# langtech-bsc/quantool

Hardware: AMD Instinct MI355X
Metric: quantized weights/sec (GPTQ int4, Llama-3-8B, 512 calib samples) (higher is better)
Workload: dtype f32

## Files before the change

include/quantool_amd.h:

```cpp
#ifndef QUANTOOL_AMD_H
#define QUANTOOL_AMD_H

#include <stddef.h>
#include <stdint.h>

#ifdef __cplusplus
extern "C" {
#endif

typedef void* qt_stream_t;

enum qt_status {
    QT_OK = 0,
    QT_ERR_INVALID = -1,
    QT_ERR_NOT_PD = -2,
    QT_ERR_WORKSPACE = -3,
    QT_ERR_HIP = -4,
    QT_ERR_UNSUPPORTED = -5
};

enum qt_dtype { QT_F32 = 0, QT_BF16 = 1, QT_F16 = 2 };

int qt_version(void);
const char* qt_last_error(void);

size_t qt_xtx_workspace_bytes(int64_t n_tokens, int K);
int qt_xtx_accumulate(const void* X, int x_dtype, int64_t n_tokens, int K, int64_t ldx, float* G,
                      void* workspace, size_t workspace_bytes, qt_stream_t stream);

size_t qt_xtx_accumulate_f32_workspace_bytes(int64_t n_tokens, int K);
int qt_xtx_accumulate_f32(const float* X, int64_t n_tokens, int K, int64_t ldx, float* G, void* workspace,
                          size_t workspace_bytes, qt_stream_t stream);

size_t qt_act_stats_workspace_bytes(int64_t n_tokens, int K);
int qt_act_stats_accumulate(const void* X, int x_dtype, int64_t n_tokens, int K, int64_t ldx, float* abs_sum,
                            float* cmin, float* cmax, void* workspace, size_t workspace_bytes,
                            qt_stream_t stream);

size_t qt_hessian_prepare_workspace_bytes(int K);
int qt_hessian_prepare(const float* G, int K, int64_t n_samples, float percdamp,
                       const int32_t* perm, float* A, uint8_t* dead, float* diag_out,
                       void* workspace, size_t workspace_bytes, qt_stream_t stream);
int qt_hessian_prepare_damp(const float* G, int K, int64_t n_samples, float percdamp,
                            const int32_t* perm, float* A, uint8_t* dead, float* diag_out, float* damp_out,
                            void* workspace, size_t workspace_bytes, qt_stream_t stream);
int qt_hessian_diag(const float* G, int K, int64_t n_samples, float* diag_out, qt_stream_t stream);
int qt_argsort_desc(const float* values, int K, int32_t* perm, int32_t* inv, qt_stream_t stream);

size_t qt_cholesky_inverse_upper_workspace_bytes(int K);
int qt_cholesky_inverse_upper(float* A, int K, float* U, int32_t* info, void* workspace,
                              size_t workspace_bytes, qt_stream_t stream);

size_t qt_cholesky_inverse_upper_batched_workspace_bytes(int K, int n_problems);
int qt_cholesky_inverse_upper_batched(float* A, int64_t strideA, int K, float* U, int64_t strideU, int32_t* info,
                                      int n_problems, void* workspace, size_t workspace_bytes, qt_stream_t stream);

int qt_cholesky_inverse_upper_bounded(float* A, int K, float* U, int32_t* info, const float* min_eig_lb,
                                      void* workspace, size_t workspace_bytes, qt_stream_t stream);
int qt_cholesky_inverse_upper_batched_bounded(float* A, int64_t strideA, int K, float* U, int64_t strideU, int32_t* info,
                                              int n_problems, const float* min_eig_lb, void* workspace,
                                              size_t workspace_bytes, qt_stream_t stream);

int qt_group_minmax_qparams(const void* W, int w_dtype, int R, int K, int64_t ldw, int group_size,
                            int symmetric, int num_bits, float* scale, float* zp, float* scale_t,
                            float* zp_t, qt_stream_t stream);

int qt_weight_gather_f32(const void* W, int w_dtype, int R, int K, int64_t ldw, const int32_t* perm,
                         const uint8_t* dead, float* W_f32, qt_stream_t stream);

int qt_weight_gather_qparams(const void* W, int w_dtype, int R, int K, int64_t ldw, const int32_t* perm,
                             const uint8_t* dead, int group_size, int symmetric, int num_bits, float* W_f32, float* scale,
                             float* zp, float* scale_t, float* zp_t, int64_t ld_t, qt_stream_t stream);

size_t qt_gptq_sweep_workspace_bytes(int R, int K, int blocksize);
int qt_gptq_sweep(float* W, int R, int K, const float* U, const float* scale_t, const float* zp_t,
                  int G, const int32_t* g_idx, int blocksize, int num_bits, int8_t* Qt,
                  float* loss, void* workspace, size_t workspace_bytes, qt_stream_t stream);

int qt_gptq_sweep_grouped(float* W, int R, int K, const float* U, int64_t strideU, int n_groups, const int32_t* row_end,
                          const float* scale_t, const float* zp_t, int G, const int32_t* g_idx, int blocksize,
                          int num_bits, int8_t* Qt, float* loss, void* workspace, size_t workspace_bytes,
                          qt_stream_t stream);

int qt_pack_int4(const int8_t* Qt, int R, int K, const int32_t* col_src, int32_t* packed,
                 qt_stream_t stream);

int qt_dequantize(const int8_t* Qt, int R, int K, const int32_t* col_src, const float* scale,
                  const float* zp, int G, const int32_t* g_of_col, void* out, int out_dtype,
                  int64_t ldo, qt_stream_t stream);

size_t qt_awq_weight_mean_workspace_bytes(int R, int K);
int qt_awq_weight_mean_accumulate(const void* W, int w_dtype, int R, int K, int64_t ldw, int group_size,
                                  float* w_sum, void* workspace, size_t workspace_bytes,
                                  qt_stream_t stream);
int qt_awq_scales(const float* x_abs_sum, int64_t n_tokens, const float* w_sum, int64_t n_rows, int K,
                  int n_grid, int duo_scaling, float* scales, qt_stream_t stream);
int qt_symmetrize_lower(float* G, int K, qt_stream_t stream);
size_t qt_awq_loss_workspace_bytes(int R, int K);
int qt_awq_loss(const void* W, int w_dtype, int R, int K, int64_t ldw, const float* s, int group_size,
                int symmetric, int num_bits, const float* Gfull, int64_t n_tokens, int exact, float weight,
                int accumulate, float* loss_out, void* workspace, size_t workspace_bytes, qt_stream_t stream);
size_t qt_awq_losses_workspace_bytes(int R, int K, int n_grid);
int qt_awq_losses(const void* W, int w_dtype, int R, int K, int64_t ldw, const float* scales, int n_grid,
                  int group_size, int symmetric, int num_bits, const float* Gfull, int64_t n_tokens, float weight,
                  int accumulate, float* losses, void* workspace, size_t workspace_bytes, qt_stream_t stream);
int qt_argmin_f32(const float* values, int n, int32_t* index_out, qt_stream_t stream);
int qt_awq_pseudo_quantize(const void* W, int w_dtype, int R, int K, int64_t ldw, const float* s, int group_size,
                           int symmetric, int num_bits, void* out, int64_t ldo, qt_stream_t stream);
int qt_scale_columns(const void* W, int w_dtype, int R, int K, int64_t ldw, const float* s, int divide,
                     void* out, int64_t ldo, qt_stream_t stream);
int qt_rtn_quantize(const void* W, int w_dtype, int R, int K, int64_t ldw, const float* scale,
                    const float* zp, int G, int group_size, int num_bits, int8_t* Qt, qt_stream_t stream);

size_t qt_col_absmax_workspace_bytes(int R, int K);
int qt_col_absmax_accumulate(const void* W, int w_dtype, int R, int K, int64_t ldw, float* wmax,
                             void* workspace, size_t workspace_bytes, qt_stream_t stream);
int qt_smoothquant_scales(const float* cmin, const float* cmax, const float* wmax, int K, float alpha,
                          float* s, qt_stream_t stream);

size_t qt_sgemm_tn_f32_workspace_bytes(int M, int N);
int qt_sgemm_tn_f32(const float* A, int64_t lda, const float* B, int64_t ldb, const float* Cin,
                    int64_t ldcin, float* Cout, int64_t ldcout, int M, int N, int kdim, int skip_zero_k,
                    int mode, int allow_split_k, void* workspace, size_t workspace_bytes, qt_stream_t stream);

int qt_xtx_tile_table_check(int K, int* n_tiles_out, int* chunk_panels_out, int* round_panels_out);

size_t qt_xtx_dot_workspace_bytes(int64_t n_tokens, int K);
int qt_xtx_dot(const void* X, int x_dtype, int64_t n_tokens, int K, int64_t ldx, const float* H, double scale,
               float* out, int accumulate, void* workspace, size_t workspace_bytes, qt_stream_t stream);

size_t qt_gemm3_tn_f32_workspace_bytes(int M, int N, int k);
int qt_gemm3_tn_f32(const float* A, int64_t lda, const float* B, int64_t ldb, float* C, int64_t ldc, int M,
                    int N, int k, int kind, void* workspace, size_t workspace_bytes, qt_stream_t stream);
int qt_gemm3_tn_f32_ex(const float* A, int64_t lda, const float* B, int64_t ldb, float* C, int64_t ldc, int M, int N,
                       int k, int kind, int tri, int tight, int batch, int64_t bsA, int64_t bsB, int64_t bsC,
                       void* workspace, size_t workspace_bytes, qt_stream_t stream);

int qt_gemm3_tn_f16x2(const float* A, int64_t lda, const float* B, int64_t ldb, float* C, int64_t ldc, int M, int N,
                      int k, int kind, int tri, int tight, int batch, int64_t bsA, int64_t bsB, int64_t bsC,
                      const float* bound_a, const float* bound_b, void* workspace, size_t workspace_bytes,
                      qt_stream_t stream);

int qt_gemm3_plan_check(int Tm, int Tn, int c_end, int tri, int* n_items_out, int* n_slabs_out, int* longest_out);
int qt_chol_g3_plan_check(int K, int merged, int min_chunks, long long* counts_out);
enum qt_act { QT_ACT_SILU = 0 };
#define QT_I8_MID_MAX_M 128
#define QT_I8_MID_K_UNIT 128
#define QT_I8_RING_K_UNIT 128
#define QT_I8_RING_SLOTS 8
#define QT_I8_RING_LEAD 6
#define QT_I8_RING_W4_K_UNIT 128
#define QT_I8_RING_W4_SLOTS 8
#define QT_I8_RING_W4_LEAD 6
#define QT_MOE_I8_WIDE_K_UNIT 128
#define QT_MOE_I8_WIDE_TILE_ROWS 128
#define QT_MOE_I8_WIDE_MAX_E 4096
enum qt_weight_format { QT_W_INT8 = 0, QT_W_INT4_PACKED = 1 };
int qt_quantize_tokens_i8(const void* X, int x_dtype, int64_t M, int K, int64_t ldx, const int32_t* col_perm,
                          int symmetric, int8_t* Xq, float* s_x, int32_t* zp_x, qt_stream_t stream);
int qt_act_mul_quantize_i8(const void* gate, int64_t ldg, const void* up, int64_t ldu, int x_dtype, int64_t M, int K,
                           int act, const int32_t* col_perm, int symmetric, int8_t* Xq, float* s_x, int32_t* zp_x,
                           void* H, int64_t ldh, qt_stream_t stream);
int qt_rmsnorm_quantize_i8(const void* X, int64_t ldx, const void* weight, int x_dtype, int64_t M, int K, float eps,
                           const int32_t* col_perm, int symmetric, int8_t* Xq, float* s_x, int32_t* zp_x,
                           void* Y, int64_t ldy, float* rstd, qt_stream_t stream);
int qt_gemm_i8(const int8_t* Xq, int64_t M, int K, const void* Wq, int w_format, int N, const float* s_x,
               const int32_t* zp_x, const float* s_w, int G, const int32_t* wsum, const void* bias, void* Y,
               int out_dtype, int64_t ldy, qt_stream_t stream);
int qt_gemm_i8_skinny(const int8_t* Xq, int M, int K, const void* Wq, int w_format, int N, const float* s_x,
                      const int32_t* zp_x, const float* s_w, int G, const int32_t* wsum, const void* bias, void* Y,
                      int out_dtype, int64_t ldy, qt_stream_t stream);
int qt_gemm_i8_ring(const int8_t* Xq, int64_t M, int K, const void* Wq, int w_format, int N, const float* s_x,
                    const int32_t* zp_x, const float* s_w, int G, const int32_t* wsum, const void* bias, void* Y,
                    int out_dtype, int64_t ldy, qt_stream_t stream);
int qt_gemm_i8_ring_w4(const int8_t* Xq, int64_t M, int K, const void* Wq, int w_format, int N, const float* s_x,
                       const int32_t* zp_x, const float* s_w, int G, const int32_t* wsum, const void* bias, void* Y,
                       int out_dtype, int64_t ldy, qt_stream_t stream);
int qt_gemm_i8_mid(const int8_t* Xq, int64_t M, int K, const void* Wq, int w_format, int N, const float* s_x,
                   const int32_t* zp_x, const float* s_w, int G, const int32_t* wsum, const void* bias, void* Y,
                   int out_dtype, int64_t ldy, qt_stream_t stream);

int qt_moe_route(const void* top_k_index, int index_is_int64, int64_t T, int k, int E, int32_t* offsets,
                 int32_t* src_token, int32_t* src_slot, int32_t* row_of, qt_stream_t stream);
int qt_gemm_i8_grouped(const int8_t* Xq, int K, const int32_t* row_idx, int64_t R, const int32_t* offsets, int E,
                       const void* Wq, int w_format, int N, const float* s_x, const int32_t* zp_x, const float* s_w,
                       int G, const int32_t* wsum, void* Y, int out_dtype, int64_t ldy, qt_stream_t stream);
int qt_gemm_i8_skinny_grouped(const int8_t* Xq, int K, const int32_t* row_idx, int64_t R, const int32_t* offsets,
                              int E, const void* Wq, int w_format, int N, const float* s_x, const int32_t* zp_x,
                              const float* s_w, int G, const int32_t* wsum, void* Y, int out_dtype, int64_t ldy,
                              qt_stream_t stream);
int qt_gemm_i8_ring_grouped(const int8_t* Xq, int K, const int32_t* row_idx, int64_t R, const int32_t* offsets, int E,
                            const void* Wq, int w_format, int N, const float* s_x, const int32_t* zp_x,
                            const float* s_w, int G, const int32_t* wsum, void* Y, int out_dtype, int64_t ldy,
                            int64_t x_rows, qt_stream_t stream);
int qt_moe_gemm_i8_ring_w4(const int8_t* Xq, int K, const int32_t* row_idx, int64_t R, const int32_t* offsets, int E,
                           const void* Wq, int w_format, int N, const float* s_x, const int32_t* zp_x,
                           const float* s_w, int G, const int32_t* wsum, void* Y, int out_dtype, int64_t ldy,
                           int64_t x_rows, qt_stream_t stream);
int qt_moe_gemm_i8_wide(const int8_t* Xq, int K, const int32_t* row_idx, int64_t R, const int32_t* offsets, int E,
                        const void* Wq, int w_format, int N, const float* s_x, const int32_t* zp_x, const float* s_w,
                        int G, const int32_t* wsum, void* Y, int out_dtype, int64_t ldy, int64_t x_rows,
                        qt_stream_t stream);
int qt_moe_combine(const void* Y, int dtype, int H, int64_t ldy, const int32_t* row_of, const float* weights,
                   int64_t T, int k, void* out, qt_stream_t stream);

int qt_dequantize_weight(const void* Wq, int w_format, int N, int K, const float* s_w, int G, const int8_t* zp_w,
                         const int32_t* g_idx, void* W, int dtype, int64_t ldw, qt_stream_t stream);
int qt_gemm_wq_skinny(const void* X, int x_dtype, int M, int K, int64_t ldx, const void* Wq, int w_format, int N,
                      const float* s_w, int G, const int8_t* zp_w, const int32_t* g_idx, const void* bias, void* Y,
                      int64_t ldy, qt_stream_t stream);

int qt_gemm_wq_stream(const void* X, int x_dtype, int M, int K, int64_t ldx, const void* Wq, int w_format, int N,
                      const float* s_w, int G, const int8_t* zp_w, const int32_t* g_idx, const void* bias, void* Y,
                      int64_t ldy, qt_stream_t stream);
#define QT_WQ_STREAM_MAX_M 128
#define QT_WQ_STREAM_K_UNIT 128
#define QT_WQ_STREAM_MAX_LDX 33554432

int qt_gemm_wq_grouped(const void* X, int x_dtype, int K, int64_t ldx, const int32_t* row_idx, int64_t R,
                       const int32_t* offsets, int E, const void* Wq, int w_format, int N, const float* s_w, int G,
                       const int8_t* zp_w, const int32_t* g_idx, void* Y, int64_t ldy, qt_stream_t stream);

int qt_moe_gemm_wq_wide(const void* X, int x_dtype, int K, int64_t ldx, const int32_t* row_idx, int64_t R,
                        const int32_t* offsets, int E, const void* Wq, int w_format, int N, const float* s_w, int G,
                        const int8_t* zp_w, const int32_t* g_idx, void* Y, int64_t ldy, int64_t x_rows,
                        qt_stream_t stream);
#define QT_MOE_WQ_WIDE_K_UNIT 128
#define QT_MOE_WQ_WIDE_MAX_E 4096
#define QT_MOE_WQ_WIDE_MAX_SLOTS 65535

enum qt_prof_kernel { QT_PROF_XTX = 0, QT_PROF_SWEEP_BLOCK = 1, QT_PROF_NUM_KERNELS = 2 };
int qt_profile_enable(int on);
int qt_profile_read(int kernel_id, double* total_ms, int64_t* launches);

#ifdef __cplusplus
}
#endif
#endif
```

quantool_amd/csrc/cholesky.hip:

```cpp
#include <stdlib.h>
#include <string.h>

#include <map>
#include <tuple>
#include <vector>

#include "common.h"
#include "gemm3_tn.h"
#include "sgemm_tn.h"

namespace {

constexpr int NB = 128;
constexpr int NBO_MAX = 1024;
static int chol_block_env(const char* name) {
    const char* e = getenv(name);
    if (!e) return 0;
    int x = atoi(e) / 128 * 128;
    return x < 128 ? 128 : (x > NBO_MAX ? NBO_MAX : x);
}
struct G3Step {
    int n_items = 0, n_red = 0;
    size_t item_off = 0, red_off = 0;
};
struct CholG3Plan {
    bool any = false;
    std::vector<G3Step> fac, inv;
    std::vector<G3Step> row;
    char* blob = nullptr;
    size_t blob_bytes = 0;
    int max_slabs = 0;
    bool any_row = false;
};

static int chol_g3_min_chunks() {
    const char* on = getenv("QT_CHOL_G3");
    if (on && atoi(on) == 0) return 0;
    const char* e = getenv("QT_CHOL_G3_MIN_CHUNKS");
    const int x = e ? atoi(e) : 64;
    return x < 1 ? 1 : x;
}

static int chol_g3_target_items(int K) {
    const char* e = getenv("QT_G3_TARGET_ITEMS");
    if (e && atoi(e) > 0) return atoi(e);
    return K < 8192 ? 96 : 256;
}

enum { CHOL_TWO_PHASE = 0, CHOL_WALK = 1, CHOL_WALK_MERGED = 2 };
static int chol_merge_mode() {
    const char* e = getenv("QT_CHOL_MERGE");
    if (!e) return CHOL_WALK_MERGED;
    if (strcmp(e, "order") == 0) return CHOL_WALK;
    return atoi(e) != 0 ? CHOL_WALK_MERGED : CHOL_TWO_PHASE;
}

static void chol_g3_build(int K, int NBO, int NBI, int min_chunks, int target_items, bool merged, CholG3Plan& pl,
                          std::vector<char>& bytes) {
    pl = CholG3Plan();
    bytes.clear();
    int slab_budget = 0;
    if (merged) {
        CholG3Plan sep;
        std::vector<char> sep_bytes;
        chol_g3_build(K, NBO, NBI, min_chunks, target_items, false, sep, sep_bytes);
        slab_budget = sep.max_slabs;
    }
    auto enough = [&](int Tm, int Tn, int c_end, int tri) {
        return min_chunks > 0 && K % 8 == 0 && g3_row_chunks(Tm, Tn, c_end, tri) * G3_CHUNK_ROWS >= (long)min_chunks * 128;
    };
    auto store = [&](const std::vector<G3Item>& items, const std::vector<G3Red>& red) {
        G3Step st;
        st.n_items = (int)items.size();
        st.n_red = (int)red.size();
        st.item_off = qt_align_up(bytes.size(), 256);
        bytes.resize(st.item_off + items.size() * sizeof(G3Item));
        memcpy(bytes.data() + st.item_off, items.data(), items.size() * sizeof(G3Item));
        st.red_off = qt_align_up(bytes.size(), 256);
        bytes.resize(st.red_off + red.size() * sizeof(G3Red));
        if (!red.empty()) memcpy(bytes.data() + st.red_off, red.data(), red.size() * sizeof(G3Red));
        for (const G3Red& r : red) pl.max_slabs = pl.max_slabs > r.first + r.count ? pl.max_slabs : r.first + r.count;
        pl.any = true;
        return st;
    };
    auto add = [&](int Tm, int Tn, int c_end, int tri) {
        if (!enough(Tm, Tn, c_end, tri)) return G3Step();
        std::vector<G3Item> items;
        std::vector<G3Red> red;
        g3_plan_row(Tm, Tn, c_end, tri, items, red, target_items);
        return store(items, red);
    };
    const bool walk = merged && NBO == NBI;
    const int cap = target_items > 0 && target_items < 256 ? target_items : 256;
    pl.row.assign(walk ? (K + NBO - 1) / NBO : 0, G3Step());
    std::vector<char> is_merged(pl.row.size(), 0);
    for (int J0 = 0, Jb = 0; J0 < K; J0 += NBO, ++Jb) {
        const int J1 = (K - J0 < NBO) ? K : J0 + NBO;
        const int Tm = (J1 - J0 + 255) / 256, Tn0 = (K - J0 + 255) / 256, Tn1 = (J0 + 255) / 256, c_end = J0 / G3_CHUNK_ROWS;
        if (walk && J0 > 0 && 2 * Tm * (Tn0 + Tn1) <= cap && enough(Tm, Tn0, c_end, 0) && enough(Tm, Tn1, c_end, 1)) {
            std::vector<G3Item> items;
            std::vector<G3Red> red;
            g3_plan_row2(Tm, Tn0, Tn1, c_end, items, red, target_items, slab_budget);
            pl.row[Jb] = store(items, red);
            is_merged[Jb] = 1;
            pl.any_row = true;
        }
    }
    for (int J0 = 0, Jb = 0; J0 < K; J0 += NBO, ++Jb) {
        const int J1 = (K - J0 < NBO) ? K : J0 + NBO;
        const bool skip = J0 == 0 || (walk && is_merged[Jb]);
        pl.fac.push_back(skip ? G3Step() : add((J1 - J0 + 255) / 256, (K - J0 + 255) / 256, J0 / G3_CHUNK_ROWS, 0));
    }
    for (int I0 = 0, Ib = 0; I0 < K; I0 += NBI, ++Ib) {
        const int I1 = (K - I0 < NBI) ? K : I0 + NBI;
        const bool skip = I0 == 0 || (walk && is_merged[Ib]);
        pl.inv.push_back(skip ? G3Step() : add((I1 - I0 + 255) / 256, (I0 + 255) / 256, I0 / G3_CHUNK_ROWS, 1));
    }
    pl.blob_bytes = pl.any ? qt_align_up(bytes.size(), 256) : 0;
}

static const CholG3Plan* chol_g3_plan(int K, int NBO, int NBI, bool merged = false) {
    static std::mutex m;
    static std::map<std::tuple<int, int, int, int>, CholG3Plan*> plans;
    const int min_chunks = chol_g3_min_chunks();
    const int target_items = chol_g3_target_items(K);
    std::lock_guard<std::mutex> lock(m);
    const auto key = std::make_tuple(K, NBO, NBI, (merged ? 1 << 30 : 0) + min_chunks * 1024 + target_items);
    auto it = plans.find(key);
    if (it != plans.end()) return it->second;
    CholG3Plan* pl = new CholG3Plan();
    std::vector<char> bytes;
    chol_g3_build(K, NBO, NBI, min_chunks, target_items, merged, *pl, bytes);
    if (pl->any) {
        if (hipHostMalloc((void**)&pl->blob, pl->blob_bytes, hipHostMallocDefault) != hipSuccess) {
            pl->any = false;
            pl->blob = nullptr;
        } else {
            memcpy(pl->blob, bytes.data(), bytes.size());
        }
    }
    if (!pl->any) {
        pl->blob_bytes = 0;
        pl->max_slabs = 0;
        for (G3Step& st : pl->fac) st = G3Step();
        for (G3Step& st : pl->inv) st = G3Step();
        for (G3Step& st : pl->row) st = G3Step();
    }
    plans[key] = pl;
    return pl;
}
static size_t chol_g3_ws_bytes(const CholG3Plan* pl, int K) {
    if (!pl->any) return 0;
    return 2 * qt_align_up((size_t)3 * K * K * 2, 256) + (size_t)pl->max_slabs * 256 * 256 * 4 + pl->blob_bytes + 256;
}

static const CholG3Plan* chol_blocks(int K, int& NBO, int& NBI) {
    const int eo = chol_block_env("QT_CHOL_NBO"), ei = chol_block_env("QT_CHOL_NBI");
    NBO = eo ? eo : 512;
    NBI = ei ? ei : 512;
    const CholG3Plan* pl = chol_g3_plan(K, NBO, NBI);
    if (pl->any) return pl;
    NBO = eo ? eo : 256;
    NBI = ei ? ei : 256;
    return chol_g3_plan(K, NBO, NBI);
}

constexpr int LDP = NB + 1;

constexpr int LDT = NB + 4;
constexpr int RD_STRIDE = NB * NB + 4 * 32 * 32;

#define QT_SEL4(kb, v0, v1, v2, v3) ((kb) == 0 ? (v0) : (kb) == 1 ? (v1) : (kb) == 2 ? (v2) : (v3))

constexpr int LDA = NB + 4;

__device__ __forceinline__ float readlane_f(float v, int lane) {
    return __int_as_float(__builtin_amdgcn_readlane(__float_as_int(v), lane));
}

__device__ __forceinline__ void mma32_tn(const float* A, int lda, const float* B, int ldb, f32x16& acc,
                                         int l31, int h, bool negate_a) {
#pragma unroll
    for (int kk = 0; kk < 16; ++kk) {
        float a = A[(2 * kk + h) * lda + l31];
        const float b = B[(2 * kk + h) * ldb + l31];
        if (negate_a) a = -a;
        acc = __builtin_amdgcn_mfma_f32_32x32x2f32(a, b, acc, 0, 0, 0);
    }
}

constexpr int POTF2_THREADS = 512, POTF2_WAVES = POTF2_THREADS / 64;
__global__ __launch_bounds__(POTF2_THREADS) void potf2_kernel(const float* P, int64_t ldp, int n,
                                                    float* Rout, int64_t ldr,
                                                    float* __restrict__ Rd, int32_t* info, int col0, int prio,
                                                    int64_t bsP, int64_t bsRd) {
    qt_set_chain_prio(prio);
    if (blockIdx.x) {
        P += (size_t)blockIdx.x * bsP;
        Rout += (size_t)blockIdx.x * bsP;
        Rd += (size_t)blockIdx.x * bsRd;
        info += blockIdx.x;
    }
    extern __shared__ __attribute__((aligned(16))) float sm[];
    float* As = sm;
    float* Xs = sm + NB * LDA;
    const int tid = threadIdx.x, lane = tid & 63;
    const int wave = __builtin_amdgcn_readfirstlane(tid >> 6);
    const int l31 = lane & 31, h = lane >> 5;

    if ((ldp & 3) == 0 && (n & 3) == 0 && (((uintptr_t)P) & 15) == 0) {
        constexpr int NV = NB * NB / 4 / POTF2_THREADS;
        f32x4 v[NV];
#pragma unroll
        for (int r = 0; r < NV; ++r) {
            const int e4 = tid + POTF2_THREADS * r;
            const int i = e4 >> 5, j = (e4 & 31) * 4;
            const int ic = i < n ? i : n - 1, jc = j < n ? j : n - 4;
            v[r] = *(const f32x4*)(P + (size_t)ic * ldp + jc);
        }
#pragma unroll
        for (int r = 0; r < NV; ++r) {
            const int e4 = tid + POTF2_THREADS * r;
            const int i = e4 >> 5, j = (e4 & 31) * 4;
            f32x4 x;
#pragma unroll
            for (int q = 0; q < 4; ++q) x[q] = (i < n && j + q < n) ? v[r][q] : (i == j + q ? 1.0f : 0.0f);
            *(f32x4*)(As + i * LDA + j) = x;
        }
    } else {
        for (int e = tid; e < NB * NB; e += POTF2_THREADS) {
            const int i = e / NB, j = e % NB;
            const int lo = i < j ? i : j, hi = i < j ? j : i;
            float v = (i == j) ? 1.0f : 0.0f;
            if (hi < n) v = P[(size_t)lo * ldp + hi];
            As[i * LDA + j] = v;
        }
    }
    __syncthreads();

    int bad = 0;
#pragma unroll 1
    for (int kb = 0; kb < 4; ++kb) {
        float* Akk = As + (32 * kb) * LDA + 32 * kb;
        if (wave == 0) {
            f32x16 c1, c2;
#pragma unroll
            for (int r = 0; r < 16; ++r) {
                const int i = (r & 3) + 8 * (r >> 2) + 4 * h;
                c1[r] = Akk[i * LDA + l31];
                c2[r] = (i == l31) ? 1.0f : 0.0f;
            }
#pragma unroll
            for (int c = 0; c < 32; ++c) {
                const int rc = (c & 3) + 4 * (c >> 3);
                const int hc = (c >> 2) & 1;
                float piv = readlane_f(c1[rc], c + 32 * hc);
                const bool isbad = !(piv > 0.0f);
                bad = (isbad && bad == 0 && 32 * kb + c < n) ? 32 * kb + c + 1 : bad;
                piv = isbad ? 1.0f : piv;
                float rs = __builtin_amdgcn_rsqf(piv);
                rs = rs * fmaf(-0.5f * piv * rs, rs, 1.5f);
                const bool mine = h == hc;
                const float rr = c1[rc] * rs, zz = c2[rc] * rs;
                c1[rc] = mine ? rr : c1[rc];
                c2[rc] = mine ? zz : c2[rc];
                if (c < 31) {
                    const float a = (mine && l31 > c) ? -rr : 0.0f;
                    const float b1 = (mine && l31 >= c) ? rr : 0.0f, b2 = mine ? zz : 0.0f;
                    c1 = __builtin_amdgcn_mfma_f32_32x32x2f32(a, b1, c1, 0, 0, 0);
                    c2 = __builtin_amdgcn_mfma_f32_32x32x2f32(a, b2, c2, 0, 0, 0);
                }
            }
#pragma unroll
            for (int r = 0; r < 16; ++r) {
                const int i = (r & 3) + 8 * (r >> 2) + 4 * h;
                Akk[i * LDA + l31] = (i <= l31) ? c1[r] : 0.0f;
                Xs[(kb * 32 + l31) * 32 + i] = (i >= l31) ? c2[r] : 0.0f;
            }
        }
        __syncthreads();
        if (kb == 3) break;
        for (int a = kb + 1 + wave; a < 4; a += POTF2_WAVES) {
            f32x16 acc;
#pragma unroll
            for (int r = 0; r < 16; ++r) acc[r] = 0.0f;
            float* Bt = As + (32 * kb) * LDA + 32 * a;
            mma32_tn(Xs + kb * 1024, 32, Bt, LDA, acc, l31, h, false);
#pragma unroll
            for (int r = 0; r < 16; ++r) Bt[((r & 3) + 8 * (r >> 2) + 4 * h) * LDA + l31] = acc[r];
        }
        __syncthreads();
        {
            int t = 0;
            for (int a = kb + 1; a < 4; ++a)
                for (int a2 = a; a2 < 4; ++a2, ++t) {
                    if ((t % POTF2_WAVES) != wave) continue;
                    float* Ct = As + (32 * a) * LDA + 32 * a2;
                    f32x16 acc;
#pragma unroll
                    for (int r = 0; r < 16; ++r) acc[r] = Ct[((r & 3) + 8 * (r >> 2) + 4 * h) * LDA + l31];
                    mma32_tn(As + (32 * kb) * LDA + 32 * a, LDA, As + (32 * kb) * LDA + 32 * a2, LDA, acc, l31, h,
                             true);
#pragma unroll
                    for (int r = 0; r < 16; ++r) Ct[((r & 3) + 8 * (r >> 2) + 4 * h) * LDA + l31] = acc[r];
                }
        }
        __syncthreads();
    }
    if (bad != 0 && tid == 0) atomicCAS(info, 0, col0 + bad);
    const bool vec_out = (ldr & 3) == 0 && (n & 3) == 0 && (((uintptr_t)Rout) & 15) == 0;
    for (int e4 = tid; e4 < NB * NB / 4; e4 += POTF2_THREADS) {
        const int i = e4 >> 5, j = (e4 & 31) * 4;
        f32x4 v = *(const f32x4*)(As + i * LDA + j);
#pragma unroll
        for (int q = 0; q < 4; ++q) v[q] = (j + q >= i) ? v[q] : 0.0f;
        *(f32x4*)(Rd + i * NB + j) = v;
        if (i < n && j + 3 >= i && j < n) {
            if (vec_out) {
                *(f32x4*)(Rout + (size_t)i * ldr + j) = v;
            } else {
#pragma unroll
                for (int q = 0; q < 4; ++q)
                    if (j + q >= i && j + q < n) Rout[(size_t)i * ldr + j + q] = v[q];
            }
        }
    }
    for (int e4 = tid; e4 < 4 * 32 * 32 / 4; e4 += POTF2_THREADS) *(f32x4*)(Rd + NB * NB + 4 * e4) = *(const f32x4*)(Xs + 4 * e4);
}

__global__ __launch_bounds__(256) void trsm_rt_kernel(const float* __restrict__ Rd, int n,
                                                      const float* B, int64_t ldb,
                                                      float* Z, int64_t ldz, int ncols, int prio, int64_t bsRd,
                                                      int64_t bsB) {
    qt_set_chain_prio(prio);
    if (blockIdx.y) {
        Rd += (size_t)blockIdx.y * bsRd;
        B += (size_t)blockIdx.y * bsB;
        Z += (size_t)blockIdx.y * bsB;
    }
    extern __shared__ __attribute__((aligned(16))) float Rs[];
    const int tid = threadIdx.x, lane = tid & 63, wave = tid >> 6;
    const float* D32 = Rs + NB * NB;
    const int l31 = lane & 31, h = lane >> 5;
    const int col = blockIdx.x * 128 + wave * 32 + l31;
    const bool cok = col < ncols;
    const int colc = cok ? col : ncols - 1;

    f32x16 acc[4];
#pragma unroll
    for (int a = 0; a < 4; ++a)
#pragma unroll
        for (int r = 0; r < 16; ++r) {
            const int row = 32 * a + (r & 3) + 8 * (r >> 2) + 4 * h;
            acc[a][r] = (row < n) ? B[(size_t)row * ldb + colc] : 0.0f;
        }
    {
        constexpr int NV = RD_STRIDE / 4 / 256;
        static_assert(NV * 4 * 256 == RD_STRIDE, "whole float4s per thread");
        f32x4 v[NV];
#pragma unroll
        for (int r = 0; r < NV; ++r) v[r] = ((const f32x4*)Rd)[tid + 256 * r];
#pragma unroll
        for (int r = 0; r < NV; ++r) ((f32x4*)Rs)[tid + 256 * r] = v[r];
    }
    __syncthreads();

#pragma unroll
    for (int b = 0; b < 4; ++b) {
        f32x16 zb;
#pragma unroll
        for (int r = 0; r < 16; ++r) zb[r] = 0.0f;
#pragma unroll
        for (int r = 0; r < 16; ++r) {
            const int k = (r & 3) + 8 * (r >> 2) + 4 * h;
            const float av = D32[(b * 32 + k) * 32 + l31];
            zb = __builtin_amdgcn_mfma_f32_32x32x2f32(av, acc[b][r], zb, 0, 0, 0);
        }
        acc[b] = zb;
#pragma unroll
        for (int a = b + 1; a < 4; ++a) {
#pragma unroll
            for (int r = 0; r < 16; ++r) {
                const int k = (r & 3) + 8 * (r >> 2) + 4 * h;
                const float av = -Rs[(32 * b + k) * NB + 32 * a + l31];
                acc[a] = __builtin_amdgcn_mfma_f32_32x32x2f32(av, zb[r], acc[a], 0, 0, 0);
            }
        }
    }
    if (cok) {
#pragma unroll
        for (int a = 0; a < 4; ++a)
#pragma unroll
            for (int r = 0; r < 16; ++r) {
                const int row = 32 * a + (r & 3) + 8 * (r >> 2) + 4 * h;
                if (row < n) Z[(size_t)row * ldz + col] = acc[a][r];
            }
    }
}

__global__ __launch_bounds__(128) void trinv_batched_kernel(const float* __restrict__ Rd_all, int K,
                                                            float* __restrict__ Dinv_all,
                                                            float* __restrict__ Y, int64_t ldy, int64_t bsW, int64_t bsY,
                                                            int blk0) {
    if (blockIdx.y) {
        Rd_all += (size_t)blockIdx.y * bsW;
        Dinv_all += (size_t)blockIdx.y * bsW;
        Y += (size_t)blockIdx.y * bsY;
    }
    extern __shared__ __attribute__((aligned(16))) float sm[];
    float* Rt = sm;
    float* Xs = sm + NB * LDT;
    const int b = blk0 + blockIdx.x;
    const int n = (K - b * NB < NB) ? K - b * NB : NB;
    const float* Rd = Rd_all + (size_t)b * RD_STRIDE;
    const int j = threadIdx.x;
    for (int e = j; e < NB * NB; e += NB) {
        const int i = e / NB, c = e % NB;
        Rt[c * LDT + i] = Rd[e];
    }
    __syncthreads();
    float x0[32], x1[32], x2[32], x3[32];
#pragma unroll
    for (int r = 0; r < 32; ++r) {
        x0[r] = (r == j) ? 1.0f : 0.0f;
        x1[r] = (32 + r == j) ? 1.0f : 0.0f;
        x2[r] = (64 + r == j) ? 1.0f : 0.0f;
        x3[r] = (96 + r == j) ? 1.0f : 0.0f;
    }
#pragma unroll 1
    for (int pb = 3; pb >= 0; --pb) {
#pragma unroll
        for (int pp = 31; pp >= 0; --pp) {
            const int p = 32 * pb + pp;
            const float* rp = Rt + p * LDT;
            const float xp = QT_SEL4(pb, x0[pp], x1[pp], x2[pp], x3[pp]) / rp[p];
            if (pb == 0) x0[pp] = xp;
            if (pb == 1) x1[pp] = xp;
            if (pb == 2) x2[pp] = xp;
            if (pb == 3) x3[pp] = xp;
#define QT_XUPD(arr, a, r_to)                                                 \
    _Pragma("unroll") for (int r4 = 0; r4 < (r_to); r4 += 4) {                 \
        const f32x4 v4 = *(const f32x4*)(rp + 32 * (a) + r4);                 \
        _Pragma("unroll") for (int e = 0; e < 4; ++e)                         \
            if (r4 + e < (r_to)) arr[r4 + e] = fmaf(-v4[e], xp, arr[r4 + e]); \
    }
            if (pb == 0) { QT_XUPD(x0, 0, pp) } else { QT_XUPD(x0, 0, 32) }
            if (pb == 1) { QT_XUPD(x1, 1, pp) } else if (pb > 1) { QT_XUPD(x1, 1, 32) }
            if (pb == 2) { QT_XUPD(x2, 2, pp) } else if (pb > 2) { QT_XUPD(x2, 2, 32) }
            if (pb == 3) { QT_XUPD(x3, 3, pp) }
#undef QT_XUPD
        }
    }
#pragma unroll
    for (int r = 0; r < 32; ++r) {
        Xs[r * LDP + j] = x0[r];
        Xs[(32 + r) * LDP + j] = x1[r];
        Xs[(64 + r) * LDP + j] = x2[r];
        Xs[(96 + r) * LDP + j] = x3[r];
    }
    __syncthreads();
    float* Dinv = Dinv_all + (size_t)b * NB * NB;
    float* Yd = Y + (size_t)(b * NB) * ldy + b * NB;
    for (int e = j; e < NB * NB; e += NB) {
        const int i = e / NB, jj = e % NB;
        const bool in = (i < n && jj < n);
        Dinv[e] = (in && jj >= i) ? Xs[i * LDP + jj] : 0.0f;
        if (in) Yd[(size_t)i * ldy + jj] = (jj <= i) ? Xs[jj * LDP + i] : 0.0f;
    }
}

__global__ __launch_bounds__(256) void trinv_mfma_kernel(const float* __restrict__ Rd_all, int K,
                                                         float* __restrict__ Dinv_all,
                                                         float* __restrict__ Y, int64_t ldy, int64_t bsW, int64_t bsY,
                                                         int blk0) {
    if (blockIdx.y) {
        Rd_all += (size_t)blockIdx.y * bsW;
        Dinv_all += (size_t)blockIdx.y * bsW;
        Y += (size_t)blockIdx.y * bsY;
    }
    extern __shared__ __attribute__((aligned(16))) float Rs[];
    const int blk = blk0 + blockIdx.x;
    const int n = (K - blk * NB < NB) ? K - blk * NB : NB;
    const float* Rd = Rd_all + (size_t)blk * RD_STRIDE;
    const int tid = threadIdx.x, lane = tid & 63, wave = tid >> 6;
    {
        constexpr int NV = RD_STRIDE / 4 / 256;
        f32x4 v[NV];
#pragma unroll
        for (int r = 0; r < NV; ++r) v[r] = ((const f32x4*)Rd)[tid + 256 * r];
#pragma unroll
        for (int r = 0; r < NV; ++r) ((f32x4*)Rs)[tid + 256 * r] = v[r];
    }
    const float* D32 = Rs + NB * NB;
    const int l31 = lane & 31, h = lane >> 5;
    const int col = wave * 32 + l31;

    f32x16 acc[4];
#pragma unroll
    for (int a = 0; a < 4; ++a)
#pragma unroll
        for (int r = 0; r < 16; ++r) {
            const int row = 32 * a + (r & 3) + 8 * (r >> 2) + 4 * h;
            acc[a][r] = (row == col) ? 1.0f : 0.0f;
        }
    __syncthreads();

#pragma unroll
    for (int b = 0; b < 4; ++b) {
        f32x16 zb;
#pragma unroll
        for (int r = 0; r < 16; ++r) zb[r] = 0.0f;
#pragma unroll
        for (int r = 0; r < 16; ++r) {
            const int k = (r & 3) + 8 * (r >> 2) + 4 * h;
            const float av = D32[(b * 32 + k) * 32 + l31];
            zb = __builtin_amdgcn_mfma_f32_32x32x2f32(av, acc[b][r], zb, 0, 0, 0);
        }
        acc[b] = zb;
#pragma unroll
        for (int a = b + 1; a < 4; ++a) {
#pragma unroll
            for (int r = 0; r < 16; ++r) {
                const int k = (r & 3) + 8 * (r >> 2) + 4 * h;
                const float av = -Rs[(32 * b + k) * NB + 32 * a + l31];
                acc[a] = __builtin_amdgcn_mfma_f32_32x32x2f32(av, zb[r], acc[a], 0, 0, 0);
            }
        }
    }
    float* Dinv = Dinv_all + (size_t)blk * NB * NB;
    float* Yd = Y + (size_t)(blk * NB) * ldy + blk * NB;
#pragma unroll
    for (int a = 0; a < 4; ++a)
#pragma unroll
        for (int r = 0; r < 16; ++r) {
            const int row = 32 * a + (r & 3) + 8 * (r >> 2) + 4 * h;
            const bool in = row < n && col < n;
            const float z = (in && row >= col) ? acc[a][r] : 0.0f;
            Dinv[col * NB + row] = z;
            if (in) Yd[(size_t)row * ldy + col] = z;
        }
}

__global__ __launch_bounds__(256) void transpose_lower_block_kernel(const float* __restrict__ Y, int64_t ldy, int w,
                                                                    float* __restrict__ XT, int ldx, int64_t bsY,
                                                                    int64_t bsXT) {
    if (blockIdx.z) {
        Y += (size_t)blockIdx.z * bsY;
        XT += (size_t)blockIdx.z * bsXT;
    }
    __shared__ float tile[32][33];
    const int bx = blockIdx.x * 32, by = blockIdx.y * 32;
    const int tx = threadIdx.x & 31, ty = threadIdx.x >> 5;
    for (int r = ty; r < 32; r += 8) {
        const int m = bx + r, k = by + tx;
        tile[r][tx] = (m < w && k < w && k <= m) ? Y[(size_t)m * ldy + k] : 0.0f;
    }
    __syncthreads();
    for (int r = ty; r < 32; r += 8) {
        const int k = by + r, m = bx + tx;
        if (k < w && m < w) XT[(size_t)k * ldx + m] = tile[tx][r];
    }
}

__global__ __launch_bounds__(256) void flat_reverse_lower_to_upper_kernel(float* __restrict__ U, int K, int64_t bsU) {
    U += (size_t)blockIdx.z * bsU;
    const int j = blockIdx.x * blockDim.x + threadIdx.x;
    const int i = blockIdx.y;
    if (j >= K || j < i) return;
    const size_t e = (size_t)i * K + j;
    const size_t pe = (size_t)(K - 1 - i) * K + (K - 1 - j);
    if (i == j) {
        if (e <= pe) {
            const float t = U[e];
            U[e] = U[pe];
            U[pe] = t;
        }
    } else {
        U[e] = U[pe];
        U[pe] = 0.0f;
    }
}

__global__ __launch_bounds__(256) void identity_if_failed_kernel(float* __restrict__ U, int K,
                                                                 const int32_t* __restrict__ info, int64_t bsU) {
    if (info[blockIdx.z] == 0) return;
    U += (size_t)blockIdx.z * bsU;
    for (int i = blockIdx.x; i < K; i += gridDim.x)
        for (int j = threadIdx.x; j < K; j += blockDim.x) U[(size_t)i * K + j] = (i == j) ? 1.0f : 0.0f;
}

__global__ __launch_bounds__(256) void chol_scales_kernel(const float* __restrict__ A, int64_t bsA, int K,
                                                          const float* __restrict__ min_eig_lb, int32_t* __restrict__ e,
                                                          int32_t* __restrict__ info) {
    __shared__ float red[256];
    const int b = blockIdx.x, nprob = gridDim.x;
    const float* Ab = A + (size_t)b * bsA;
    float m = 0.0f;
    for (int i = threadIdx.x; i < K; i += 256) m = fmaxf(m, Ab[(size_t)i * K + i]);
    red[threadIdx.x] = m;
    __syncthreads();
    for (int s = 128; s > 0; s >>= 1) {
        if ((int)threadIdx.x < s) red[threadIdx.x] = fmaxf(red[threadIdx.x], red[threadIdx.x + s]);
        __syncthreads();
    }
    if (threadIdx.x == 0) {
        auto clampe = [](float t) { return (int)fminf(fmaxf(t, (float)-G3_E_MAX), (float)G3_E_MAX); };
        const float d = red[0], lb = min_eig_lb[b];
        e[b] = (d > 0.0f && d < 3.0e38f) ? clampe(3.0f - ceilf(0.5f * log2f(d))) : 0;
        if (lb > 0.0f && lb < 3.0e38f) {
            e[nprob + b] = clampe(3.0f - ceilf(-0.5f * log2f(lb)));
        } else {
            e[nprob + b] = 0;
            info[b] = K + 1;
        }
    }
}

}

static size_t chol_problem_ws_bytes(int K, const CholG3Plan* g3) {
    const size_t nb = (K + NB - 1) / NB;
    const size_t split = (size_t)2048 * NB * NB * 4 + (size_t)NBO_MAX * K * 4;
    size_t n = (size_t)NB * K * 4 + (size_t)NBO_MAX * K * 4 + (size_t)NBO_MAX * NBO_MAX * 4 + nb * (NB * NB + RD_STRIDE) * 4 + split + 256;
    if (g3->any) n += 2 * qt_align_up((size_t)3 * K * K * 2, 256) + (size_t)g3->max_slabs * 256 * 256 * 4 + 256;
    return qt_align_up(n, 256);
}

extern "C" size_t qt_cholesky_inverse_upper_batched_workspace_bytes(int K, int n_problems) {
    if (K <= 0 || n_problems <= 0) return 0;
    int nbo_, nbi_;
    const CholG3Plan* g3 = chol_blocks(K, nbo_, nbi_);
    return (size_t)n_problems * chol_problem_ws_bytes(K, g3) + g3->blob_bytes + 512;
}

extern "C" size_t qt_cholesky_inverse_upper_workspace_bytes(int K) {
    return qt_cholesky_inverse_upper_batched_workspace_bytes(K, 1);
}

static int chol_run(float* A, int64_t strideA, int K, float* U, int64_t strideU, int32_t* info, int nprob, void* workspace,
                    size_t workspace_bytes, hipStream_t stream, const float* min_eig_lb = nullptr) {
    bool f16x2 = min_eig_lb != nullptr;
    if (const char* e = getenv("QT_CHOL_PLANES")) {
        if (strcmp(e, "bf16x3") == 0) f16x2 = false;
        else if (strcmp(e, "f16x2") == 0) {
            QT_CHECK_ARG(min_eig_lb, "qt_cholesky_inverse_upper: QT_CHOL_PLANES=f16x2 needs a bound on lambda_min (the _bounded entry points)");
        } else {
            QT_CHECK_ARG(false, "qt_cholesky_inverse_upper: QT_CHOL_PLANES=%s (bf16x3 | f16x2)", e);
        }
    }
    const size_t need = qt_cholesky_inverse_upper_batched_workspace_bytes(K, nprob);
    if (!workspace || workspace_bytes < need) {
        qt_set_error("qt_cholesky_inverse_upper: workspace %zu < required %zu", workspace_bytes, need);
        return QT_ERR_WORKSPACE;
    }
    const int nblk = (K + NB - 1) / NB;
    char* ws = (char*)qt_align_up((size_t)workspace, 256);
    int NBO, NBI;
    const CholG3Plan* g3 = chol_blocks(K, NBO, NBI);
    int merge_mode = (g3->any && NBO == NBI) ? chol_merge_mode() : CHOL_TWO_PHASE;
    const CholG3Plan* tab = g3;
    if (merge_mode == CHOL_WALK_MERGED) {
        tab = chol_g3_plan(K, NBO, NBI, true);
        if (!tab->any || !tab->any_row || tab->max_slabs > g3->max_slabs || tab->blob_bytes > g3->blob_bytes) {
            tab = g3;
            merge_mode = CHOL_TWO_PHASE;
        }
    }
    const size_t prob_bytes = chol_problem_ws_bytes(K, g3);
    const int64_t sW = (int64_t)(prob_bytes / 4);
    const int64_t sA = nprob > 1 ? strideA : 0, sU = nprob > 1 ? strideU : 0;
    float* T = (float*)ws;
    float* TI = T + (size_t)NB * K;
    float* XT = TI + (size_t)NBO_MAX * K;
    float* Rd = XT + (size_t)NBO_MAX * NBO_MAX;
    float* Dinv = Rd + (size_t)nblk * RD_STRIDE;
    float* split_ws = Dinv + (size_t)nblk * NB * NB;
    const size_t split_ws_bytes = (size_t)2048 * NB * NB * 4 + (size_t)NBO_MAX * K * 4;
    unsigned short *Rpl = nullptr, *Ypl = nullptr;
    float* g3_slabs = nullptr;
    char* g3_tab = nullptr;
    const int64_t plane_stride = (int64_t)K * K;
    if (g3->any) {
        char* q = (char*)qt_align_up((size_t)((char*)split_ws + split_ws_bytes), 256);
        Rpl = (unsigned short*)q;
        q += qt_align_up((size_t)3 * K * K * 2, 256);
        Ypl = (unsigned short*)q;
        q += qt_align_up((size_t)3 * K * K * 2, 256);
        g3_slabs = (float*)q;
        g3_tab = (char*)qt_align_up((size_t)(ws + (size_t)nprob * prob_bytes), 256);
        QT_HIP(hipMemcpyAsync(g3_tab, tab->blob, tab->blob_bytes, hipMemcpyHostToDevice, stream));
    }
    f16x2 = f16x2 && g3->any;
    int32_t* eR = f16x2 ? (int32_t*)(Rpl + 2 * plane_stride) : nullptr;
    int32_t* eY = f16x2 ? eR + nprob : nullptr;
    static_assert(2 * SG_MAX_BATCH * sizeof(int32_t) <= (size_t)NB * NB * 2, "the exponents fit the smallest third plane");
    auto g3_row = [&](const G3Step& st, const unsigned short* Bplanes, int col_a0, int col_b0, int M, int N, float* C,
                      int64_t bsC, int mode, bool second = false) -> int {
        G3Args a;
        a.Apl = Rpl;
        a.Bpl = Bplanes;
        a.plane_stride = plane_stride;
        a.ld = K;
        a.rowA0 = a.rowB0 = 0;
        a.colA0 = col_a0;
        a.colB0 = col_b0;
        a.colmax = K;
        a.M = M;
        a.N = N;
        a.C = C;
        a.ldc = K;
        a.mode = mode;
        a.slabs = g3_slabs;
        a.items = (const G3Item*)(g3_tab + st.item_off);
        a.n_items = st.n_items;
        a.red = (const G3Red*)(g3_tab + st.red_off);
        a.n_red = st.n_red;
        a.batch = nprob;
        a.bsApl = a.bsBpl = sW * 2;
        a.bsC = bsC;
        a.bsSlabs = sW;
        if (f16x2) {
            a.planes = G3_F16X2;
            a.eA = eR;
            a.eB = Bplanes == Rpl ? eR : eY;
        }
        if (second) {
            a.Bpl1 = Ypl;
            a.colB01 = 0;
            a.eB1 = eY;
            a.C1 = TI;
            a.ldc1 = K;
            a.bsC1 = sW;
            a.mode1 = G3_SET;
            a.N1 = col_a0;
        }
        return qt_gemm3_launch(a, stream);
    };
    auto sgemm = [&](SgemmArgs& g, int64_t bsA_, int64_t bsB_, int64_t bsC_) -> int {
        g.batch = nprob;
        g.bsA = bsA_;
        g.bsB = bsB_;
        g.bsCin = g.bsCout = bsC_;
        g.bs_split = sW;
        return qt_sgemm_tn(g, stream);
    };
    float* Y = U;
    const int64_t sY = sU;
    const size_t inv_lds = (size_t)(NB * LDT + NB * LDP) * sizeof(float);
    const size_t potf2_lds = (size_t)(NB * LDA + 4 * 32 * 32) * sizeof(float);
    static QtOncePerDevice lds_attr;
    QT_HIP(lds_attr.run([&] {
        hipError_t e = hipFuncSetAttribute((const void*)potf2_kernel, hipFuncAttributeMaxDynamicSharedMemorySize,
                                           (int)potf2_lds);
        if (e == hipSuccess)
            e = hipFuncSetAttribute((const void*)trsm_rt_kernel, hipFuncAttributeMaxDynamicSharedMemorySize,
                                    (int)(RD_STRIDE * sizeof(float)));
        if (e == hipSuccess)
            e = hipFuncSetAttribute((const void*)trinv_batched_kernel, hipFuncAttributeMaxDynamicSharedMemorySize,
                                    (int)inv_lds);
        if (e == hipSuccess)
            e = hipFuncSetAttribute((const void*)trinv_mfma_kernel, hipFuncAttributeMaxDynamicSharedMemorySize,
                                    (int)(RD_STRIDE * sizeof(float)));
        return e;
    }));
    QT_HIP(hipMemsetAsync(info, 0, sizeof(int32_t) * nprob, stream));
    const int prio = qt_chain_prio();
    if (f16x2) {
        hipLaunchKernelGGL(chol_scales_kernel, dim3(nprob), dim3(256), 0, stream, (const float*)A, sA, K, min_eig_lb, eR, info);
        QT_LAUNCH_CHECK();
    }

    auto fac_product = [&](int J0, int J1, int Jb) -> int {
        if (!(g3->any && J0 > 0)) return QT_OK;
        const G3Step& st = tab->fac[Jb];
        float* C = A + (size_t)J0 * K + J0;
        if (st.n_items > 0) return g3_row(st, Rpl, J0, J0, J1 - J0, K - J0, C, sA, G3_SUB);
        SgemmArgs g;
        g.A = A + J0; g.lda = K;
        g.B = A + J0; g.ldb = K;
        g.Cin = C; g.ldcin = K;
        g.Cout = C; g.ldcout = K;
        g.M = J1 - J0; g.N = K - J0; g.kdim = J0; g.k_mode = SG_K_FULL; g.mode = SG_MODE_SUB;
        g.split_ws = split_ws; g.split_ws_bytes = split_ws_bytes;
        return sgemm(g, sA, sA, sA);
    };
    auto fac_panels = [&](int J0, int J1) -> int {
        for (int j0 = J0; j0 < J1; j0 += NB) {
            const int j = j0 / NB, nbj = (K - j0 < NB) ? K - j0 : NB;
            float* Ajj = A + (size_t)j0 * K + j0;
            if (j0 > J0) {
                SgemmArgs g;
                g.A = A + (size_t)J0 * K + j0; g.lda = K;
                g.B = A + (size_t)J0 * K + j0; g.ldb = K;
                g.Cin = Ajj; g.ldcin = K;
                g.Cout = Ajj; g.ldcout = K;
                g.M = nbj; g.N = K - j0; g.kdim = j0 - J0; g.k_mode = SG_K_FULL; g.mode = SG_MODE_SUB;
                int rc = sgemm(g, sA, sA, sA);
                if (rc) return rc;
            }
            hipLaunchKernelGGL(potf2_kernel, dim3(nprob), dim3(POTF2_THREADS), potf2_lds, stream, (const float*)Ajj, (int64_t)K, nbj,
                               Ajj, (int64_t)K, Rd + (size_t)j * RD_STRIDE, info, j0, prio, sA, sW);
            QT_LAUNCH_CHECK();
            const int rest = K - j0 - nbj;
            if (rest > 0) {
                hipLaunchKernelGGL(trsm_rt_kernel, dim3((rest + 127) / 128, nprob), dim3(256), RD_STRIDE * sizeof(float),
                                   stream, (const float*)(Rd + (size_t)j * RD_STRIDE), nbj, (const float*)(Ajj + nbj),
                                   (int64_t)K, Ajj + nbj, (int64_t)K, rest, prio, sW, sA);
                QT_LAUNCH_CHECK();
            }
        }
        const int rem = K - J1;
        if (g3->any) {
            if (rem > 0) {
                int rc = f16x2 ? qt_split2h_launch(A + (size_t)J0 * K + J0, K, J1 - J0, K - J0, Rpl + (size_t)J0 * K + J0, K,
                                                   plane_stride, 0, 0, 0, eR, stream, nprob, sA, sW * 2)
                               : qt_split3_launch(A + (size_t)J0 * K + J0, K, J1 - J0, K - J0, Rpl + (size_t)J0 * K + J0, K,
                                                  plane_stride, 0, 0, 0, stream, nprob, sA, sW * 2);
                if (rc) return rc;
            }
        } else if (rem > 0) {
            SgemmArgs g;
            g.A = A + (size_t)J0 * K + J1; g.lda = K;
            g.B = A + (size_t)J0 * K + J1; g.ldb = K;
            g.Cin = A + (size_t)J1 * K + J1; g.ldcin = K;
            g.Cout = A + (size_t)J1 * K + J1; g.ldcout = K;
            g.M = rem; g.N = rem; g.kdim = J1 - J0; g.k_mode = SG_K_FULL; g.mode = SG_MODE_SUB;
            g.upper_only = 1;
            int rc = sgemm(g, sA, sA, sA);
            if (rc) return rc;
        }
        return QT_OK;
    };
    auto trinv = [&](int blk0, int n) -> int {
        const char* e = getenv("QT_CHOL_TRINV");
        if (e && strcmp(e, "div") == 0)
            hipLaunchKernelGGL(trinv_batched_kernel, dim3(n, nprob), dim3(NB), inv_lds, stream, (const float*)Rd, K, Dinv, Y,
                               (int64_t)K, sW, sY, blk0);
        else
            hipLaunchKernelGGL(trinv_mfma_kernel, dim3(n, nprob), dim3(256), RD_STRIDE * sizeof(float), stream,
                               (const float*)Rd, K, Dinv, Y, (int64_t)K, sW, sY, blk0);
        QT_LAUNCH_CHECK();
        return QT_OK;
    };
    auto inv_product = [&](int I0, int I1, int Ib) -> int {
        if (I0 == 0) return QT_OK;
        if (g3->any && tab->inv[Ib].n_items > 0) return g3_row(tab->inv[Ib], Ypl, I0, 0, I1 - I0, I0, TI, sW, G3_SET);
        SgemmArgs g;
        g.A = A + I0; g.lda = K;
        g.B = Y; g.ldb = K;
        g.Cin = nullptr; g.ldcin = 0;
        g.Cout = TI; g.ldcout = K;
        g.M = I1 - I0; g.N = I0; g.kdim = I0; g.k_mode = SG_K_FROM_N0; g.mode = SG_MODE_SET;
        g.split_ws = split_ws; g.split_ws_bytes = split_ws_bytes;
        return sgemm(g, sA, sY, sW);
    };
    auto inv_row = [&](int I0, int I1) -> int {
        const int Wi = I1 - I0;
        for (int i0 = I0 + NB; i0 < I1; i0 += NB) {
            const int i = i0 / NB, nbi = (K - i0 < NB) ? K - i0 : NB;
            SgemmArgs g;
            g.A = A + (size_t)I0 * K + i0; g.lda = K;
            g.B = Y + (size_t)I0 * K + I0; g.ldb = K;
            g.Cin = nullptr; g.ldcin = 0;
            g.Cout = T; g.ldcout = K;
            g.M = nbi; g.N = i0 - I0; g.kdim = i0 - I0; g.k_mode = SG_K_FROM_N0; g.mode = SG_MODE_SET;
            int rc = sgemm(g, sA, sY, sW);
            if (rc) return rc;
            SgemmArgs t;
            t.A = Dinv + (size_t)i * NB * NB; t.lda = NB;
            t.B = T; t.ldb = K;
            t.Cin = nullptr; t.ldcin = 0;
            t.Cout = Y + (size_t)i0 * K + I0; t.ldcout = K;
            t.M = nbi; t.N = i0 - I0; t.kdim = nbi; t.k_mode = SG_K_FULL; t.mode = SG_MODE_NEG;
            rc = sgemm(t, sW, sW, sY);
            if (rc) return rc;
        }
        auto split_row = [&]() -> int {
            if (!g3->any || I1 >= K) return QT_OK;
            if (f16x2)
                return qt_split2h_launch(Y + (size_t)I0 * K, K, Wi, I1, Ypl + (size_t)I0 * K, K, plane_stride, 1, I0, 0, eY,
                                         stream, nprob, sY, sW * 2);
            return qt_split3_launch(Y + (size_t)I0 * K, K, Wi, I1, Ypl + (size_t)I0 * K, K, plane_stride, 1, I0, 0, stream,
                                    nprob, sY, sW * 2);
        };
        if (I0 == 0) return split_row();
        hipLaunchKernelGGL(transpose_lower_block_kernel, dim3((Wi + 31) / 32, (Wi + 31) / 32, nprob), dim3(256), 0, stream,
                           (const float*)(Y + (size_t)I0 * K + I0), (int64_t)K, Wi, XT, NBO_MAX, sY, sW);
        QT_LAUNCH_CHECK();
        SgemmArgs t;
        t.A = XT; t.lda = NBO_MAX;
        t.B = TI; t.ldb = K;
        t.Cin = nullptr; t.ldcin = 0;
        t.Cout = Y + (size_t)I0 * K; t.ldcout = K;
        t.M = Wi; t.N = I0; t.kdim = Wi; t.k_mode = SG_K_FULL; t.mode = SG_MODE_NEG;
        int rc = sgemm(t, sW, sW, sY);
        if (rc) return rc;
        return split_row();
    };
    if (merge_mode == CHOL_TWO_PHASE) {
        for (int J0 = 0, Jb = 0; J0 < K; J0 += NBO, ++Jb) {
            const int J1 = (K - J0 < NBO) ? K : J0 + NBO;
            int rc = fac_product(J0, J1, Jb);
            if (!rc) rc = fac_panels(J0, J1);
            if (rc) return rc;
        }
        int rc = trinv(0, nblk);
        if (rc) return rc;
        for (int I0 = 0, Ib = 0; I0 < K; I0 += NBI, ++Ib) {
            const int I1 = (K - I0 < NBI) ? K : I0 + NBI;
            rc = inv_product(I0, I1, Ib);
            if (!rc) rc = inv_row(I0, I1);
            if (rc) return rc;
        }
    } else {
        for (int J0 = 0, Jb = 0; J0 < K; J0 += NBO, ++Jb) {
            const int J1 = (K - J0 < NBO) ? K : J0 + NBO;
            int rc;
            if (merge_mode == CHOL_WALK_MERGED && tab->row[Jb].n_items > 0) {
                rc = g3_row(tab->row[Jb], Rpl, J0, J0, J1 - J0, K - J0, A + (size_t)J0 * K + J0, sA, G3_SUB, true);
            } else {
                rc = fac_product(J0, J1, Jb);
                if (!rc) rc = inv_product(J0, J1, Jb);
            }
            if (!rc) rc = fac_panels(J0, J1);
            if (!rc) rc = trinv(J0 / NB, (J1 - J0 + NB - 1) / NB);
            if (!rc) rc = inv_row(J0, J1);
            if (rc) return rc;
        }
    }
    hipLaunchKernelGGL(flat_reverse_lower_to_upper_kernel, dim3((K + 255) / 256, K, nprob), dim3(256), 0, stream, U, K, sU);
    QT_LAUNCH_CHECK();
    hipLaunchKernelGGL(identity_if_failed_kernel, dim3(K < 1024 ? K : 1024, 1, nprob), dim3(256), 0, stream, U, K,
                       (const int32_t*)info, sU);
    QT_LAUNCH_CHECK();
    return QT_OK;
}

extern "C" int qt_cholesky_inverse_upper(float* A, int K, float* U, int32_t* info, void* workspace,
                                         size_t workspace_bytes, qt_stream_t stream_) {
    QT_CHECK_ARG(K > 0 && A && U && info, "qt_cholesky_inverse_upper: bad arguments");
    return chol_run(A, 0, K, U, 0, info, 1, workspace, workspace_bytes, (hipStream_t)stream_);
}

extern "C" int qt_cholesky_inverse_upper_batched(float* A, int64_t strideA, int K, float* U, int64_t strideU, int32_t* info,
                                                 int n_problems, void* workspace, size_t workspace_bytes,
                                                 qt_stream_t stream_) {
    QT_CHECK_ARG(K > 0 && A && U && info && n_problems >= 1 && n_problems <= SG_MAX_BATCH,
                 "qt_cholesky_inverse_upper_batched: bad arguments (1 <= n_problems <= %d)", SG_MAX_BATCH);
    QT_CHECK_ARG(n_problems == 1 || (strideA >= (int64_t)K * K && strideU >= (int64_t)K * K && strideA % 4 == 0 && strideU % 4 == 0),
                 "qt_cholesky_inverse_upper_batched: strides must be multiples of 4 elements and >= K*K");
    return chol_run(A, strideA, K, U, strideU, info, n_problems, workspace, workspace_bytes, (hipStream_t)stream_);
}

extern "C" int qt_cholesky_inverse_upper_bounded(float* A, int K, float* U, int32_t* info, const float* min_eig_lb,
                                                 void* workspace, size_t workspace_bytes, qt_stream_t stream_) {
    QT_CHECK_ARG(K > 0 && A && U && info && min_eig_lb, "qt_cholesky_inverse_upper_bounded: bad arguments");
    return chol_run(A, 0, K, U, 0, info, 1, workspace, workspace_bytes, (hipStream_t)stream_, min_eig_lb);
}

extern "C" int qt_cholesky_inverse_upper_batched_bounded(float* A, int64_t strideA, int K, float* U, int64_t strideU,
                                                         int32_t* info, int n_problems, const float* min_eig_lb,
                                                         void* workspace, size_t workspace_bytes, qt_stream_t stream_) {
    QT_CHECK_ARG(K > 0 && A && U && info && min_eig_lb && n_problems >= 1 && n_problems <= SG_MAX_BATCH,
                 "qt_cholesky_inverse_upper_batched_bounded: bad arguments (1 <= n_problems <= %d)", SG_MAX_BATCH);
    QT_CHECK_ARG(n_problems == 1 || (strideA >= (int64_t)K * K && strideU >= (int64_t)K * K && strideA % 4 == 0 && strideU % 4 == 0),
                 "qt_cholesky_inverse_upper_batched_bounded: strides must be multiples of 4 elements and >= K*K");
    return chol_run(A, strideA, K, U, strideU, info, n_problems, workspace, workspace_bytes, (hipStream_t)stream_, min_eig_lb);
}

extern "C" int qt_chol_g3_plan_check(int K, int merged, int min_chunks, long long* counts_out) {
    if (K <= 0) return -1;
    constexpr int NBX = 512, TRI_STEP = 256 / G3_CHUNK_ROWS;
    if (min_chunks <= 0) min_chunks = 64;
    const int cap = chol_g3_target_items(K);
    CholG3Plan sep, pl;
    std::vector<char> sep_bytes, bytes;
    chol_g3_build(K, NBX, NBX, min_chunks, cap, false, sep, sep_bytes);
    chol_g3_build(K, NBX, NBX, min_chunks, cap, merged != 0, pl, bytes);
    if (pl.max_slabs > sep.max_slabs || pl.blob_bytes > sep.blob_bytes) return -2;
    long long launches = 0, n_items = 0, n_slabs = 0;
    auto check = [&](const G3Step& st, int Tm, int Tn0, int tri0, int Tn1, int c_end) -> int {
        if (st.n_items <= 0) return 0;
        const G3Item* items = (const G3Item*)(bytes.data() + st.item_off);
        const G3Red* red = (const G3Red*)(bytes.data() + st.red_off);
        if (st.n_items > cap && st.n_items > Tm * (Tn0 + Tn1)) return -3;
        const int Tn[2] = {Tn0, Tn1};
        auto lo_of = [&](int seg, int tj) { return (seg == 1 || tri0) ? TRI_STEP * tj : 0; };
        std::vector<int> cover((size_t)2 * Tm * (Tn0 + Tn1 + 1) * c_end, 0);
        auto cell = [&](int seg, int ti, int tj, int c) { return (((size_t)seg * Tm + ti) * (Tn0 + Tn1 + 1) + tj) * c_end + c; };
        std::vector<int> owner(sep.max_slabs, -1);
        int slabs_here = 0;
        for (int q = 0; q < st.n_items; ++q) {
            const G3Item& it = items[q];
            const int seg = (it.tile & G3_SEG_BIT) ? 1 : 0, ti = it.tile >> 16, tj = it.tile & G3_TJ_MASK;
            if (ti < 0 || ti >= Tm || tj >= Tn[seg]) return -4;
            const int lo = lo_of(seg, tj);
            if (it.c_lo < lo || it.c_hi > c_end || it.c_hi - it.c_lo < 2) return -5;
            for (int c = it.c_lo; c < it.c_hi; ++c) cover[cell(seg, ti, tj, c)]++;
            if (it.slab < 0) {
                if (it.c_lo != lo || it.c_hi != c_end) return -6;
            } else {
                if (it.slab >= sep.max_slabs) return -7;
                if (owner[it.slab] >= 0) return -8;
                owner[it.slab] = q;
                ++slabs_here;
            }
        }
        for (int seg = 0; seg < 2; ++seg)
            for (int ti = 0; ti < Tm; ++ti)
                for (int tj = 0; tj < Tn[seg]; ++tj)
                    for (int c = 0; c < c_end; ++c)
                        if (cover[cell(seg, ti, tj, c)] != (c >= lo_of(seg, tj) ? 1 : 0)) return -9;
        int in_red = 0;
        for (int r = 0; r < st.n_red; ++r) {
            const G3Red& e = red[r];
            if (e.count < 2 || e.first < 0 || e.first + e.count > sep.max_slabs || (e.seg != 0 && e.seg != 1)) return -10;
            const int want_tile = e.tile | (e.seg ? G3_SEG_BIT : 0);
            int prev_hi = lo_of(e.seg, e.tile & G3_TJ_MASK);
            for (int q = 0; q < e.count; ++q) {
                const int o = owner[e.first + q];
                if (o < 0 || items[o].tile != want_tile || items[o].c_lo != prev_hi) return -11;
                prev_hi = items[o].c_hi;
                owner[e.first + q] = -2;
            }
            if (prev_hi != c_end) return -12;
            in_red += e.count;
        }
        if (in_red != slabs_here) return -13;
        ++launches;
        n_items += st.n_items;
        n_slabs += slabs_here;
        return 0;
    };
    for (int J0 = 0, Jb = 0; J0 < K; J0 += NBX, ++Jb) {
        const int J1 = (K - J0 < NBX) ? K : J0 + NBX;
        const int Tm = (J1 - J0 + 255) / 256, Tn0 = (K - J0 + 255) / 256, Tn1 = (J0 + 255) / 256, c_end = J0 / G3_CHUNK_ROWS;
        int rc = 0;
        if (Jb < (int)pl.row.size() && pl.row[Jb].n_items > 0) {
            if (pl.fac[Jb].n_items > 0 || pl.inv[Jb].n_items > 0) return -14;
            rc = check(pl.row[Jb], Tm, Tn0, 0, Tn1, c_end);
        } else {
            rc = check(pl.fac[Jb], Tm, Tn0, 0, 0, c_end);
            if (!rc) rc = check(pl.inv[Jb], Tm, Tn1, 1, 0, c_end);
        }
        if (rc) return rc;
    }
    if (counts_out) {
        counts_out[0] = launches;
        counts_out[1] = n_items;
        counts_out[2] = n_slabs;
        counts_out[3] = sep.max_slabs;
        counts_out[4] = (long long)pl.blob_bytes;
    }
    return 0;
}
```

quantool_amd/csrc/common.h:

```cpp
#pragma once
#include <hip/hip_runtime.h>
#include <stdint.h>
#include <stdio.h>

#include <mutex>

#include "../../include/quantool_amd.h"

typedef __attribute__((ext_vector_type(8))) __bf16 bf16x8;
typedef __attribute__((ext_vector_type(8))) _Float16 f16x8;
typedef __attribute__((ext_vector_type(4))) short s16x4;
typedef __attribute__((ext_vector_type(8))) short s16x8;
typedef __attribute__((ext_vector_type(2))) float f32x2;
typedef __attribute__((ext_vector_type(4))) float f32x4;
typedef __attribute__((ext_vector_type(16))) float f32x16;

#define QT_LDS __attribute__((address_space(3)))
#define QT_GLOBAL __attribute__((address_space(1)))

void qt_set_error(const char* fmt, ...);
void qt_prof_mark(int kernel_id, hipStream_t stream);

#define QT_CHECK_ARG(cond, ...)         \
    do {                                \
        if (!(cond)) {                  \
            qt_set_error(__VA_ARGS__);  \
            return QT_ERR_INVALID;      \
        }                               \
    } while (0)

#define QT_HIP(expr)                                                              \
    do {                                                                          \
        hipError_t _e = (expr);                                                   \
        if (_e != hipSuccess) {                                                   \
            qt_set_error("%s failed: %s (%s:%d)", #expr, hipGetErrorString(_e),   \
                         __FILE__, __LINE__);                                     \
            return QT_ERR_HIP;                                                    \
        }                                                                         \
    } while (0)

#define QT_LAUNCH_CHECK()                                                         \
    do {                                                                          \
        hipError_t _e = hipGetLastError();                                        \
        if (_e != hipSuccess) {                                                   \
            qt_set_error("kernel launch failed: %s (%s:%d)", hipGetErrorString(_e), \
                         __FILE__, __LINE__);                                     \
            return QT_ERR_HIP;                                                    \
        }                                                                         \
    } while (0)

static inline size_t qt_align_up(size_t x, size_t a) { return (x + a - 1) / a * a; }

size_t qt_xtx_frobenius_workspace_bytes(int64_t n_tokens, int K, int n_batch);
int qt_xtx_frobenius(const void* X, int x_dtype, int64_t n_tokens, int K, int64_t ldx, const float* H, double scale,
                     float* loss_out, int accumulate, void* workspace, size_t workspace_bytes, hipStream_t stream,
                     int n_batch, int64_t x_batch_stride);

int qt_chain_prio();
__device__ __forceinline__ void qt_set_chain_prio(int prio) {
    if (prio >= 3) __builtin_amdgcn_s_setprio(3);
    else if (prio == 2) __builtin_amdgcn_s_setprio(2);
    else if (prio == 1) __builtin_amdgcn_s_setprio(1);
}

struct QtOncePerDevice {
    std::mutex m;
    uint64_t done = 0;
    template <class F>
    hipError_t run(F&& f) {
        int dev = 0;
        hipError_t e = hipGetDevice(&dev);
        if (e != hipSuccess) return e;
        const uint64_t bit = 1ull << (dev & 63);
        std::lock_guard<std::mutex> lock(m);
        if (done & bit) return hipSuccess;
        e = f();
        if (e == hipSuccess) done |= bit;
        return e;
    }
};

__device__ __forceinline__ float qt_bf16_to_f32(unsigned short h) {
    return __uint_as_float(((unsigned)h) << 16);
}
__device__ __forceinline__ float qt_f16_to_f32(unsigned short h) {
    return (float)__builtin_bit_cast(_Float16, h);
}
__device__ __forceinline__ float qt_h16_to_f32(unsigned short h, int dtype) {
    return dtype == QT_F16 ? qt_f16_to_f32(h) : qt_bf16_to_f32(h);
}
__device__ __forceinline__ float qt_load_w(const void* W, int dtype, size_t idx) {
    if (dtype == QT_F32) return ((const float*)W)[idx];
    return qt_h16_to_f32(((const unsigned short*)W)[idx], dtype);
}
__device__ __forceinline__ void qt_store_w(void* out, int dtype, size_t idx, float v) {
    if (dtype == QT_F32) ((float*)out)[idx] = v;
    else if (dtype == QT_F16) ((_Float16*)out)[idx] = (_Float16)v;
    else ((__bf16*)out)[idx] = (__bf16)v;
}
static inline bool qt_dtype_ok(int d) { return d == QT_F32 || d == QT_BF16 || d == QT_F16; }
static inline bool qt_dtype_is16(int d) { return d == QT_BF16 || d == QT_F16; }
static inline size_t qt_dtype_size(int d) { return d == QT_F32 ? 4 : 2; }
```

quantool_amd/csrc/gemm3_tn.h:

```cpp
#pragma once
#include <vector>

#include "common.h"

constexpr int G3_CHUNK_ROWS = 64;

struct G3Item {
    int tile;
    int c_lo;
    int c_hi;
    int slab;
};
struct G3Red {
    int tile;
    int first;
    int count;
    int seg;
};
constexpr int G3_SEG_BIT = 1 << 15;
constexpr int G3_TJ_MASK = G3_SEG_BIT - 1;

enum { G3_SUB = 0, G3_SET = 1, G3_ADD = 2 };

enum { G3_BF16X3 = 0, G3_F16X2 = 1 };
constexpr int G3_E_MAX = 40;

struct G3Args {
    const unsigned short* Apl;
    const unsigned short* Bpl;
    int64_t plane_stride;
    int64_t ld;
    int64_t rowA0, rowB0;
    int colA0, colB0;
    int colmax;
    int M, N;
    float* C;
    int64_t ldc;
    int64_t ldB = 0, plane_strideB = 0;
    int colmaxB = 0;
    int mode;
    float* slabs;
    const G3Item* items;
    int n_items;
    const G3Red* red;
    int n_red;
    int batch = 1;
    int64_t bsApl = 0, bsBpl = 0, bsC = 0, bsSlabs = 0;
    int planes = G3_BF16X3;
    const int32_t* eA = nullptr;
    const int32_t* eB = nullptr;
    const unsigned short* Bpl1 = nullptr;
    int colB01 = 0;
    const int32_t* eB1 = nullptr;
    float* C1 = nullptr;
    int64_t ldc1 = 0, bsC1 = 0;
    int mode1 = G3_SET;
    int N1 = 0;
};

int qt_gemm3_launch(const G3Args& a, hipStream_t stream);

int qt_split3_launch(const float* src, int64_t ld_src, int rows, int cols, unsigned short* planes, int64_t ld_pl,
                     int64_t plane_stride, int mask_upper, int row_g0, int col_g0, hipStream_t stream, int batch = 1,
                     int64_t bs_src = 0, int64_t bs_planes = 0);

int qt_split2h_launch(const float* src, int64_t ld_src, int rows, int cols, unsigned short* planes, int64_t ld_pl,
                      int64_t plane_stride, int mask_upper, int row_g0, int col_g0, const int32_t* e, hipStream_t stream,
                      int batch = 1, int64_t bs_src = 0, int64_t bs_planes = 0);

int g3_scale_exponent(float bound);

long g3_row_chunks(int Tm, int Tn, int c_end, int tri);
void g3_plan_row(int Tm, int Tn, int c_end, int tri, std::vector<G3Item>& items, std::vector<G3Red>& red, int target_items = 0);
void g3_plan_row2(int Tm, int Tn0, int Tn1, int c_end, std::vector<G3Item>& items, std::vector<G3Red>& red,
                  int target_items = 0, int max_slabs = 0);
```

quantool_amd/csrc/gemm3_tn.hip:

```cpp
#include <math.h>
#include <stdlib.h>
#include <string.h>

#include <algorithm>
#include <map>
#include <mutex>
#include <type_traits>

#include "gemm3_tn.h"
#include "ring_pipe.h"

namespace {

constexpr int RING = 8;
constexpr int CH_ROWS = G3_CHUNK_ROWS;
constexpr int CH_UNITS = 6 * (CH_ROWS / UT);
constexpr int TRING = 3;
constexpr int TRI_BYTES = 3 * UNIT_BYTES;
constexpr int TRI_DMA = 6;
constexpr int DRING = 4;
constexpr int DUO_BYTES = 2 * UNIT_BYTES;
constexpr int DUO_DMA = 4;
constexpr int DUO_LEAD = 2;
enum { LOOP_CHUNK = 0, LOOP_TRI = 1, LOOP_DUO = 2 };
static_assert(CH_ROWS / UT == 4, "the phase code below recomputes the source pointers every 4 units");
constexpr unsigned PA_BITS = 2u | (0u << 2) | (1u << 4) | (1u << 6) | (0u << 8) | (0u << 10);
constexpr unsigned PB_BITS = 0u | (2u << 2) | (1u << 4) | (0u << 6) | (1u << 8) | (0u << 10);
constexpr int g3_plane_a(int pr) { return (PA_BITS >> (2 * pr)) & 3u; }
constexpr int g3_plane_b(int pr) { return (PB_BITS >> (2 * pr)) & 3u; }

struct G3Params {
    const char* Apl;
    const char* Bpl;
    int64_t plane_bytes, plane_bytesB;
    int64_t ld2, ld2B;
    int64_t rowA0, rowB0;
    int colA0, colB0, colmax, colmaxB;
    int M, N;
    float* C;
    int64_t ldc;
    float* slabs;
    const G3Item* items;
    int64_t bsA_bytes, bsB_bytes, bsC, bsSlabs;
    const int32_t* eA;
    const int32_t* eB;
    const char* Bpl1;
    const int32_t* eB1;
    float* C1;
    int64_t ldc1, bsC1;
    int colB01, N1, mode1;
};

template <int MODE, int LOOP>
__global__ __launch_bounds__(NTHREADS, 2) void gemm3_kernel(G3Params p) {
    constexpr bool TRI = LOOP == LOOP_TRI;
    __shared__ __attribute__((aligned(16))) char ring[LOOP == LOOP_DUO ? DRING * DUO_BYTES : TRI ? TRING * TRI_BYTES : RING * UNIT_BYTES];
    const int tid = threadIdx.x;
    const int lane = tid & 63;
    const int wave = __builtin_amdgcn_readfirstlane(tid >> 6);
    const int wave_m = wave >> 2, wave_n = wave & 3;
    const bool group_b = wave >= 4;

    const G3Item* itp = p.items + blockIdx.x;
    const int it_tile = __builtin_amdgcn_readfirstlane(itp->tile);
    const bool seg1 = (it_tile & G3_SEG_BIT) != 0;
    const char* Bpl = seg1 ? p.Bpl1 : p.Bpl;
    const int colB0 = seg1 ? p.colB01 : p.colB0;
    if (blockIdx.y) {
        p.Apl += (size_t)blockIdx.y * p.bsA_bytes;
        Bpl += (size_t)blockIdx.y * p.bsB_bytes;
        p.slabs += (size_t)blockIdx.y * p.bsSlabs;
    }
    const int c_lo = __builtin_amdgcn_readfirstlane(itp->c_lo);
    const int c_hi = __builtin_amdgcn_readfirstlane(itp->c_hi);
    const int slab_idx = __builtin_amdgcn_readfirstlane(itp->slab);
    const int ti = it_tile >> 16, tj = it_tile & G3_TJ_MASK;
    const int nu = (c_hi - c_lo) * (LOOP != LOOP_CHUNK ? CH_ROWS / UT : CH_UNITS);

    const int rsub = lane >> 4;
    const int lch = (lane & 15) ^ (rsub << 2);
    const int trow = 4 * (wave & 3) + rsub;
    int colA = p.colA0 + ti * BT + (wave >> 2) * 128 + lch * 8;
    int colB = colB0 + tj * BT + (wave >> 2) * 128 + lch * 8;
    colA = colA > p.colmax - 8 ? p.colmax - 8 : colA;
    colB = colB > p.colmaxB - 8 ? p.colmaxB - 8 : colB;
    const unsigned voffA = (unsigned)((size_t)trow * (size_t)p.ld2 + (size_t)colA * 2);
    const unsigned voffB = (unsigned)((size_t)trow * (size_t)p.ld2B + (size_t)colB * 2);
    const unsigned ring_lds = (unsigned)(size_t)(QT_LDS char*)ring;
    const unsigned dst_wave =
        __builtin_amdgcn_readfirstlane(ring_lds + (wave >> 2) * 4096 + (wave & 3) * 1024);

    const int64_t ustride = (int64_t)UT * p.ld2, ustrideB = (int64_t)UT * p.ld2B;

    const int g = lane >> 4, il = lane & 15, q = il >> 2, pp = il & 3;
    const int rowpart = (8 * (g >> 1) + q) * 256 + 32 * (g & 1) + 8 * pp;
    int aoff[4], boff[2];
#pragma unroll
    for (int mi = 0; mi < 4; ++mi) aoff[mi] = wave_m * 4096 + rowpart + 64 * (mi ^ q);
#pragma unroll
    for (int ni = 0; ni < 2; ++ni)
        boff[ni] = (2 + (wave_n >> 1)) * 4096 + rowpart + 64 * ((((wave_n & 1) << 1) + ni) ^ q);

    f32x16 acc[4][2];
#pragma unroll
    for (int mi = 0; mi < 4; ++mi)
#pragma unroll
        for (int ni = 0; ni < 2; ++ni)
#pragma unroll
            for (int r = 0; r < 16; ++r) acc[mi][ni][r] = 0.0f;

    if constexpr (LOOP == LOOP_DUO) {
        const char* runA = p.Apl + (p.rowA0 + (int64_t)c_lo * CH_ROWS) * p.ld2;
        const char* runB = Bpl + (p.rowB0 + (int64_t)c_lo * CH_ROWS) * p.ld2B;
        auto issue2 = [&](int slot) {
            const unsigned d = dst_wave + (unsigned)slot * DUO_BYTES;
#pragma unroll
            for (int pl = 0; pl < 2; ++pl)
                glds16_pair2(voffA, voffB, runA + pl * p.plane_bytes, runB + pl * p.plane_bytesB, d + pl * UNIT_BYTES,
                             d + pl * UNIT_BYTES + 8192);
            runA += ustride;
            runB += ustrideB;
        };
        s16x8 fa[2][4], fb[2][2];
        auto phase = [&](auto slot_c, int u) {
            constexpr int S = decltype(slot_c)::value;
            constexpr int ISLOT = (S + DUO_LEAD) % DRING;
            const char* base = ring + S * DUO_BYTES;
#pragma unroll
            for (int pl = 0; pl < 2; ++pl) {
#pragma unroll
                for (int mi = 0; mi < 4; ++mi) fa[pl][mi] = tr_load8(base + pl * UNIT_BYTES + aoff[mi]);
#pragma unroll
                for (int ni = 0; ni < 2; ++ni) fb[pl][ni] = tr_load8(base + pl * UNIT_BYTES + boff[ni]);
            }
            if (u + DUO_LEAD < nu) issue2(ISLOT);
            ring_drain_wait<DUO_DMA, DUO_LEAD>(nu - u - 2);
            ring_sync_math([&] {
                s16x8 fbs[2];
#pragma unroll
                for (int ni = 0; ni < 2; ++ni)
                    fbs[ni] = __builtin_bit_cast(s16x8, __builtin_bit_cast(f16x8, fb[0][ni]) * (_Float16)2048.0f);
                ring_mma32<true>(fa[1], fb[0], acc);
                ring_mma32<true>(fa[0], fb[1], acc);
                ring_mma32<true>(fa[0], fbs, acc);
            });
        };
        if (nu > 0) {
            issue2(0);
            issue2(1);
            wait_vmcnt<DUO_DMA*(DUO_LEAD - 1)>();
            ring_stagger_begin(group_b);
            for (int u = 0; u < nu; u += DRING) ring_body<DRING>(phase, u);
            ring_stagger_end(group_b);
        }
        const int es = -(11 + p.eA[blockIdx.y] + (seg1 ? p.eB1 : p.eB)[blockIdx.y]);
        const float unscale = __builtin_bit_cast(float, (unsigned)(127 + (es < -126 ? -126 : es > 127 ? 127 : es)) << 23);
#pragma unroll
        for (int mi = 0; mi < 4; ++mi)
#pragma unroll
            for (int ni = 0; ni < 2; ++ni)
#pragma unroll
                for (int r = 0; r < 16; ++r) acc[mi][ni][r] *= unscale;
    } else if constexpr (TRI) {
        const char* runA = p.Apl + (p.rowA0 + (int64_t)c_lo * CH_ROWS) * p.ld2;
        const char* runB = Bpl + (p.rowB0 + (int64_t)c_lo * CH_ROWS) * p.ld2B;
        auto issue3 = [&](int slot) {
            const unsigned d = dst_wave + (unsigned)slot * TRI_BYTES;
#pragma unroll
            for (int pl = 0; pl < 3; ++pl)
                glds16_pair2(voffA, voffB, runA + pl * p.plane_bytes, runB + pl * p.plane_bytesB, d + pl * UNIT_BYTES,
                             d + pl * UNIT_BYTES + 8192);
            runA += ustride;
            runB += ustrideB;
        };
        s16x8 fa[3][4], fb[3][2];
        auto phase = [&](auto slot_c, int u) {
            constexpr int S = decltype(slot_c)::value;
            constexpr int ISLOT = (S + 2) % TRING;
            const bool more = u + 2 < nu;
            if (group_b && more) issue3(ISLOT);
            const char* base = ring + S * TRI_BYTES;
#pragma unroll
            for (int pl = 0; pl < 3; ++pl) {
#pragma unroll
                for (int mi = 0; mi < 4; ++mi) fa[pl][mi] = tr_load8(base + pl * UNIT_BYTES + aoff[mi]);
#pragma unroll
                for (int ni = 0; ni < 2; ++ni) fb[pl][ni] = tr_load8(base + pl * UNIT_BYTES + boff[ni]);
            }
            if (group_b) ring_drain_wait<TRI_DMA, 2>(nu - u - 2);
            ring_sync_math(
                [&] {
                    if (!group_b && more) issue3(ISLOT);
                },
                [&] {
                    ring_mma32<false>(fa[g3_plane_a(0)], fb[g3_plane_b(0)], acc);
                    ring_mma32<false>(fa[g3_plane_a(1)], fb[g3_plane_b(1)], acc);
                    ring_mma32<false>(fa[g3_plane_a(2)], fb[g3_plane_b(2)], acc);
                    ring_mma32<false>(fa[g3_plane_a(3)], fb[g3_plane_b(3)], acc);
                    ring_mma32<false>(fa[g3_plane_a(4)], fb[g3_plane_b(4)], acc);
                    ring_mma32<false>(fa[g3_plane_a(5)], fb[g3_plane_b(5)], acc);
                },
                [&] {
                    if (!group_b) ring_drain_wait<TRI_DMA, 2>(nu - u - 2);
                });
        };
        if (nu > 0) {
            issue3(0);
            issue3(1);
            wait_vmcnt<TRI_DMA>();
            ring_stagger_begin(group_b);
            int u = 0;
            for (; u + TRING <= nu; u += TRING) ring_body<TRING>(phase, u);
            if (u < nu) phase(std::integral_constant<int, 0>{}, u);
            if (u + 1 < nu) phase(std::integral_constant<int, 1>{}, u + 1);
            ring_stagger_end(group_b);
        }
    } else {
        constexpr int LEAD = 6;
        auto unit_src = [&](int i, const char*& a, const char*& b) {
            const int g = i >> 2, j = i & 3;
            const int c = g / 6, pr = g - 6 * c;
            const int64_t plA = (PA_BITS >> (2 * pr)) & 3u, plB = (PB_BITS >> (2 * pr)) & 3u;
            const int64_t row = (int64_t)(c_lo + c) * CH_ROWS + j * UT;
            a = p.Apl + plA * p.plane_bytes + (p.rowA0 + row) * p.ld2;
            b = Bpl + plB * p.plane_bytesB + (p.rowB0 + row) * p.ld2B;
        };
        auto issue = [&](int i, int slot) {
            const char *a, *b;
            unit_src(i, a, b);
            const unsigned d = dst_wave + (unsigned)slot * UNIT_BYTES;
            glds16_pair2(voffA, voffB, a, b, d, d + 8192);
        };
        const char *runA = nullptr, *runB = nullptr;

        s16x8 fa[4], fb[2];
        auto drain_wait = [&](int u) {
            ring_drain_wait<2, LEAD>(nu - u - 2);
        };
        auto phase = [&](auto slot_c, auto steady_c, int u) {
            constexpr int S = decltype(slot_c)::value;
            constexpr bool STEADY = decltype(steady_c)::value;
            constexpr int ISLOT = (S + LEAD) & (RING - 1);
            const char* base = ring + S * UNIT_BYTES;
#pragma unroll
            for (int mi = 0; mi < 4; ++mi) fa[mi] = tr_load8(base + aoff[mi]);
#pragma unroll
            for (int ni = 0; ni < 2; ++ni) fb[ni] = tr_load8(base + boff[ni]);
            if (STEADY) {
                if (S == 2 || S == 6) unit_src(u + LEAD, runA, runB);
                const unsigned d = dst_wave + (unsigned)ISLOT * UNIT_BYTES;
                glds16_pair2(voffA, voffB, runA, runB, d, d + 8192);
                runA += ustride;
                runB += ustrideB;
                wait_vmcnt<2 * (LEAD - 1)>();
            } else if (u + LEAD < nu) {
                issue(u + LEAD, ISLOT);
                wait_vmcnt<2 * (LEAD - 1)>();
            } else {
                drain_wait(u);
            }
            ring_sync_math([&] { ring_mma32<false>(fa, fb, acc); });
        };
        auto body8 = [&](auto steady_c, int u) {
            ring_body<8>([&](auto slot_c, int uu) { phase(slot_c, steady_c, uu); }, u);
        };

        if (nu > 0) {
#pragma unroll
            for (int i = 0; i < LEAD; ++i) issue(i, i);
            wait_vmcnt<2 * (LEAD - 1)>();
            ring_stagger_begin(group_b);
            unit_src(LEAD, runA, runB);
            int u = 0;
            for (; u + 8 + LEAD <= nu; u += 8) body8(std::true_type{}, u);
            for (; u + 8 <= nu; u += 8) body8(std::false_type{}, u);
            ring_stagger_end(group_b);
        }
    }

    const int jl = lane & 31, ih = 4 * (lane >> 5);
    if (slab_idx < 0) {
        float* C = (seg1 ? p.C1 : p.C) + (size_t)blockIdx.y * (size_t)(seg1 ? p.bsC1 : p.bsC);
        const int64_t ldc = seg1 ? p.ldc1 : p.ldc;
        const int N = seg1 ? p.N1 : p.N;
        auto apply = [&](auto mode_c) {
            constexpr int M_ = decltype(mode_c)::value;
#pragma unroll
            for (int mi = 0; mi < 4; ++mi)
#pragma unroll
                for (int ni = 0; ni < 2; ++ni) {
                    const int gj = tj * BT + wave_n * 64 + ni * 32 + jl;
#pragma unroll
                    for (int r = 0; r < 16; ++r) {
                        const int gi = ti * BT + wave_m * 128 + mi * 32 + (r & 3) + 8 * (r >> 2) + ih;
                        if (gi < p.M && gj < N) {
                            float* dst = C + (size_t)gi * ldc + gj;
                            if (M_ == G3_SUB) *dst = *dst - acc[mi][ni][r];
                            else if (M_ == G3_ADD) *dst = *dst + acc[mi][ni][r];
                            else *dst = acc[mi][ni][r];
                        }
                    }
                }
        };
        const int mode = seg1 ? p.mode1 : MODE;
        if (mode == G3_SUB) apply(std::integral_constant<int, G3_SUB>{});
        else if (mode == G3_ADD) apply(std::integral_constant<int, G3_ADD>{});
        else apply(std::integral_constant<int, G3_SET>{});
    } else {
        float* slab = p.slabs + (size_t)slab_idx * (size_t)(BT * BT);
#pragma unroll
        for (int mi = 0; mi < 4; ++mi)
#pragma unroll
            for (int ni = 0; ni < 2; ++ni)
#pragma unroll
                for (int r = 0; r < 16; ++r) {
                    const int i_loc = wave_m * 128 + mi * 32 + (r & 3) + 8 * (r >> 2) + ih;
                    const int j_loc = wave_n * 64 + ni * 32 + jl;
                    slab[i_loc * BT + j_loc] = acc[mi][ni][r];
                }
    }
}

__global__ __launch_bounds__(256) void gemm3_reduce_kernel(const float* __restrict__ slabs,
                                                           const G3Red* __restrict__ red, float* C, int64_t ldc,
                                                           int M, int N, int mode, int64_t bsSlabs, int64_t bsC,
                                                           float* C1, int64_t ldc1, int N1, int mode1, int64_t bsC1) {
    const G3Red t = red[blockIdx.x];
    if (t.seg) {
        C = C1;
        ldc = ldc1;
        N = N1;
        mode = mode1;
        bsC = bsC1;
    }
    if (blockIdx.z) {
        slabs += (size_t)blockIdx.z * bsSlabs;
        C += (size_t)blockIdx.z * bsC;
    }
    const int ti = t.tile >> 16, tj = t.tile & 0xFFFF;
    const int part = blockIdx.y;
    const size_t tile_elems = (size_t)BT * BT;
    for (int e = threadIdx.x; e < 16 * (BT / 4); e += blockDim.x) {
        const int i_loc = part * 16 + e / (BT / 4);
        const int j_loc = (e % (BT / 4)) * 4;
        const int gi = ti * BT + i_loc, gj = tj * BT + j_loc;
        if (gi >= M || gj >= N) continue;
        f32x4 s = {0.f, 0.f, 0.f, 0.f};
        for (int sp = 0; sp < t.count; ++sp) {
            const f32x4 v = *(const f32x4*)(slabs + (size_t)(t.first + sp) * tile_elems + (size_t)i_loc * BT + j_loc);
            s += v;
        }
        float* dst = C + (size_t)gi * ldc + gj;
        if (gj + 3 < N && (ldc & 3) == 0 && (((uintptr_t)C) & 15) == 0) {
            if (mode == G3_SUB) {
                f32x4 o = *(f32x4*)dst;
                o -= s;
                *(f32x4*)dst = o;
            } else if (mode == G3_ADD) {
                f32x4 o = *(f32x4*)dst;
                o += s;
                *(f32x4*)dst = o;
            } else {
                *(f32x4*)dst = s;
            }
        } else {
            for (int c = 0; c < 4 && gj + c < N; ++c)
                dst[c] = (mode == G3_SUB) ? dst[c] - s[c] : (mode == G3_ADD) ? dst[c] + s[c] : s[c];
        }
    }
}

__device__ __forceinline__ unsigned short bf16_bits_rne(float v) {
    return __builtin_bit_cast(unsigned short, (__bf16)v);
}

__global__ __launch_bounds__(256) void split3_kernel(const float* __restrict__ src, int64_t ld_src, int cols,
                                                     unsigned short* __restrict__ planes, int64_t ld_pl,
                                                     int64_t plane_stride, int mask_upper, int row_g0, int col_g0,
                                                     int64_t bs_src, int64_t bs_planes) {
    if (blockIdx.z) {
        src += (size_t)blockIdx.z * bs_src;
        planes += (size_t)blockIdx.z * bs_planes;
    }
    const int c4 = (blockIdx.x * 256 + threadIdx.x) * 4;
    const int r = blockIdx.y;
    if (c4 >= cols) return;
    f32x4 v = *(const f32x4*)(src + (size_t)r * ld_src + c4);
    typedef __attribute__((ext_vector_type(4))) unsigned short u16x4;
    u16x4 hi, mid, lo;
#pragma unroll
    for (int e = 0; e < 4; ++e) {
        float x = v[e];
        if (mask_upper && col_g0 + c4 + e > row_g0 + r) x = 0.0f;
        const unsigned short h = bf16_bits_rne(x);
        const float r1 = x - qt_bf16_to_f32(h);
        const unsigned short m = bf16_bits_rne(r1);
        const float r2 = r1 - qt_bf16_to_f32(m);
        hi[e] = h;
        mid[e] = m;
        lo[e] = bf16_bits_rne(r2);
    }
    unsigned short* dst = planes + (size_t)r * ld_pl + c4;
    *(u16x4*)dst = hi;
    *(u16x4*)(dst + plane_stride) = mid;
    *(u16x4*)(dst + 2 * plane_stride) = lo;
}

__global__ __launch_bounds__(256) void split2h_kernel(const float* __restrict__ src, int64_t ld_src, int cols,
                                                      unsigned short* __restrict__ planes, int64_t ld_pl,
                                                      int64_t plane_stride, int mask_upper, int row_g0, int col_g0,
                                                      int64_t bs_src, int64_t bs_planes, const int32_t* __restrict__ e) {
    const int ex = e[blockIdx.z];
    if (blockIdx.z) {
        src += (size_t)blockIdx.z * bs_src;
        planes += (size_t)blockIdx.z * bs_planes;
    }
    const int c4 = (blockIdx.x * 256 + threadIdx.x) * 4;
    const int r = blockIdx.y;
    if (c4 >= cols) return;
    const float scale = __builtin_bit_cast(float, (unsigned)(127 + (ex < -G3_E_MAX ? -G3_E_MAX : ex > G3_E_MAX ? G3_E_MAX : ex)) << 23);
    f32x4 v = *(const f32x4*)(src + (size_t)r * ld_src + c4);
    typedef __attribute__((ext_vector_type(4))) unsigned short u16x4;
    u16x4 hi, lo;
#pragma unroll
    for (int q = 0; q < 4; ++q) {
        float x = v[q] * scale;
        if (mask_upper && col_g0 + c4 + q > row_g0 + r) x = 0.0f;
        const _Float16 h = (_Float16)x;
        const float r1 = x - (float)h;
        hi[q] = __builtin_bit_cast(unsigned short, h);
        lo[q] = __builtin_bit_cast(unsigned short, (_Float16)(r1 * 2048.0f));
    }
    unsigned short* dst = planes + (size_t)r * ld_pl + c4;
    *(u16x4*)dst = hi;
    *(u16x4*)(dst + plane_stride) = lo;
}

}

int qt_gemm3_launch(const G3Args& a, hipStream_t stream) {
    if (a.n_items <= 0) return QT_OK;
    QT_CHECK_ARG(a.ld % 8 == 0 && a.colmax >= 8, "qt_gemm3_launch: plane pitch %lld must be a multiple of 8", (long long)a.ld);
    QT_CHECK_ARG(((uintptr_t)a.Apl & 15) == 0 && ((uintptr_t)a.Bpl & 15) == 0 && (a.plane_stride % 8) == 0,
                 "qt_gemm3_launch: planes must be 16-byte aligned");
    QT_CHECK_ARG((uint64_t)a.ld * 2 * UT + (uint64_t)a.colmax * 2 < ((uint64_t)1 << 32), "qt_gemm3_launch: pitch too large");
    G3Params p;
    p.Apl = (const char*)a.Apl;
    p.Bpl = (const char*)a.Bpl;
    p.plane_bytes = a.plane_stride * 2;
    p.ld2 = a.ld * 2;
    p.plane_bytesB = (a.plane_strideB ? a.plane_strideB : a.plane_stride) * 2;
    p.ld2B = (a.ldB ? a.ldB : a.ld) * 2;
    p.colmaxB = a.colmaxB ? a.colmaxB : a.colmax;
    QT_CHECK_ARG(p.ld2B % 16 == 0 && p.colmaxB >= 8 && (p.plane_bytesB % 16) == 0 &&
                     (uint64_t)p.ld2B * UT + (uint64_t)p.colmaxB * 2 < ((uint64_t)1 << 32),
                 "qt_gemm3_launch: B-side pitch %lld / columns %d unsupported", (long long)(p.ld2B / 2), p.colmaxB);
    p.rowA0 = a.rowA0;
    p.rowB0 = a.rowB0;
    p.colA0 = a.colA0;
    p.colB0 = a.colB0;
    p.colmax = a.colmax;
    p.M = a.M;
    p.N = a.N;
    p.C = a.C;
    p.ldc = a.ldc;
    p.slabs = a.slabs;
    p.items = a.items;
    const int nb = a.batch > 1 ? a.batch : 1;
    QT_CHECK_ARG(nb <= 65535 && (a.bsApl % 8) == 0 && (a.bsBpl % 8) == 0, "qt_gemm3_launch: batch %d / plane strides unsupported", nb);
    p.bsA_bytes = a.bsApl * 2;
    p.bsB_bytes = a.bsBpl * 2;
    p.bsC = a.bsC;
    p.bsSlabs = a.bsSlabs;
    QT_CHECK_ARG(a.planes == G3_BF16X3 || (a.planes == G3_F16X2 && a.eA && a.eB),
                 "qt_gemm3_launch: plane mode %d needs its scale exponents", a.planes);
    p.eA = a.eA;
    p.eB = a.eB;
    const bool two = a.Bpl1 != nullptr;
    QT_CHECK_ARG(!two || (((uintptr_t)a.Bpl1 & 15) == 0 && a.C1 && a.N1 > 0 && (a.planes != G3_F16X2 || a.eB1) &&
                          a.mode1 >= G3_SUB && a.mode1 <= G3_ADD),
                 "qt_gemm3_launch: second segment incomplete");
    p.Bpl1 = two ? (const char*)a.Bpl1 : p.Bpl;
    p.eB1 = two ? a.eB1 : a.eB;
    p.C1 = two ? a.C1 : a.C;
    p.ldc1 = two ? a.ldc1 : a.ldc;
    p.bsC1 = two ? a.bsC1 : a.bsC;
    p.colB01 = two ? a.colB01 : a.colB0;
    p.N1 = two ? a.N1 : a.N;
    p.mode1 = two ? a.mode1 : a.mode;
    const dim3 grid(a.n_items, nb);
    const char* loop_env = getenv("QT_G3_LOOP");
    const bool chunk_loop = loop_env && strcmp(loop_env, "chunk") == 0;
    auto launch = [&](auto loop_c) {
        constexpr int LOOP = decltype(loop_c)::value;
        if (a.mode == G3_SUB) hipLaunchKernelGGL((gemm3_kernel<G3_SUB, LOOP>), grid, dim3(NTHREADS), 0, stream, p);
        else if (a.mode == G3_ADD) hipLaunchKernelGGL((gemm3_kernel<G3_ADD, LOOP>), grid, dim3(NTHREADS), 0, stream, p);
        else hipLaunchKernelGGL((gemm3_kernel<G3_SET, LOOP>), grid, dim3(NTHREADS), 0, stream, p);
    };
    if (a.planes == G3_F16X2) launch(std::integral_constant<int, LOOP_DUO>{});
    else if (chunk_loop) launch(std::integral_constant<int, LOOP_CHUNK>{});
    else launch(std::integral_constant<int, LOOP_TRI>{});
    QT_LAUNCH_CHECK();
    if (a.n_red > 0) {
        hipLaunchKernelGGL(gemm3_reduce_kernel, dim3(a.n_red, 16, nb), dim3(256), 0, stream, (const float*)a.slabs, a.red,
                           a.C, a.ldc, a.M, a.N, a.mode, a.bsSlabs, a.bsC, p.C1, p.ldc1, p.N1, p.mode1, p.bsC1);
        QT_LAUNCH_CHECK();
    }
    return QT_OK;
}

int qt_split3_launch(const float* src, int64_t ld_src, int rows, int cols, unsigned short* planes, int64_t ld_pl,
                     int64_t plane_stride, int mask_upper, int row_g0, int col_g0, hipStream_t stream, int batch,
                     int64_t bs_src, int64_t bs_planes) {
    if (rows <= 0 || cols <= 0) return QT_OK;
    QT_CHECK_ARG(cols % 4 == 0 && ld_src % 4 == 0 && ld_pl % 4 == 0 && plane_stride % 4 == 0 &&
                     ((uintptr_t)src & 15) == 0 && ((uintptr_t)planes & 7) == 0,
                 "qt_split3_launch: columns / pitches must be multiples of 4 and the pointers aligned");
    QT_CHECK_ARG(bs_src % 4 == 0 && bs_planes % 4 == 0, "qt_split3_launch: batch strides must be multiples of 4");
    hipLaunchKernelGGL(split3_kernel, dim3((cols / 4 + 255) / 256, rows, batch > 1 ? batch : 1), dim3(256), 0, stream, src,
                       ld_src, cols, planes, ld_pl, plane_stride, mask_upper, row_g0, col_g0, bs_src, bs_planes);
    QT_LAUNCH_CHECK();
    return QT_OK;
}

int qt_split2h_launch(const float* src, int64_t ld_src, int rows, int cols, unsigned short* planes, int64_t ld_pl,
                      int64_t plane_stride, int mask_upper, int row_g0, int col_g0, const int32_t* e, hipStream_t stream,
                      int batch, int64_t bs_src, int64_t bs_planes) {
    if (rows <= 0 || cols <= 0) return QT_OK;
    QT_CHECK_ARG(e && cols % 4 == 0 && ld_src % 4 == 0 && ld_pl % 4 == 0 && plane_stride % 4 == 0 &&
                     ((uintptr_t)src & 15) == 0 && ((uintptr_t)planes & 7) == 0,
                 "qt_split2h_launch: columns / pitches must be multiples of 4 and the pointers aligned");
    QT_CHECK_ARG(bs_src % 4 == 0 && bs_planes % 4 == 0, "qt_split2h_launch: batch strides must be multiples of 4");
    hipLaunchKernelGGL(split2h_kernel, dim3((cols / 4 + 255) / 256, rows, batch > 1 ? batch : 1), dim3(256), 0, stream, src,
                       ld_src, cols, planes, ld_pl, plane_stride, mask_upper, row_g0, col_g0, bs_src, bs_planes, e);
    QT_LAUNCH_CHECK();
    return QT_OK;
}

long g3_row_chunks(int Tm, int Tn, int c_end, int tri) {
    constexpr int TRI_STEP = 256 / G3_CHUNK_ROWS;
    long total = 0;
    for (int tj = 0; tj < Tn; ++tj) total += (long)Tm * std::max(0, c_end - (tri ? TRI_STEP * tj : 0));
    return total;
}

namespace {
struct G3PlanTile {
    int tile, lo, seg;
};
void g3_deal_xcds(std::vector<G3Item>& items);
void g3_plan_tiles(const std::vector<G3PlanTile>& tiles, int c_end, std::vector<G3Item>& items, std::vector<G3Red>& red,
                   int target_items, int max_slabs) {
    items.clear();
    red.clear();
    long total = 0;
    for (const G3PlanTile& t : tiles) total += std::max(0, c_end - t.lo);
    const int cap = target_items > 0 && target_items < NUM_CU ? target_items : NUM_CU;
    auto count_items = [&](int per, long& n_slabs) {
        long n_items = 0;
        n_slabs = 0;
        for (const G3PlanTile& t : tiles) {
            const int n = c_end - t.lo;
            if (n <= 0) continue;
            const int pieces = (n + per - 1) / per;
            n_items += pieces;
            if (pieces > 1) n_slabs += pieces;
        }
        return n_items;
    };
    int per = std::max(2, (int)((total + cap - 1) / cap));
    long n_slabs = 0;
    while ((count_items(per, n_slabs) > cap || (max_slabs > 0 && n_slabs > max_slabs)) && per < c_end) ++per;
    int next_slab = 0;
    for (const G3PlanTile& t : tiles) {
        const int lo = t.lo, n = c_end - lo;
        if (n <= 0) continue;
        const int pieces = (n + per - 1) / per;
        if (pieces == 1) {
            items.push_back({t.tile, lo, c_end, -1});
            continue;
        }
        red.push_back({t.tile & ~G3_SEG_BIT, next_slab, pieces, t.seg});
        for (int s = 0; s < pieces; ++s) {
            const int a = lo + (int)((long)n * s / pieces), b = lo + (int)((long)n * (s + 1) / pieces);
            items.push_back({t.tile, a, b, next_slab++});
        }
    }
    g3_deal_xcds(items);
}
}

void g3_plan_row(int Tm, int Tn, int c_end, int tri, std::vector<G3Item>& items, std::vector<G3Red>& red, int target_items) {
    constexpr int TRI_STEP = 256 / G3_CHUNK_ROWS;
    std::vector<G3PlanTile> tiles;
    for (int ti = 0; ti < Tm; ++ti)
        for (int tj = 0; tj < Tn; ++tj) tiles.push_back({(ti << 16) | tj, tri ? TRI_STEP * tj : 0, 0});
    g3_plan_tiles(tiles, c_end, items, red, target_items, 0);
}

void g3_plan_row2(int Tm, int Tn0, int Tn1, int c_end, std::vector<G3Item>& items, std::vector<G3Red>& red, int target_items,
                  int max_slabs) {
    constexpr int TRI_STEP = 256 / G3_CHUNK_ROWS;
    std::vector<G3PlanTile> tiles;
    for (int ti = 0; ti < Tm; ++ti)
        for (int tj = 0; tj < Tn0; ++tj) tiles.push_back({(ti << 16) | tj, 0, 0});
    for (int ti = 0; ti < Tm; ++ti)
        for (int tj = 0; tj < Tn1; ++tj) tiles.push_back({(ti << 16) | G3_SEG_BIT | tj, TRI_STEP * tj, 1});
    g3_plan_tiles(tiles, c_end, items, red, target_items, max_slabs);
}

namespace {
void g3_deal_xcds(std::vector<G3Item>& items) {
    std::stable_sort(items.begin(), items.end(),
                     [](const G3Item& x, const G3Item& y) { return (x.c_hi - x.c_lo) > (y.c_hi - y.c_lo); });
    static const bool deal = [] { const char* e = getenv("QT_G3_DEAL"); return !(e && atoi(e) == 0); }();
    if (deal && items.size() > 8) {
        std::vector<int> starts;
        for (const G3Item& it : items) starts.push_back(it.c_lo);
        std::sort(starts.begin(), starts.end());
        starts.erase(std::unique(starts.begin(), starts.end()), starts.end());
        const int P = (int)starts.size();
        const int g = P >= 8 ? 1 : 8 / P;
        std::vector<std::vector<G3Item>> cls(8);
        for (const G3Item& it : items) {
            const int rank = (int)(std::lower_bound(starts.begin(), starts.end(), it.c_lo) - starts.begin());
            const int tj = it.tile & 0xFFFF;
            cls[(rank * g + (g > 1 ? tj % g : 0)) % 8].push_back(it);
        }
        std::vector<G3Item> dealt;
        dealt.reserve(items.size());
        for (size_t q = 0; dealt.size() < items.size(); ++q)
            for (int x = 0; x < 8; ++x)
                if (q < cls[x].size()) dealt.push_back(cls[x][q]);
        items.swap(dealt);
    }
}
}

int g3_scale_exponent(float bound) {
    if (!(bound > 0.0f) || bound > 3.0e38f) return 0;
    int x;
    const float m = frexpf(bound, &x);
    const int ceil_log2 = m == 0.5f ? x - 1 : x;
    const int e = 3 - ceil_log2;
    return e < -G3_E_MAX ? -G3_E_MAX : e > G3_E_MAX ? G3_E_MAX : e;
}

constexpr size_t G3_TEST_TABLE_BYTES = (size_t)1 << 20;
constexpr size_t G3_TEST_SLACK = 1024;
static size_t g3_test_layout(int M, int N, int k, int64_t& ldp, size_t& planes_bytes, size_t& slabs_bytes) {
    ldp = (int64_t)qt_align_up((size_t)std::max(M, N), 256);
    planes_bytes = (size_t)3 * k * ldp * 2;
    slabs_bytes = (size_t)2 * NUM_CU * BT * BT * 4;
    return 2 * planes_bytes + slabs_bytes + G3_TEST_TABLE_BYTES + G3_TEST_SLACK;
}

extern "C" size_t qt_gemm3_tn_f32_workspace_bytes(int M, int N, int k) {
    if (M <= 0 || N <= 0 || k <= 0) return 0;
    int64_t ldp;
    size_t pb, sb;
    return g3_test_layout(M, N, k, ldp, pb, sb);
}

static int g3_test_run(const char* who, const float* A, int64_t lda, const float* B, int64_t ldb, float* C, int64_t ldc,
                       int M, int N, int k, int kind, int tri, int tight, int batch, int64_t bsA, int64_t bsB, int64_t bsC,
                       void* workspace, size_t workspace_bytes, hipStream_t stream, const float* bound_a = nullptr,
                       const float* bound_b = nullptr) {
    const bool f16x2 = bound_a && bound_b;
    constexpr size_t EXP_BYTES = 256;
    QT_CHECK_ARG(!f16x2 || batch <= 32, "%s: at most 32 problems with bounds", who);
    QT_CHECK_ARG(A && B && C && M > 0 && N > 0 && k > 0 && k % 128 == 0, "%s: k=%d must be a positive multiple of 128", who, k);
    QT_CHECK_ARG(M % 4 == 0 && N % 4 == 0 && lda % 4 == 0 && ldb % 4 == 0, "%s: M, N, lda, ldb must be multiples of 4", who);
    QT_CHECK_ARG(batch >= 1 && bsA % 4 == 0 && bsB % 4 == 0, "%s: batch %d / strides unsupported", who, batch);
    int64_t ldp;
    size_t pb, sb;
    const size_t need = g3_test_layout(M, N, k, ldp, pb, sb);
    if (!workspace || workspace_bytes < need * (size_t)batch) {
        qt_set_error("%s: workspace %zu < required %zu", who, workspace_bytes, need * (size_t)batch);
        return QT_ERR_WORKSPACE;
    }
    const size_t per = need - G3_TEST_SLACK;
    if (tight) ldp = (int64_t)qt_align_up((size_t)std::max(M, N), 8);
    const int64_t plane_stride = (int64_t)k * ldp;
    char* ws = (char*)qt_align_up((size_t)workspace, 256);
    unsigned short* Apl = (unsigned short*)ws;
    unsigned short* Bpl = (unsigned short*)(ws + pb);
    float* slabs = (float*)(ws + 2 * pb);
    char* tab = ws + 2 * pb + sb;
    int32_t* exps = (int32_t*)(tab + G3_TEST_TABLE_BYTES - EXP_BYTES);
    if (f16x2) {
        int32_t host_e[64] = {0};
        for (int b = 0; b < batch; ++b) {
            QT_CHECK_ARG(bound_a[b] > 0.0f && bound_b[b] > 0.0f, "%s: bounds must be positive", who);
            host_e[b] = g3_scale_exponent(bound_a[b]);
            host_e[32 + b] = g3_scale_exponent(bound_b[b]);
        }
        QT_HIP(hipStreamSynchronize(stream));
        QT_HIP(hipMemcpy(exps, host_e, sizeof(host_e), hipMemcpyHostToDevice));
    }
    for (int b = 0; b < batch; ++b) QT_HIP(hipMemsetAsync(ws + (size_t)b * per, 0, 2 * pb, stream));
    int rc = f16x2 ? qt_split2h_launch(A, lda, k, M, Apl, ldp, plane_stride, 0, 0, 0, exps, stream, batch, bsA, (int64_t)(per / 2))
                   : qt_split3_launch(A, lda, k, M, Apl, ldp, plane_stride, 0, 0, 0, stream, batch, bsA, (int64_t)(per / 2));
    if (rc) return rc;
    rc = f16x2 ? qt_split2h_launch(B, ldb, k, N, Bpl, ldp, plane_stride, 0, 0, 0, exps + 32, stream, batch, bsB, (int64_t)(per / 2))
               : qt_split3_launch(B, ldb, k, N, Bpl, ldp, plane_stride, 0, 0, 0, stream, batch, bsB, (int64_t)(per / 2));
    if (rc) return rc;
    const int Tm = (M + BT - 1) / BT, Tn = (N + BT - 1) / BT, nch = k / CH_ROWS;
    constexpr int TRI_STEP = 256 / G3_CHUNK_ROWS;
    QT_CHECK_ARG(!tri || TRI_STEP * (Tn - 1) < nch, "%s: tri needs k > 256 * (tile columns - 1)", who);
    std::vector<G3Item> items;
    std::vector<G3Red> red;
    if (kind == 0) {
        for (int ti = 0; ti < Tm; ++ti)
            for (int tj = 0; tj < Tn; ++tj) items.push_back({(ti << 16) | tj, tri ? TRI_STEP * tj : 0, nch, -1});
    } else {
        int next = 0;
        for (int ti = 0; ti < Tm; ++ti)
            for (int tj = 0; tj < Tn; ++tj) {
                const int lo = tri ? TRI_STEP * tj : 0, n = nch - lo;
                const int pieces = std::min(n / 2, std::max(1, 2 * NUM_CU / (Tm * Tn)));
                red.push_back({(ti << 16) | tj, next, pieces, 0});
                for (int s = 0; s < pieces; ++s)
                    items.push_back({(ti << 16) | tj, lo + (int)((long)n * s / pieces), lo + (int)((long)n * (s + 1) / pieces), next++});
            }
        QT_CHECK_ARG((size_t)next * BT * BT * 4 <= sb, "%s: too many tiles for the test face", who);
    }
    const size_t ib = items.size() * sizeof(G3Item), rb = red.size() * sizeof(G3Red);
    QT_CHECK_ARG(qt_align_up(ib, 256) + rb <= G3_TEST_TABLE_BYTES - EXP_BYTES, "%s: table too large for the test face", who);
    QT_HIP(hipStreamSynchronize(stream));
    QT_HIP(hipMemcpy(tab, items.data(), ib, hipMemcpyHostToDevice));
    if (rb) QT_HIP(hipMemcpy(tab + qt_align_up(ib, 256), red.data(), rb, hipMemcpyHostToDevice));
    G3Args g;
    g.Apl = Apl;
    g.Bpl = Bpl;
    g.plane_stride = plane_stride;
    g.ld = ldp;
    g.rowA0 = g.rowB0 = 0;
    g.colA0 = g.colB0 = 0;
    g.colmax = (int)ldp;
    g.M = M;
    g.N = N;
    g.C = C;
    g.ldc = ldc;
    g.mode = kind == 0 ? G3_SUB : G3_SET;
    g.slabs = slabs;
    g.items = (const G3Item*)tab;
    g.n_items = (int)items.size();
    g.red = (const G3Red*)(tab + qt_align_up(ib, 256));
    g.n_red = (int)red.size();
    g.batch = batch;
    g.bsApl = g.bsBpl = (int64_t)(per / 2);
    g.bsC = bsC;
    g.bsSlabs = (int64_t)(per / 4);
    if (f16x2) {
        g.planes = G3_F16X2;
        g.eA = exps;
        g.eB = exps + 32;
    }
    return qt_gemm3_launch(g, stream);
}

extern "C" int qt_gemm3_tn_f32(const float* A, int64_t lda, const float* B, int64_t ldb, float* C, int64_t ldc, int M,
                               int N, int k, int kind, void* workspace, size_t workspace_bytes, qt_stream_t stream_) {
    return g3_test_run("qt_gemm3_tn_f32", A, lda, B, ldb, C, ldc, M, N, k, kind, 0, 0, 1, 0, 0, 0, workspace, workspace_bytes,
                       (hipStream_t)stream_);
}

extern "C" int qt_gemm3_tn_f32_ex(const float* A, int64_t lda, const float* B, int64_t ldb, float* C, int64_t ldc, int M,
                                  int N, int k, int kind, int tri, int tight, int batch, int64_t bsA, int64_t bsB,
                                  int64_t bsC, void* workspace, size_t workspace_bytes, qt_stream_t stream_) {
    return g3_test_run("qt_gemm3_tn_f32_ex", A, lda, B, ldb, C, ldc, M, N, k, kind, tri, tight, batch, bsA, bsB, bsC, workspace,
                       workspace_bytes, (hipStream_t)stream_);
}

extern "C" int qt_gemm3_tn_f16x2(const float* A, int64_t lda, const float* B, int64_t ldb, float* C, int64_t ldc, int M,
                                 int N, int k, int kind, int tri, int tight, int batch, int64_t bsA, int64_t bsB,
                                 int64_t bsC, const float* bound_a, const float* bound_b, void* workspace,
                                 size_t workspace_bytes, qt_stream_t stream_) {
    QT_CHECK_ARG(bound_a && bound_b, "qt_gemm3_tn_f16x2: bounds are required");
    return g3_test_run("qt_gemm3_tn_f16x2", A, lda, B, ldb, C, ldc, M, N, k, kind, tri, tight, batch, bsA, bsB, bsC, workspace,
                       workspace_bytes, (hipStream_t)stream_, bound_a, bound_b);
}

constexpr int XF_CHUNK = 8192;

static int64_t xf_pitch(int K) { return (int64_t)qt_align_up((size_t)K, 256); }

extern "C" size_t qt_xtx_accumulate_f32_workspace_bytes(int64_t n_tokens, int K) {
    if (n_tokens <= 0 || K <= 0) return 0;
    const int nt = (K + BT - 1) / BT;
    return (size_t)3 * XF_CHUNK * xf_pitch(K) * 2 + qt_align_up((size_t)nt * (nt + 1) / 2 * sizeof(G3Item), 256) * 2 + 1024;
}

extern "C" int qt_xtx_accumulate_f32(const float* X, int64_t n_tokens, int K, int64_t ldx, float* G, void* workspace,
                                     size_t workspace_bytes, qt_stream_t stream_) {
    hipStream_t stream = (hipStream_t)stream_;
    QT_CHECK_ARG(X && G && K > 0 && n_tokens >= 0 && ldx >= K, "qt_xtx_accumulate_f32: bad arguments");
    QT_CHECK_ARG(K % 4 == 0 && ldx % 4 == 0 && ((uintptr_t)X & 15) == 0,
                 "qt_xtx_accumulate_f32: K, ldx must be multiples of 4 and X 16-byte aligned (K=%d)", K);
    if (n_tokens == 0) return QT_OK;
    const size_t need = qt_xtx_accumulate_f32_workspace_bytes(n_tokens, K);
    if (!workspace || workspace_bytes < need) {
        qt_set_error("qt_xtx_accumulate_f32: workspace %zu < required %zu", workspace_bytes, need);
        return QT_ERR_WORKSPACE;
    }
    const int64_t ldp = xf_pitch(K);
    const int64_t plane_stride = (int64_t)XF_CHUNK * ldp;
    char* ws = (char*)qt_align_up((size_t)workspace, 256);
    unsigned short* planes = (unsigned short*)ws;
    const size_t planes_bytes = (size_t)3 * XF_CHUNK * ldp * 2;
    char* tab = ws + planes_bytes;
    const int nt = (K + BT - 1) / BT;
    const size_t tab_bytes = qt_align_up((size_t)nt * (nt + 1) / 2 * sizeof(G3Item), 256);
    static std::mutex m;
    static std::map<std::pair<int, int>, G3Item*> tabs;
    auto table = [&](int nch) -> const G3Item* {
        std::lock_guard<std::mutex> lock(m);
        auto key = std::make_pair(K, nch);
        auto it = tabs.find(key);
        if (it != tabs.end()) return it->second;
        G3Item* pinned = nullptr;
        if (hipHostMalloc((void**)&pinned, tab_bytes, hipHostMallocDefault) != hipSuccess) return nullptr;
        int n = 0;
        for (int ti = 0; ti < nt; ++ti)
            for (int tj = 0; tj <= ti; ++tj) pinned[n++] = {(ti << 16) | tj, 0, nch, -1};
        tabs[key] = pinned;
        return pinned;
    };
    if (ldp != K) QT_HIP(hipMemsetAsync(planes, 0, planes_bytes, stream));
    int slot = 0;
    for (int64_t t0 = 0; t0 < n_tokens; t0 += XF_CHUNK) {
        const int rows = (int)std::min<int64_t>(XF_CHUNK, n_tokens - t0);
        const int rows_pad = (rows + 127) / 128 * 128;
        if (rows_pad != rows) {
            for (int q = 0; q < 3; ++q)
                QT_HIP(hipMemsetAsync(planes + q * plane_stride + (size_t)rows * ldp, 0, (size_t)(rows_pad - rows) * ldp * 2,
                                      stream));
        }
        int rc = qt_split3_launch(X + (size_t)t0 * ldx, ldx, rows, K, planes, ldp, plane_stride, 0, 0, 0, stream);
        if (rc) return rc;
        const int nch = rows_pad / CH_ROWS;
        const G3Item* host_tab = table(nch);
        if (!host_tab) {
            qt_set_error("qt_xtx_accumulate_f32: hipHostMalloc failed");
            return QT_ERR_HIP;
        }
        char* dev_tab = tab + (size_t)(slot & 1) * tab_bytes;
        ++slot;
        QT_HIP(hipMemcpyAsync(dev_tab, host_tab, (size_t)nt * (nt + 1) / 2 * sizeof(G3Item), hipMemcpyHostToDevice, stream));
        G3Args g;
        g.Apl = planes;
        g.Bpl = planes;
        g.plane_stride = plane_stride;
        g.ld = ldp;
        g.rowA0 = g.rowB0 = 0;
        g.colA0 = g.colB0 = 0;
        g.colmax = (int)ldp;
        g.M = K;
        g.N = K;
        g.C = G;
        g.ldc = K;
        g.mode = G3_ADD;
        g.slabs = nullptr;
        g.items = (const G3Item*)dev_tab;
        g.n_items = nt * (nt + 1) / 2;
        g.red = nullptr;
        g.n_red = 0;
        rc = qt_gemm3_launch(g, stream);
        if (rc) return rc;
    }
    return QT_OK;
}

extern "C" int qt_gemm3_plan_check(int Tm, int Tn, int c_end, int tri, int* n_items_out, int* n_slabs_out,
                                   int* longest_out) {
    if (Tm <= 0 || Tn <= 0 || c_end <= 0) return -1;
    std::vector<G3Item> items;
    std::vector<G3Red> red;
    g3_plan_row(Tm, Tn, c_end, tri, items, red);
    const int step = 256 / G3_CHUNK_ROWS;
    std::vector<int> cover((size_t)Tm * Tn * c_end, 0);
    std::vector<int> slab_seen;
    int longest = 0, n_slabs = 0;
    for (const G3Item& it : items) {
        const int ti = it.tile >> 16, tj = it.tile & 0xFFFF;
        if (ti >= Tm || tj >= Tn || it.c_lo >= it.c_hi || it.c_hi > c_end) return -2;
        const int lo = tri ? step * tj : 0;
        if (it.c_lo < lo) return -3;
        for (int c = it.c_lo; c < it.c_hi; ++c) cover[((size_t)ti * Tn + tj) * c_end + c]++;
        longest = std::max(longest, it.c_hi - it.c_lo);
        if (it.slab < 0) {
            if (it.c_lo != lo || it.c_hi != c_end) return -4;
        } else {
            if ((int)slab_seen.size() <= it.slab) slab_seen.resize(it.slab + 1, 0);
            if (slab_seen[it.slab]++) return -5;
            n_slabs = std::max(n_slabs, it.slab + 1);
        }
    }
    for (int ti = 0; ti < Tm; ++ti)
        for (int tj = 0; tj < Tn; ++tj)
            for (int c = 0; c < c_end; ++c) {
                const int want = (c >= (tri ? step * tj : 0)) ? 1 : 0;
                if (cover[((size_t)ti * Tn + tj) * c_end + c] != want) return -6;
            }
    std::vector<int> in_red(n_slabs, 0);
    for (const G3Red& r : red) {
        if (r.count < 2 || r.first < 0 || r.first + r.count > n_slabs) return -7;
        for (int q = 0; q < r.count; ++q)
            if (in_red[r.first + q]++) return -8;
        int prev_hi = -1;
        for (int q = 0; q < r.count; ++q) {
            bool found = false;
            for (const G3Item& it : items)
                if (it.slab == r.first + q) {
                    if (it.tile != r.tile || (prev_hi >= 0 && it.c_lo != prev_hi)) return -9;
                    prev_hi = it.c_hi;
                    found = true;
                }
            if (!found) return -10;
        }
    }
    for (int q = 0; q < n_slabs; ++q)
        if (!in_red[q]) return -11;
    long tiles = 0;
    for (int tj = 0; tj < Tn; ++tj) tiles += (c_end > (tri ? step * tj : 0)) ? Tm : 0;
    if (tiles <= NUM_CU && (long)items.size() > NUM_CU) return -12;
    if (n_items_out) *n_items_out = (int)items.size();
    if (n_slabs_out) *n_slabs_out = n_slabs;
    if (longest_out) *longest_out = longest;
    return 0;
}
```

quantool_amd/csrc/sgemm_tn.hip:

```cpp
#include <stdlib.h>

#include <type_traits>

#include "ring_pipe.h"
#include "sgemm_ring.h"
#include "sgemm_tn.h"

namespace {

constexpr int BK = 16;

#ifndef QT_SGEMM_PD
#define QT_SGEMM_PD 2
#endif

template <int N, class F>
__device__ __forceinline__ void sg_static_for(F&& f) {
    if constexpr (N > 0) {
        sg_static_for<N - 1>(f);
        f(std::integral_constant<int, N - 1>{});
    }
}

template <int BM, int BN, int MODE, bool CHAIN = false, int NWAVE = 4>
__global__ __launch_bounds__(64 * NWAVE) __attribute__((amdgpu_waves_per_eu(NWAVE == 8 ? 4 : 2))) void sgemm_tn_kernel(const SgemmArgs p) {
    constexpr int NT = 64 * NWAVE;
    constexpr int WGM = NWAVE == 8 ? 4 : 2, WGN = 2;
    constexpr int WM = BM / (32 * WGM), WN = BN / (32 * WGN);
    constexpr int A4 = BK * BM / 4 / NT;
    constexpr int B4 = BK * BN / 4 / NT;
    static_assert(A4 >= 1 && B4 >= 1, "tile too small for the workgroup");
    __shared__ __attribute__((aligned(16))) float As[2][BK][BM];
    __shared__ __attribute__((aligned(16))) float Bs[2][BK][BN];

    const int tid = threadIdx.x, lane = tid & 63, wave = tid >> 6;
    const int wave_m = wave >> 1, wave_n = wave & 1;
    const int m0 = blockIdx.y * BM, n0 = blockIdx.x * BN;
    if (p.upper_only && m0 >= n0 + BN) return;
    const float* Ap = p.A;
    const float* Bp = p.B;
    const float* Cinp = p.Cin;
    float* Coutp = p.Cout;
    int zsplit = blockIdx.z;
    if (p.batch > 1) {
        const int b = zsplit / p.n_splits;
        zsplit -= b * p.n_splits;
        Ap += (size_t)b * p.bsA;
        Bp += (size_t)b * p.bsB;
        if (Cinp) Cinp += (size_t)b * p.bsCin;
        Coutp += (size_t)b * p.bsCout;
    }
    if (p.n_groups > 0) {
        int g = 0;
        while (g + 1 < p.n_groups && m0 >= p.group_m_end[g]) ++g;
        Bp += (size_t)g * p.group_bsB;
    }
    const bool tile_inside = p.fast_interior && m0 + BM <= p.M && n0 + BN <= p.N;

    int k_begin = 0;
    if (p.k_mode == SG_K_FROM_N0) k_begin = n0 / BK * BK;
    int k_end = p.kdim;
    if (p.k_chunk > 0) {
        const int lo = zsplit * p.k_chunk, hi = lo + p.k_chunk;
        k_begin = k_begin > lo ? k_begin : lo;
        k_end = k_end < hi ? k_end : hi;
        Coutp += (size_t)zsplit * (size_t)p.M * (size_t)p.N;
    }

    const bool a_vec = (p.lda % 4 == 0) && (((uintptr_t)Ap & 15) == 0);
    const bool b_vec = (p.ldb % 4 == 0) && (((uintptr_t)Bp & 15) == 0);

    constexpr int PD = (BM == 64 && BN == 64 && !CHAIN) ? QT_SGEMM_PD : 1;
    static_assert(PD == 1 || PD % 2 == 0, "the LDS buffer of a step is s & 1: the unrolled ring must be even");
    f32x4 ra[PD][A4], rb[PD][B4];

    const bool interior = p.fast_interior && a_vec && b_vec && m0 + BM <= p.M && n0 + BN <= p.N;
    auto gload_fast = [&](int k0, auto slot_c) {
        constexpr int slot = decltype(slot_c)::value;
#pragma unroll
        for (int r = 0; r < A4; ++r) {
            const int idx = tid + NT * r;
            ra[slot][r] = *(const f32x4*)(Ap + (size_t)(k0 + idx / (BM / 4)) * p.lda + m0 + (idx % (BM / 4)) * 4);
        }
#pragma unroll
        for (int r = 0; r < B4; ++r) {
            const int idx = tid + NT * r;
            rb[slot][r] = *(const f32x4*)(Bp + (size_t)(k0 + idx / (BN / 4)) * p.ldb + n0 + (idx % (BN / 4)) * 4);
        }
    };
    auto gload = [&](int k0, auto slot_c) {
        constexpr int slot = decltype(slot_c)::value;
        if (interior && k0 + BK <= k_end) {
            gload_fast(k0, slot_c);
            return;
        }
#pragma unroll
        for (int r = 0; r < A4; ++r) {
            const int idx = tid + NT * r;
            const int kr = idx / (BM / 4), c = (idx % (BM / 4)) * 4;
            const int k = k0 + kr, m = m0 + c;
            f32x4 v = {0.f, 0.f, 0.f, 0.f};
            if (k < k_end) {
                const float* src = Ap + (size_t)k * p.lda + m;
                if (a_vec && m + 3 < p.M) {
                    v = *(const f32x4*)src;
                } else {
#pragma unroll
                    for (int e = 0; e < 4; ++e)
                        if (m + e < p.M) v[e] = src[e];
                }
            }
            ra[slot][r] = v;
        }
#pragma unroll
        for (int r = 0; r < B4; ++r) {
            const int idx = tid + NT * r;
            const int kr = idx / (BN / 4), c = (idx % (BN / 4)) * 4;
            const int k = k0 + kr, n = n0 + c;
            f32x4 v = {0.f, 0.f, 0.f, 0.f};
            if (k < k_end) {
                const float* src = Bp + (size_t)k * p.ldb + n;
                if (b_vec && n + 3 < p.N) {
                    v = *(const f32x4*)src;
                } else {
#pragma unroll
                    for (int e = 0; e < 4; ++e)
                        if (n + e < p.N) v[e] = src[e];
                }
            }
            rb[slot][r] = v;
        }
    };
    auto lstore = [&](int buf, auto slot_c) {
        constexpr int slot = decltype(slot_c)::value;
#pragma unroll
        for (int r = 0; r < A4; ++r) {
            const int idx = tid + NT * r;
            *(f32x4*)&As[buf][idx / (BM / 4)][(idx % (BM / 4)) * 4] = ra[slot][r];
        }
#pragma unroll
        for (int r = 0; r < B4; ++r) {
            const int idx = tid + NT * r;
            *(f32x4*)&Bs[buf][idx / (BN / 4)][(idx % (BN / 4)) * 4] = rb[slot][r];
        }
    };

    f32x16 acc[WM][WN];
#pragma unroll
    for (int i = 0; i < WM; ++i)
#pragma unroll
        for (int j = 0; j < WN; ++j)
#pragma unroll
            for (int r = 0; r < 16; ++r) acc[i][j][r] = 0.0f;

    const int h = lane >> 5, l31 = lane & 31;
    f32x16 cpre[WM][WN];
    if (MODE == SG_MODE_SUB) {
#pragma unroll
        for (int i = 0; i < WM; ++i)
#pragma unroll
            for (int j = 0; j < WN; ++j)
#pragma unroll
                for (int r = 0; r < 16; ++r) {
                    const int row = m0 + wave_m * (BM / WGM) + i * 32 + (r & 3) + 8 * (r >> 2) + 4 * h;
                    const int col = n0 + wave_n * (BN / WGN) + j * 32 + l31;
                    cpre[i][j][r] = (tile_inside || (row < p.M && col < p.N)) ? Cinp[(size_t)row * p.ldcin + col] : 0.0f;
                }
    }
    const int nsteps = (k_end - k_begin + BK - 1) / BK;
    auto kstep = [&](int s, auto u_c, auto fast_c) {
        constexpr int u = decltype(u_c)::value;
        constexpr bool FAST = decltype(fast_c)::value;
        const int buf = s & 1;
        if constexpr (FAST) {
            const int sn = s + PD < nsteps ? s + PD : nsteps - 1;
            gload_fast(k_begin + sn * BK, std::integral_constant<int, u>{});
        } else {
            if (s + PD < nsteps) gload(k_begin + (s + PD) * BK, std::integral_constant<int, u>{});
        }
#pragma unroll
        for (int kk = 0; kk < BK / 2; ++kk) {
                float a[WM], b[WN];
#pragma unroll
                for (int i = 0; i < WM; ++i) a[i] = As[buf][2 * kk + h][wave_m * (BM / WGM) + i * 32 + l31];
#pragma unroll
                for (int j = 0; j < WN; ++j) b[j] = Bs[buf][2 * kk + h][wave_n * (BN / WGN) + j * 32 + l31];
#pragma unroll
                for (int i = 0; i < WM; ++i)
#pragma unroll
                    for (int j = 0; j < WN; ++j)
                        acc[i][j] = __builtin_amdgcn_mfma_f32_32x32x2f32(a[i], b[j], acc[i][j], 0, 0, 0);
            }
        if (FAST || s + 1 < nsteps) lstore(buf ^ 1, std::integral_constant<int, (u + 1) % PD>{});
        if (CHAIN && s + 1 < nsteps && ((s + 1) * BK) % p.chain_len == 0) {
#pragma unroll
            for (int i = 0; i < WM; ++i)
#pragma unroll
                for (int j = 0; j < WN; ++j) {
#pragma unroll
                    for (int r = 0; r < 16; ++r) {
                        cpre[i][j][r] = cpre[i][j][r] - acc[i][j][r];
                        acc[i][j][r] = 0.0f;
                    }
                    __builtin_amdgcn_sched_barrier(0);
                }
        }
        __syncthreads();
    };
    using I0 = std::integral_constant<int, 0>;
    if (PD > 1 && interior && nsteps > 0 && nsteps % PD == 0 && (k_end - k_begin) % BK == 0) {
        sg_static_for<PD>([&](auto d) { gload_fast(k_begin + decltype(d)::value * BK, d); });
        lstore(0, I0{});
        __syncthreads();
        for (int s0 = 0; s0 < nsteps; s0 += PD)
            sg_static_for<PD>([&](auto u) { kstep(s0 + decltype(u)::value, u, std::true_type{}); });
    } else if (nsteps > 0) {
        sg_static_for<PD>([&](auto d) {
            if (decltype(d)::value < nsteps) gload(k_begin + decltype(d)::value * BK, d);
        });
        lstore(0, I0{});
        __syncthreads();
        for (int s0 = 0; s0 < nsteps; s0 += PD)
            sg_static_for<PD>([&](auto u) {
                if (s0 + decltype(u)::value < nsteps) kstep(s0 + decltype(u)::value, u, std::false_type{});
            });
    }

#pragma unroll
    for (int i = 0; i < WM; ++i)
#pragma unroll
        for (int j = 0; j < WN; ++j)
#pragma unroll
            for (int r = 0; r < 16; ++r) {
                const int row = m0 + wave_m * (BM / WGM) + i * 32 + (r & 3) + 8 * (r >> 2) + 4 * h;
                const int col = n0 + wave_n * (BN / WGN) + j * 32 + l31;
                if (tile_inside || (row < p.M && col < p.N)) {
                    float v = acc[i][j][r];
                    if (MODE == SG_MODE_SUB) v = cpre[i][j][r] - v;
                    if (MODE == SG_MODE_NEG) v = -v;
                    Coutp[(size_t)row * p.ldcout + col] = v;
                }
            }
}

__global__ __launch_bounds__(512) __attribute__((amdgpu_waves_per_eu(4, 4))) void sgemm_ring_kernel(RingArgs p) {
    __shared__ __attribute__((aligned(16))) char ring[RING_LDS_BYTES];
    sgemm_ring_body<false>(p, ring, 0);
}

__global__ __launch_bounds__(256) void splitk_reduce_kernel(const float* __restrict__ slabs, int splits, int M,
                                                            int N, const float* __restrict__ Cin, int64_t ldcin,
                                                            float* __restrict__ Cout, int64_t ldcout, int mode,
                                                            int64_t bs_slabs, int64_t bs_cin, int64_t bs_cout) {
    const int col = (blockIdx.x * blockDim.x + threadIdx.x) * 4;
    const int row = blockIdx.y;
    if (col >= N) return;
    if (blockIdx.z) {
        slabs += (size_t)blockIdx.z * bs_slabs;
        if (Cin) Cin += (size_t)blockIdx.z * bs_cin;
        Cout += (size_t)blockIdx.z * bs_cout;
    }
    const size_t mn = (size_t)M * N;
    if (col + 3 < N && (N & 3) == 0) {
        f32x4 s = {0.f, 0.f, 0.f, 0.f};
        const float* src = slabs + (size_t)row * N + col;
        int z = 0;
        for (; z + 8 <= splits; z += 8) {
            f32x4 v[8];
#pragma unroll
            for (int u = 0; u < 8; ++u) v[u] = *(const f32x4*)(src + (size_t)(z + u) * mn);
#pragma unroll
            for (int u = 0; u < 8; ++u) s += v[u];
        }
        for (; z < splits; ++z) s += *(const f32x4*)(src + (size_t)z * mn);
#pragma unroll
        for (int e = 0; e < 4; ++e) {
            float v = s[e];
            if (mode == SG_MODE_SUB) v = Cin[(size_t)row * ldcin + col + e] - v;
            if (mode == SG_MODE_NEG) v = -v;
            Cout[(size_t)row * ldcout + col + e] = v;
        }
    } else {
        for (int e = 0; e < 4 && col + e < N; ++e) {
            float v = 0.f;
            for (int z = 0; z < splits; ++z) v += slabs[z * mn + (size_t)row * N + col + e];
            if (mode == SG_MODE_SUB) v = Cin[(size_t)row * ldcin + col + e] - v;
            if (mode == SG_MODE_NEG) v = -v;
            Cout[(size_t)row * ldcout + col + e] = v;
        }
    }
}

template <int BM, int BN>
int launch(const SgemmArgs& a, hipStream_t stream, int splits = 1) {
    dim3 grid((a.N + BN - 1) / BN, (a.M + BM - 1) / BM, splits * (a.batch > 1 ? a.batch : 1));
    static const bool sub8 = [] {
        const char* e = getenv("QT_SGEMM_SUB_WAVES");
        return !(e && atoi(e) == 4);
    }();
    switch (a.mode) {
        case SG_MODE_SUB:
            if constexpr (BM == 128 && BN == 128) {
                if (sub8) {
                    if (a.chain_len > 0)
                        hipLaunchKernelGGL((sgemm_tn_kernel<BM, BN, SG_MODE_SUB, true, 8>), grid, dim3(512), 0, stream, a);
                    else
                        hipLaunchKernelGGL((sgemm_tn_kernel<BM, BN, SG_MODE_SUB, false, 8>), grid, dim3(512), 0, stream, a);
                    break;
                }
            }
            if (a.chain_len > 0)
                hipLaunchKernelGGL((sgemm_tn_kernel<BM, BN, SG_MODE_SUB, true>), grid, dim3(256), 0, stream, a);
            else
                hipLaunchKernelGGL((sgemm_tn_kernel<BM, BN, SG_MODE_SUB>), grid, dim3(256), 0, stream, a);
            break;
        case SG_MODE_SET:
            hipLaunchKernelGGL((sgemm_tn_kernel<BM, BN, SG_MODE_SET>), grid, dim3(256), 0, stream, a);
            break;
        default:
            hipLaunchKernelGGL((sgemm_tn_kernel<BM, BN, SG_MODE_NEG>), grid, dim3(256), 0, stream, a);
            break;
    }
    QT_LAUNCH_CHECK();
    return QT_OK;
}

}

int qt_splitk_reduce(const float* slabs, int splits, int M, int N, const float* Cin, int64_t ldcin, float* Cout,
                     int64_t ldcout, int mode, hipStream_t stream, int batch, int64_t bs_slabs, int64_t bs_cin,
                     int64_t bs_cout) {
    hipLaunchKernelGGL(splitk_reduce_kernel, dim3((N / 4 + 255) / 256 + 1, M, batch > 1 ? batch : 1), dim3(256), 0, stream,
                       slabs, splits, M, N, Cin, ldcin, Cout, ldcout, mode, bs_slabs, bs_cin, bs_cout);
    QT_LAUNCH_CHECK();
    return QT_OK;
}

int qt_sgemm_tn(const SgemmArgs& a_, hipStream_t stream) {
    if (a_.M <= 0 || a_.N <= 0) return QT_OK;
    QT_CHECK_ARG(a_.batch >= 1 && a_.batch <= SG_MAX_BATCH && a_.n_groups >= 0 && a_.n_groups <= SG_MAX_GROUPS &&
                     !(a_.batch > 1 && a_.n_groups > 0),
                 "qt_sgemm_tn: batch %d / row groups %d unsupported", a_.batch, a_.n_groups);
    for (int g = 0; g < a_.n_groups; ++g)
        QT_CHECK_ARG((a_.group_m_end[g] % 128 == 0 || g == a_.n_groups - 1) && (g == 0 || a_.group_m_end[g] >= a_.group_m_end[g - 1]),
                     "qt_sgemm_tn: row group %d ends at %d (boundaries must be ascending multiples of 128)", g, a_.group_m_end[g]);
    static const int fast_interior = [] {
        const char* e = getenv("QT_SGEMM_INTERIOR");
        return (e && atoi(e) == 0) ? 0 : 1;
    }();
    SgemmArgs a = a_;
    a.fast_interior = fast_interior;
    const long t128 = (long)((a.M + 127) / 128) * ((a.N + 127) / 128);
    if (a.split_ws && t128 < 384 && a.kdim >= 512) {
        static const int target_wgs = [] {
            const char* e = getenv("QT_SGEMM_SPLIT_TARGET");
            const int v = e ? atoi(e) : 256;
            return v < 256 ? 256 : v;
        }();
        static const int min_chunk = [] {
            const char* e = getenv("QT_SGEMM_SPLIT_MIN_CHUNK");
            const int v = e ? atoi(e) : 128;
            return v < 64 ? 64 : v;
        }();
        int splits = (int)(target_wgs / t128);
        if (splits > 32) splits = 32;
        if (splits < 1) splits = 1;
        int chunk = (a.kdim + splits - 1) / splits;
        chunk = (chunk + 63) / 64 * 64;
        if (chunk < min_chunk) chunk = min_chunk;
        splits = (a.kdim + chunk - 1) / chunk;
        const size_t need = (size_t)splits * a.M * a.N * sizeof(float);
        if (splits >= 2 && need <= a.split_ws_bytes && (a.batch <= 1 || (size_t)a.bs_split * sizeof(float) >= need)) {
            SgemmArgs part = a;
            part.Cin = nullptr;
            part.ldcin = 0;
            part.Cout = a.split_ws;
            part.ldcout = a.N;
            part.bsCin = 0;
            part.bsCout = a.bs_split;
            part.mode = SG_MODE_SET;
            part.k_chunk = chunk;
            part.n_splits = splits;
            const int rc = launch<128, 128>(part, stream, splits);
            if (rc) return rc;
            return qt_splitk_reduce(a.split_ws, splits, a.M, a.N, a.Cin, a.ldcin, a.Cout, a.ldcout, a.mode, stream, a.batch,
                                    a.bs_split, a.bsCin, a.bsCout);
        }
    }
    const char* ring_env = getenv("QT_SGEMM_RING");
    const int use_ring = (ring_env && atoi(ring_env) == 0) ? 0 : 1;
    const char* ring_min_env = getenv("QT_SGEMM_RING_MIN_TILES");
    const int ring_min_tiles = ring_min_env ? atoi(ring_min_env) : 32;
    if (use_ring && sgemm_ring_applies(a)) {
        const RingArgs r = sgemm_ring_args(a);
        if (r.n_tiles >= ring_min_tiles) {
            const int all = r.n_tiles * r.batch;
            const int grid = all >= 2 * 256 ? 2 * 256 : all;
            hipLaunchKernelGGL(sgemm_ring_kernel, dim3(grid), dim3(512), 0, stream, r);
            QT_LAUNCH_CHECK();
            return QT_OK;
        }
    }
    if (t128 >= 384) return launch<128, 128>(a, stream);
    return launch<64, 64>(a, stream);
}

extern "C" size_t qt_sgemm_tn_f32_workspace_bytes(int M, int N) {
    if (M <= 0 || N <= 0) return 0;
    return (size_t)32 * M * N * 4 + 256;
}

extern "C" int qt_sgemm_tn_f32(const float* A, int64_t lda, const float* B, int64_t ldb, const float* Cin,
                               int64_t ldcin, float* Cout, int64_t ldcout, int M, int N, int kdim, int skip_zero_k,
                               int mode, int allow_split_k, void* workspace, size_t workspace_bytes,
                               qt_stream_t stream_) {
    hipStream_t stream = (hipStream_t)stream_;
    QT_CHECK_ARG(A && B && Cout && M > 0 && N > 0 && kdim >= 0, "qt_sgemm_tn_f32: bad arguments");
    QT_CHECK_ARG(mode == SG_MODE_SUB || mode == SG_MODE_SET || mode == SG_MODE_NEG, "qt_sgemm_tn_f32: mode %d", mode);
    QT_CHECK_ARG(mode != SG_MODE_SUB || Cin, "qt_sgemm_tn_f32: MODE_SUB needs Cin");
    SgemmArgs g;
    g.A = A; g.lda = lda;
    g.B = B; g.ldb = ldb;
    g.Cin = Cin; g.ldcin = ldcin;
    g.Cout = Cout; g.ldcout = ldcout;
    g.M = M; g.N = N; g.kdim = kdim;
    g.k_mode = skip_zero_k ? SG_K_FROM_N0 : SG_K_FULL;
    g.mode = mode;
    if (allow_split_k) {
        const size_t need = qt_sgemm_tn_f32_workspace_bytes(M, N);
        if (!workspace || workspace_bytes < need) {
            qt_set_error("qt_sgemm_tn_f32: workspace %zu < required %zu", workspace_bytes, need);
            return QT_ERR_WORKSPACE;
        }
        g.split_ws = (float*)qt_align_up((size_t)workspace, 256);
        g.split_ws_bytes = workspace_bytes - 256;
    }
    return qt_sgemm_tn(g, stream);
}
```

quantool_amd/hip/_lib.py:

```python
from __future__ import annotations

import ctypes
from ctypes import c_char_p, c_double, c_float, c_int, c_int32, c_int64, c_size_t, c_void_p
from pathlib import Path

_PKG = Path(__file__).resolve().parent.parent
LIB_PATH = _PKG / "lib" / "libquantool_hip.so"

QT_OK = 0
QT_ERR_INVALID = -1
QT_ERR_NOT_PD = -2
QT_ERR_WORKSPACE = -3
QT_ERR_HIP = -4
QT_ERR_UNSUPPORTED = -5

QT_F32, QT_BF16, QT_F16 = 0, 1, 2
QT_W_INT8, QT_W_INT4_PACKED = 0, 1

SIGNATURES = {
    "qt_version": (c_int, []),
    "qt_last_error": (c_char_p, []),
    "qt_xtx_workspace_bytes": (c_size_t, [c_int64, c_int]),
    "qt_xtx_accumulate": (c_int, [c_void_p, c_int, c_int64, c_int, c_int64, c_void_p, c_void_p, c_size_t, c_void_p]),
    "qt_xtx_accumulate_f32_workspace_bytes": (c_size_t, [c_int64, c_int]),
    "qt_xtx_accumulate_f32": (c_int, [c_void_p, c_int64, c_int, c_int64, c_void_p, c_void_p, c_size_t, c_void_p]),
    "qt_act_stats_workspace_bytes": (c_size_t, [c_int64, c_int]),
    "qt_act_stats_accumulate": (c_int, [c_void_p, c_int, c_int64, c_int, c_int64, c_void_p, c_void_p, c_void_p,
                                        c_void_p, c_size_t, c_void_p]),
    "qt_hessian_prepare_workspace_bytes": (c_size_t, [c_int]),
    "qt_hessian_prepare": (c_int, [c_void_p, c_int, c_int64, c_float, c_void_p, c_void_p, c_void_p, c_void_p,
                                   c_void_p, c_size_t, c_void_p]),
    "qt_hessian_prepare_damp": (c_int, [c_void_p, c_int, c_int64, c_float, c_void_p, c_void_p, c_void_p, c_void_p,
                                        c_void_p, c_void_p, c_size_t, c_void_p]),
    "qt_hessian_diag": (c_int, [c_void_p, c_int, c_int64, c_void_p, c_void_p]),
    "qt_argsort_desc": (c_int, [c_void_p, c_int, c_void_p, c_void_p, c_void_p]),
    "qt_cholesky_inverse_upper_workspace_bytes": (c_size_t, [c_int]),
    "qt_cholesky_inverse_upper": (c_int, [c_void_p, c_int, c_void_p, c_void_p, c_void_p, c_size_t, c_void_p]),
    "qt_cholesky_inverse_upper_batched_workspace_bytes": (c_size_t, [c_int, c_int]),
    "qt_cholesky_inverse_upper_batched": (c_int, [c_void_p, c_int64, c_int, c_void_p, c_int64, c_void_p, c_int, c_void_p,
                                                  c_size_t, c_void_p]),
    "qt_cholesky_inverse_upper_bounded": (c_int, [c_void_p, c_int, c_void_p, c_void_p, c_void_p, c_void_p, c_size_t,
                                                  c_void_p]),
    "qt_cholesky_inverse_upper_batched_bounded": (c_int, [c_void_p, c_int64, c_int, c_void_p, c_int64, c_void_p, c_int,
                                                          c_void_p, c_void_p, c_size_t, c_void_p]),
    "qt_group_minmax_qparams": (c_int, [c_void_p, c_int, c_int, c_int, c_int64, c_int, c_int, c_int, c_void_p,
                                        c_void_p, c_void_p, c_void_p, c_void_p]),
    "qt_weight_gather_f32": (c_int, [c_void_p, c_int, c_int, c_int, c_int64, c_void_p, c_void_p, c_void_p,
                                     c_void_p]),
    "qt_weight_gather_qparams": (c_int, [c_void_p, c_int, c_int, c_int, c_int64, c_void_p, c_void_p, c_int, c_int, c_int,
                                         c_void_p, c_void_p, c_void_p, c_void_p, c_void_p, c_int64, c_void_p]),
    "qt_gptq_sweep_workspace_bytes": (c_size_t, [c_int, c_int, c_int]),
    "qt_gptq_sweep": (c_int, [c_void_p, c_int, c_int, c_void_p, c_void_p, c_void_p, c_int, c_void_p, c_int, c_int,
                              c_void_p, c_void_p, c_void_p, c_size_t, c_void_p]),
    "qt_gptq_sweep_grouped": (c_int, [c_void_p, c_int, c_int, c_void_p, c_int64, c_int, c_void_p, c_void_p, c_void_p, c_int,
                                      c_void_p, c_int, c_int, c_void_p, c_void_p, c_void_p, c_size_t, c_void_p]),
    "qt_pack_int4": (c_int, [c_void_p, c_int, c_int, c_void_p, c_void_p, c_void_p]),
    "qt_awq_weight_mean_workspace_bytes": (c_size_t, [c_int, c_int]),
    "qt_awq_weight_mean_accumulate": (c_int, [c_void_p, c_int, c_int, c_int, c_int64, c_int, c_void_p, c_void_p,
                                              c_size_t, c_void_p]),
    "qt_awq_scales": (c_int, [c_void_p, c_int64, c_void_p, c_int64, c_int, c_int, c_int, c_void_p, c_void_p]),
    "qt_symmetrize_lower": (c_int, [c_void_p, c_int, c_void_p]),
    "qt_awq_loss_workspace_bytes": (c_size_t, [c_int, c_int]),
    "qt_awq_loss": (c_int, [c_void_p, c_int, c_int, c_int, c_int64, c_void_p, c_int, c_int, c_int, c_void_p, c_int64,
                            c_int, c_float, c_int, c_void_p, c_void_p, c_size_t, c_void_p]),
    "qt_awq_losses_workspace_bytes": (c_size_t, [c_int, c_int, c_int]),
    "qt_awq_losses": (c_int, [c_void_p, c_int, c_int, c_int, c_int64, c_void_p, c_int, c_int, c_int, c_int, c_void_p,
                              c_int64, c_float, c_int, c_void_p, c_void_p, c_size_t, c_void_p]),
    "qt_argmin_f32": (c_int, [c_void_p, c_int, c_void_p, c_void_p]),
    "qt_awq_pseudo_quantize": (c_int, [c_void_p, c_int, c_int, c_int, c_int64, c_void_p, c_int, c_int, c_int, c_void_p,
                                       c_int64, c_void_p]),
    "qt_scale_columns": (c_int, [c_void_p, c_int, c_int, c_int, c_int64, c_void_p, c_int, c_void_p, c_int64,
                                 c_void_p]),
    "qt_rtn_quantize": (c_int, [c_void_p, c_int, c_int, c_int, c_int64, c_void_p, c_void_p, c_int, c_int, c_int,
                                c_void_p, c_void_p]),
    "qt_col_absmax_workspace_bytes": (c_size_t, [c_int, c_int]),
    "qt_col_absmax_accumulate": (c_int, [c_void_p, c_int, c_int, c_int, c_int64, c_void_p, c_void_p, c_size_t,
                                         c_void_p]),
    "qt_smoothquant_scales": (c_int, [c_void_p, c_void_p, c_void_p, c_int, c_float, c_void_p, c_void_p]),
    "qt_xtx_dot_workspace_bytes": (c_size_t, [c_int64, c_int]),
    "qt_xtx_dot": (c_int, [c_void_p, c_int, c_int64, c_int, c_int64, c_void_p, c_double, c_void_p, c_int, c_void_p,
                           c_size_t, c_void_p]),
    "qt_gemm3_plan_check": (c_int, [c_int, c_int, c_int, c_int, c_void_p, c_void_p, c_void_p]),
    "qt_xtx_tile_table_check": (c_int, [c_int, c_void_p, c_void_p, c_void_p]),
    "qt_chol_g3_plan_check": (c_int, [c_int, c_int, c_int, c_void_p]),
    "qt_gemm3_tn_f32_workspace_bytes": (c_size_t, [c_int, c_int, c_int]),
    "qt_gemm3_tn_f32": (c_int, [c_void_p, c_int64, c_void_p, c_int64, c_void_p, c_int64, c_int, c_int, c_int, c_int,
                                c_void_p, c_size_t, c_void_p]),
    "qt_gemm3_tn_f32_ex": (c_int, [c_void_p, c_int64, c_void_p, c_int64, c_void_p, c_int64, c_int, c_int, c_int, c_int,
                                   c_int, c_int, c_int, c_int64, c_int64, c_int64, c_void_p, c_size_t, c_void_p]),
    "qt_gemm3_tn_f16x2": (c_int, [c_void_p, c_int64, c_void_p, c_int64, c_void_p, c_int64, c_int, c_int, c_int, c_int,
                                  c_int, c_int, c_int, c_int64, c_int64, c_int64, c_void_p, c_void_p, c_void_p, c_size_t,
                                  c_void_p]),
    "qt_sgemm_tn_f32_workspace_bytes": (c_size_t, [c_int, c_int]),
    "qt_sgemm_tn_f32": (c_int, [c_void_p, c_int64, c_void_p, c_int64, c_void_p, c_int64, c_void_p, c_int64, c_int,
                                c_int, c_int, c_int, c_int, c_int, c_void_p, c_size_t, c_void_p]),
    "qt_profile_enable": (c_int, [c_int]),
    "qt_profile_read": (c_int, [c_int, c_void_p, c_void_p]),
    "qt_dequantize": (c_int, [c_void_p, c_int, c_int, c_void_p, c_void_p, c_void_p, c_int, c_void_p, c_void_p,
                              c_int, c_int64, c_void_p]),
    "qt_quantize_tokens_i8": (c_int, [c_void_p, c_int, c_int64, c_int, c_int64, c_void_p, c_int, c_void_p, c_void_p,
                                      c_void_p, c_void_p]),
    "qt_act_mul_quantize_i8": (c_int, [c_void_p, c_int64, c_void_p, c_int64, c_int, c_int64, c_int, c_int, c_void_p,
                                       c_int, c_void_p, c_void_p, c_void_p, c_void_p, c_int64, c_void_p]),
    "qt_rmsnorm_quantize_i8": (c_int, [c_void_p, c_int64, c_void_p, c_int, c_int64, c_int, c_float, c_void_p, c_int,
                                       c_void_p, c_void_p, c_void_p, c_void_p, c_int64, c_void_p, c_void_p]),
    "qt_gemm_i8": (c_int, [c_void_p, c_int64, c_int, c_void_p, c_int, c_int, c_void_p, c_void_p, c_void_p, c_int,
                           c_void_p, c_void_p, c_void_p, c_int, c_int64, c_void_p]),
    "qt_gemm_i8_skinny": (c_int, [c_void_p, c_int, c_int, c_void_p, c_int, c_int, c_void_p, c_void_p, c_void_p, c_int,
                                  c_void_p, c_void_p, c_void_p, c_int, c_int64, c_void_p]),
    "qt_gemm_i8_ring": (c_int, [c_void_p, c_int64, c_int, c_void_p, c_int, c_int, c_void_p, c_void_p, c_void_p, c_int,
                                c_void_p, c_void_p, c_void_p, c_int, c_int64, c_void_p]),
    "qt_gemm_i8_ring_w4": (c_int, [c_void_p, c_int64, c_int, c_void_p, c_int, c_int, c_void_p, c_void_p, c_void_p,
                                   c_int, c_void_p, c_void_p, c_void_p, c_int, c_int64, c_void_p]),
    "qt_gemm_i8_mid": (c_int, [c_void_p, c_int64, c_int, c_void_p, c_int, c_int, c_void_p, c_void_p, c_void_p, c_int,
                               c_void_p, c_void_p, c_void_p, c_int, c_int64, c_void_p]),
    "qt_gemm_i8_skinny_grouped": (c_int, [c_void_p, c_int, c_void_p, c_int64, c_void_p, c_int, c_void_p, c_int, c_int,
                                          c_void_p, c_void_p, c_void_p, c_int, c_void_p, c_void_p, c_int, c_int64,
                                          c_void_p]),
    "qt_moe_route": (c_int, [c_void_p, c_int, c_int64, c_int, c_int, c_void_p, c_void_p, c_void_p, c_void_p,
                             c_void_p]),
    "qt_gemm_i8_grouped": (c_int, [c_void_p, c_int, c_void_p, c_int64, c_void_p, c_int, c_void_p, c_int, c_int,
                                   c_void_p, c_void_p, c_void_p, c_int, c_void_p, c_void_p, c_int, c_int64, c_void_p]),
    "qt_gemm_i8_ring_grouped": (c_int, [c_void_p, c_int, c_void_p, c_int64, c_void_p, c_int, c_void_p, c_int, c_int,
                                        c_void_p, c_void_p, c_void_p, c_int, c_void_p, c_void_p, c_int, c_int64,
                                        c_int64, c_void_p]),
    "qt_moe_gemm_i8_ring_w4": (c_int, [c_void_p, c_int, c_void_p, c_int64, c_void_p, c_int, c_void_p, c_int, c_int,
                                       c_void_p, c_void_p, c_void_p, c_int, c_void_p, c_void_p, c_int, c_int64,
                                       c_int64, c_void_p]),
    "qt_moe_gemm_i8_wide": (c_int, [c_void_p, c_int, c_void_p, c_int64, c_void_p, c_int, c_void_p, c_int, c_int,
                                    c_void_p, c_void_p, c_void_p, c_int, c_void_p, c_void_p, c_int, c_int64,
                                    c_int64, c_void_p]),
    "qt_moe_combine": (c_int, [c_void_p, c_int, c_int, c_int64, c_void_p, c_void_p, c_int64, c_int, c_void_p,
                               c_void_p]),
    "qt_dequantize_weight": (c_int, [c_void_p, c_int, c_int, c_int, c_void_p, c_int, c_void_p, c_void_p, c_void_p,
                                     c_int, c_int64, c_void_p]),
    "qt_gemm_wq_skinny": (c_int, [c_void_p, c_int, c_int, c_int, c_int64, c_void_p, c_int, c_int, c_void_p, c_int,
                                  c_void_p, c_void_p, c_void_p, c_void_p, c_int64, c_void_p]),
    "qt_gemm_wq_stream": (c_int, [c_void_p, c_int, c_int, c_int, c_int64, c_void_p, c_int, c_int, c_void_p, c_int,
                                  c_void_p, c_void_p, c_void_p, c_void_p, c_int64, c_void_p]),
    "qt_gemm_wq_grouped": (c_int, [c_void_p, c_int, c_int, c_int64, c_void_p, c_int64, c_void_p, c_int, c_void_p,
                                   c_int, c_int, c_void_p, c_int, c_void_p, c_void_p, c_void_p, c_int64, c_void_p]),
    "qt_moe_gemm_wq_wide": (c_int, [c_void_p, c_int, c_int, c_int64, c_void_p, c_int64, c_void_p, c_int, c_void_p,
                                    c_int, c_int, c_void_p, c_int, c_void_p, c_void_p, c_void_p, c_int64, c_int64,
                                    c_void_p]),
}

_lib = None


class HipBackendError(RuntimeError):

    def __init__(self, fn: str, status: int, message: str):
        super().__init__(f"{fn} failed with status {status}: {message}")
        self.status = status


def load() -> ctypes.CDLL:
    global _lib
    if _lib is not None:
        return _lib
    if not LIB_PATH.exists():
        raise ImportError(
            f"quantool_amd HIP library not found at {LIB_PATH}. Build it with "
            "`python -c 'import __graft_entry__ as g; g.build()'` (needs hipcc). "
            "There is no CPU fallback for the quantization path."
        )
    import torch

    lib = ctypes.CDLL(str(LIB_PATH))
    for name, (res, args) in SIGNATURES.items():
        fn = getattr(lib, name)
        fn.restype = res
        fn.argtypes = args
    _lib = lib
    return lib


def check(fn_name: str, status: int) -> None:
    if status != QT_OK:
        msg = load().qt_last_error()
        raise HipBackendError(fn_name, status, msg.decode() if msg else "")
```

Baseline: 3.287 billion.

## Fuse Cholesky inverse diagonal-step GEMMs and pair split launches to cut kernel count

Adds a fused yii_step_kernel that runs the per-step off-diagonal product, the multiply by the diagonal inverse, the Y write-back and the transpose into XT in one launch. It replaces the earlier sgemm-plus-transpose sequence. It also merges the R and Y plane-split launches into a single paired kernel when the merged schedule is active. A dry-run launch counter (qt_chol_launch_count) with a host-only plan path is added, and launch sites move to a QT_LAUNCH macro. The aim is fewer kernel launches and less launch overhead in the blocked Cholesky inverse. The cost is a more complex hand-written MFMA kernel, with a register-heavy ring of preloaded A values.

```diff
diff --git a/include/quantool_amd.h b/include/quantool_amd.h
--- a/include/quantool_amd.h
+++ b/include/quantool_amd.h
@@ -143,6 +143,7 @@
 
 int qt_gemm3_plan_check(int Tm, int Tn, int c_end, int tri, int* n_items_out, int* n_slabs_out, int* longest_out);
 int qt_chol_g3_plan_check(int K, int merged, int min_chunks, long long* counts_out);
+long long qt_chol_launch_count(int K, int merge_mode, int fuse, int bounded);
 enum qt_act { QT_ACT_SILU = 0 };
 #define QT_I8_MID_MAX_M 128
 #define QT_I8_MID_K_UNIT 128
diff --git a/quantool_amd/csrc/cholesky.hip b/quantool_amd/csrc/cholesky.hip
--- a/quantool_amd/csrc/cholesky.hip
+++ b/quantool_amd/csrc/cholesky.hip
@@ -119,19 +119,19 @@
     pl.blob_bytes = pl.any ? qt_align_up(bytes.size(), 256) : 0;
 }
 
-static const CholG3Plan* chol_g3_plan(int K, int NBO, int NBI, bool merged = false) {
+static const CholG3Plan* chol_g3_plan(int K, int NBO, int NBI, bool merged = false, bool host_only = false) {
     static std::mutex m;
     static std::map<std::tuple<int, int, int, int>, CholG3Plan*> plans;
     const int min_chunks = chol_g3_min_chunks();
     const int target_items = chol_g3_target_items(K);
     std::lock_guard<std::mutex> lock(m);
-    const auto key = std::make_tuple(K, NBO, NBI, (merged ? 1 << 30 : 0) + min_chunks * 1024 + target_items);
+    const auto key = std::make_tuple(K, host_only ? -NBO : NBO, NBI, (merged ? 1 << 30 : 0) + min_chunks * 1024 + target_items);
     auto it = plans.find(key);
     if (it != plans.end()) return it->second;
     CholG3Plan* pl = new CholG3Plan();
     std::vector<char> bytes;
     chol_g3_build(K, NBO, NBI, min_chunks, target_items, merged, *pl, bytes);
-    if (pl->any) {
+    if (pl->any && !host_only) {
         if (hipHostMalloc((void**)&pl->blob, pl->blob_bytes, hipHostMallocDefault) != hipSuccess) {
             pl->any = false;
             pl->blob = nullptr;
@@ -154,16 +154,25 @@
     return 2 * qt_align_up((size_t)3 * K * K * 2, 256) + (size_t)pl->max_slabs * 256 * 256 * 4 + pl->blob_bytes + 256;
 }
 
-static const CholG3Plan* chol_blocks(int K, int& NBO, int& NBI) {
+static const CholG3Plan* chol_blocks(int K, int& NBO, int& NBI, bool host_only = false) {
     const int eo = chol_block_env("QT_CHOL_NBO"), ei = chol_block_env("QT_CHOL_NBI");
     NBO = eo ? eo : 512;
     NBI = ei ? ei : 512;
-    const CholG3Plan* pl = chol_g3_plan(K, NBO, NBI);
+    const CholG3Plan* pl = chol_g3_plan(K, NBO, NBI, false, host_only);
     if (pl->any) return pl;
     NBO = eo ? eo : 256;
     NBI = ei ? ei : 256;
-    return chol_g3_plan(K, NBO, NBI);
-}
+    return chol_g3_plan(K, NBO, NBI, false, host_only);
+}
+
+static bool chol_fuse_on() {
+    const char* e = getenv("QT_CHOL_FUSE");
+    return !(e && atoi(e) == 0);
+}
+struct CholDry {
+    int merge_mode;
+    bool fuse, bounded;
+};
 
 constexpr int LDP = NB + 1;
 
@@ -541,6 +550,135 @@
         }
 }
 
+constexpr int YS_W = 32, YS_KS = 64, YS_RING = 4, YS_FILL = 16;
+constexpr int YS_NS_MAX = 6;
+template <int NS>
+__global__ __launch_bounds__(256) void yii_step_kernel(const float* __restrict__ Rc, int64_t lda, float* Yd, int64_t ldy,
+                                                       const float* __restrict__ Dinv_all, int blk, int nbi, int kd,
+                                                       float* __restrict__ XT, int ldx, int64_t bsA, int64_t bsY,
+                                                       int64_t bsW) {
+    if (blockIdx.y) {
+        Rc += (size_t)blockIdx.y * bsA;
+        Yd += (size_t)blockIdx.y * bsY;
+        Dinv_all += (size_t)blockIdx.y * bsW;
+        XT += (size_t)blockIdx.y * bsW;
+    }
+    __shared__ __attribute__((aligned(16))) float Bs[NS * YS_KS][YS_W];
+    __shared__ __attribute__((aligned(16))) float Ts[NB][YS_W];
+    const float* Di = Dinv_all + (size_t)blk * NB * NB;
+    const int tid = threadIdx.x, lane = tid & 63, wave = tid >> 6;
+    const int nstrips = kd / YS_W;
+    if ((int)blockIdx.x >= nstrips) {
+        const int t = ((int)blockIdx.x - nstrips) * 256 + tid;
+        const int width = kd + nbi, wq = (width + 3) / 4;
+#pragma unroll 4
+        for (int q = t; q < nbi * wq; q += YS_FILL * 256) {
+            const int c = q / wq, mm = (q - c * wq) * 4;
+            f32x4 v = {0.f, 0.f, 0.f, 0.f};
+            if (mm >= kd) v = *(const f32x4*)(Di + c * NB + (mm - kd));
+            float* dst = XT + (size_t)(kd + c) * ldx + mm;
+            if (mm + 3 < width) {
+                *(f32x4*)dst = v;
+            } else {
+#pragma unroll
+                for (int e = 0; e < 4; ++e)
+                    if (mm + e < width) dst[e] = v[e];
+            }
+        }
+        if (kd == NB) {
+            const float* D0 = Di - NB * NB;
+#pragma unroll 2
+            for (int q = t; q < NB * NB / 4; q += YS_FILL * 256)
+                *(f32x4*)(XT + (size_t)(q / (NB / 4)) * ldx + (q % (NB / 4)) * 4) = *(const f32x4*)(D0 + q * 4);
+        }
+        return;
+    }
+    const int l31 = lane & 31, h = lane >> 5;
+    const int n0 = blockIdx.x * YS_W;
+    const int m = wave * 32 + l31;
+    const bool m_ok = m < nbi;
+    const int mc = m_ok ? m : 0;
+    const int s_begin = n0 / 64;
+
+    float a[YS_RING][YS_KS / 2];
+#pragma unroll
+    for (int u = 0; u < YS_RING && u < NS; ++u)
+#pragma unroll
+        for (int q = 0; q < YS_KS / 2; ++q) a[u][q] = Rc[(size_t)(u * YS_KS + 2 * q + h) * lda + mc];
+    __builtin_amdgcn_sched_barrier(0);
+    f32x4 bv[NS * 2];
+    const bool y_vec = (ldy % 4 == 0) && (((uintptr_t)Yd & 15) == 0);
+#pragma unroll
+    for (int p = 0; p < NS * 2; ++p)
+        if (p >= 2 * s_begin) {
+            const float* src = Yd + (size_t)(p * 32 + (tid >> 3)) * ldy + n0 + (tid & 7) * 4;
+            if (y_vec) {
+                bv[p] = *(const f32x4*)src;
+            } else {
+#pragma unroll
+                for (int e = 0; e < 4; ++e) bv[p][e] = src[e];
+            }
+        }
+    __builtin_amdgcn_sched_barrier(0);
+#pragma unroll
+    for (int p = 0; p < NS * 2; ++p)
+        if (p >= 2 * s_begin) *(f32x4*)&Bs[p * 32 + (tid >> 3)][(tid & 7) * 4] = bv[p];
+    __syncthreads();
+    float d[NB / 2];
+#pragma unroll
+    for (int q = 0; q < NB / 2; ++q) d[q] = Di[(2 * q + h) * NB + m];
+    f32x16 acc;
+#pragma unroll
+    for (int r = 0; r < 16; ++r) acc[r] = 0.0f;
+#pragma unroll
+    for (int st = 0; st < NS; ++st) {
+        if (st >= s_begin) {
+#pragma unroll
+            for (int q = 0; q < YS_KS / 2; ++q)
+                acc = __builtin_amdgcn_mfma_f32_32x32x2f32(m_ok ? a[st % YS_RING][q] : 0.0f, Bs[st * YS_KS + 2 * q + h][l31], acc, 0, 0, 0);
+        }
+        if (st + YS_RING < NS) {
+#pragma unroll
+            for (int q = 0; q < YS_KS / 2; ++q)
+                a[st % YS_RING][q] = Rc[(size_t)((st + YS_RING) * YS_KS + 2 * q + h) * lda + mc];
+        }
+    }
+#pragma unroll
+    for (int r = 0; r < 16; ++r) Ts[wave * 32 + (r & 3) + 8 * (r >> 2) + 4 * h][l31] = acc[r];
+    __syncthreads();
+#pragma unroll
+    for (int r = 0; r < 16; ++r) acc[r] = 0.0f;
+#pragma unroll
+    for (int st = 0; st < NB / 16; ++st) {
+        if (st * 16 < nbi) {
+#pragma unroll
+            for (int q = st * 8; q < st * 8 + 8; ++q)
+                acc = __builtin_amdgcn_mfma_f32_32x32x2f32(d[q], Ts[2 * q + h][l31], acc, 0, 0, 0);
+        }
+    }
+    {
+        const int col = n0 + l31;
+#pragma unroll
+        for (int g = 0; g < 4; ++g) {
+            const int row = wave * 32 + 8 * g + 4 * h;
+            f32x4 v;
+#pragma unroll
+            for (int e = 0; e < 4; ++e) {
+                v[e] = -acc[4 * g + e];
+                if (row + e < nbi) Yd[(size_t)(kd + row + e) * ldy + col] = v[e];
+            }
+            float* xt = XT + (size_t)col * ldx + kd + row;
+            if (row + 3 < nbi) {
+                *(f32x4*)xt = v;
+            } else {
+#pragma unroll
+                for (int e = 0; e < 4; ++e)
+                    if (row + e < nbi) xt[e] = v[e];
+            }
+        }
+    }
+}
+
 __global__ __launch_bounds__(256) void transpose_lower_block_kernel(const float* __restrict__ Y, int64_t ldy, int w,
                                                                     float* __restrict__ XT, int ldx, int64_t bsY,
                                                                     int64_t bsXT) {
@@ -638,9 +776,9 @@
 }
 
 static int chol_run(float* A, int64_t strideA, int K, float* U, int64_t strideU, int32_t* info, int nprob, void* workspace,
-                    size_t workspace_bytes, hipStream_t stream, const float* min_eig_lb = nullptr) {
-    bool f16x2 = min_eig_lb != nullptr;
-    if (const char* e = getenv("QT_CHOL_PLANES")) {
+                    size_t workspace_bytes, hipStream_t stream, const float* min_eig_lb = nullptr, const CholDry* dry = nullptr) {
+    bool f16x2 = dry ? dry->bounded : min_eig_lb != nullptr;
+    if (const char* e = dry ? nullptr : getenv("QT_CHOL_PLANES")) {
         if (strcmp(e, "bf16x3") == 0) f16x2 = false;
         else if (strcmp(e, "f16x2") == 0) {
             QT_CHECK_ARG(min_eig_lb, "qt_cholesky_inverse_upper: QT_CHOL_PLANES=f16x2 needs a bound on lambda_min (the _bounded entry points)");
@@ -648,19 +786,21 @@
             QT_CHECK_ARG(false, "qt_cholesky_inverse_upper: QT_CHOL_PLANES=%s (bf16x3 | f16x2)", e);
         }
     }
-    const size_t need = qt_cholesky_inverse_upper_batched_workspace_bytes(K, nprob);
-    if (!workspace || workspace_bytes < need) {
+    const size_t need = dry ? 0 : qt_cholesky_inverse_upper_batched_workspace_bytes(K, nprob);
+    if (!dry && (!workspace || workspace_bytes < need)) {
         qt_set_error("qt_cholesky_inverse_upper: workspace %zu < required %zu", workspace_bytes, need);
         return QT_ERR_WORKSPACE;
     }
     const int nblk = (K + NB - 1) / NB;
     char* ws = (char*)qt_align_up((size_t)workspace, 256);
     int NBO, NBI;
-    const CholG3Plan* g3 = chol_blocks(K, NBO, NBI);
-    int merge_mode = (g3->any && NBO == NBI) ? chol_merge_mode() : CHOL_TWO_PHASE;
+    const CholG3Plan* g3 = chol_blocks(K, NBO, NBI, dry != nullptr);
+    int merge_mode = (g3->any && NBO == NBI) ? (dry ? dry->merge_mode : chol_merge_mode()) : CHOL_TWO_PHASE;
+    const bool fuse_on = dry ? dry->fuse : chol_fuse_on();
+    const bool fuse = fuse_on && NBI <= (YS_NS_MAX + 2) * YS_KS;
     const CholG3Plan* tab = g3;
     if (merge_mode == CHOL_WALK_MERGED) {
-        tab = chol_g3_plan(K, NBO, NBI, true);
+        tab = chol_g3_plan(K, NBO, NBI, true, dry != nullptr);
         if (!tab->any || !tab->any_row || tab->max_slabs > g3->max_slabs || tab->blob_bytes > g3->blob_bytes) {
             tab = g3;
             merge_mode = CHOL_TWO_PHASE;
@@ -688,7 +828,7 @@
         q += qt_align_up((size_t)3 * K * K * 2, 256);
         g3_slabs = (float*)q;
         g3_tab = (char*)qt_align_up((size_t)(ws + (size_t)nprob * prob_bytes), 256);
-        QT_HIP(hipMemcpyAsync(g3_tab, tab->blob, tab->blob_bytes, hipMemcpyHostToDevice, stream));
+        if (!dry) QT_HIP(hipMemcpyAsync(g3_tab, tab->blob, tab->blob_bytes, hipMemcpyHostToDevice, stream));
     }
     f16x2 = f16x2 && g3->any;
     int32_t* eR = f16x2 ? (int32_t*)(Rpl + 2 * plane_stride) : nullptr;
@@ -749,7 +889,7 @@
     const size_t inv_lds = (size_t)(NB * LDT + NB * LDP) * sizeof(float);
     const size_t potf2_lds = (size_t)(NB * LDA + 4 * 32 * 32) * sizeof(float);
     static QtOncePerDevice lds_attr;
-    QT_HIP(lds_attr.run([&] {
+    if (!dry) QT_HIP(lds_attr.run([&] {
         hipError_t e = hipFuncSetAttribute((const void*)potf2_kernel, hipFuncAttributeMaxDynamicSharedMemorySize,
                                            (int)potf2_lds);
         if (e == hipSuccess)
@@ -763,11 +903,10 @@
                                     (int)(RD_STRIDE * sizeof(float)));
         return e;
     }));
-    QT_HIP(hipMemsetAsync(info, 0, sizeof(int32_t) * nprob, stream));
+    if (!dry) QT_HIP(hipMemsetAsync(info, 0, sizeof(int32_t) * nprob, stream));
     const int prio = qt_chain_prio();
     if (f16x2) {
-        hipLaunchKernelGGL(chol_scales_kernel, dim3(nprob), dim3(256), 0, stream, (const float*)A, sA, K, min_eig_lb, eR, info);
-        QT_LAUNCH_CHECK();
+        QT_LAUNCH(chol_scales_kernel, dim3(nprob), dim3(256), 0, stream, (const float*)A, sA, K, min_eig_lb, eR, info);
     }
 
     auto fac_product = [&](int J0, int J1, int Jb) -> int {
@@ -784,6 +923,7 @@
         g.split_ws = split_ws; g.split_ws_bytes = split_ws_bytes;
         return sgemm(g, sA, sA, sA);
     };
+    const bool pair_copies = fuse_on && merge_mode != CHOL_TWO_PHASE;
     auto fac_panels = [&](int J0, int J1) -> int {
         for (int j0 = J0; j0 < J1; j0 += NB) {
             const int j = j0 / NB, nbj = (K - j0 < NB) ? K - j0 : NB;
@@ -798,20 +938,18 @@
                 int rc = sgemm(g, sA, sA, sA);
                 if (rc) return rc;
             }
-            hipLaunchKernelGGL(potf2_kernel, dim3(nprob), dim3(POTF2_THREADS), potf2_lds, stream, (const float*)Ajj, (int64_t)K, nbj,
-                               Ajj, (int64_t)K, Rd + (size_t)j * RD_STRIDE, info, j0, prio, sA, sW);
-            QT_LAUNCH_CHECK();
+            QT_LAUNCH(potf2_kernel, dim3(nprob), dim3(POTF2_THREADS), potf2_lds, stream, (const float*)Ajj, (int64_t)K, nbj,
+                      Ajj, (int64_t)K, Rd + (size_t)j * RD_STRIDE, info, j0, prio, sA, sW);
             const int rest = K - j0 - nbj;
             if (rest > 0) {
-                hipLaunchKernelGGL(trsm_rt_kernel, dim3((rest + 127) / 128, nprob), dim3(256), RD_STRIDE * sizeof(float),
-                                   stream, (const float*)(Rd + (size_t)j * RD_STRIDE), nbj, (const float*)(Ajj + nbj),
-                                   (int64_t)K, Ajj + nbj, (int64_t)K, rest, prio, sW, sA);
-                QT_LAUNCH_CHECK();
+                QT_LAUNCH(trsm_rt_kernel, dim3((rest + 127) / 128, nprob), dim3(256), RD_STRIDE * sizeof(float),
+                          stream, (const float*)(Rd + (size_t)j * RD_STRIDE), nbj, (const float*)(Ajj + nbj),
+                          (int64_t)K, Ajj + nbj, (int64_t)K, rest, prio, sW, sA);
             }
         }
         const int rem = K - J1;
         if (g3->any) {
-            if (rem > 0) {
+            if (rem > 0 && !pair_copies) {
                 int rc = f16x2 ? qt_split2h_launch(A + (size_t)J0 * K + J0, K, J1 - J0, K - J0, Rpl + (size_t)J0 * K + J0, K,
                                                    plane_stride, 0, 0, 0, eR, stream, nprob, sA, sW * 2)
                                : qt_split3_launch(A + (size_t)J0 * K + J0, K, J1 - J0, K - J0, Rpl + (size_t)J0 * K + J0, K,
@@ -834,12 +972,11 @@
     auto trinv = [&](int blk0, int n) -> int {
         const char* e = getenv("QT_CHOL_TRINV");
         if (e && strcmp(e, "div") == 0)
-            hipLaunchKernelGGL(trinv_batched_kernel, dim3(n, nprob), dim3(NB), inv_lds, stream, (const float*)Rd, K, Dinv, Y,
-                               (int64_t)K, sW, sY, blk0);
+            QT_LAUNCH(trinv_batched_kernel, dim3(n, nprob), dim3(NB), inv_lds, stream, (const float*)Rd, K, Dinv, Y,
+                      (int64_t)K, sW, sY, blk0);
         else
-            hipLaunchKernelGGL(trinv_mfma_kernel, dim3(n, nprob), dim3(256), RD_STRIDE * sizeof(float), stream,
-                               (const float*)Rd, K, Dinv, Y, (int64_t)K, sW, sY, blk0);
-        QT_LAUNCH_CHECK();
+            QT_LAUNCH(trinv_mfma_kernel, dim3(n, nprob), dim3(256), RD_STRIDE * sizeof(float), stream,
+                      (const float*)Rd, K, Dinv, Y, (int64_t)K, sW, sY, blk0);
         return QT_OK;
     };
     auto inv_product = [&](int I0, int I1, int Ib) -> int {
@@ -858,6 +995,17 @@
         const int Wi = I1 - I0;
         for (int i0 = I0 + NB; i0 < I1; i0 += NB) {
             const int i = i0 / NB, nbi = (K - i0 < NB) ? K - i0 : NB;
+            if (fuse) {
+                const dim3 grid((i0 - I0) / YS_W + YS_FILL, nprob);
+#define QT_YII_STEP(NS)                                                                                               \
+    QT_LAUNCH(yii_step_kernel<NS>, grid, dim3(256), 0, stream, (const float*)(A + (size_t)I0 * K + i0), (int64_t)K, \
+              Y + (size_t)I0 * K + I0, (int64_t)K, (const float*)Dinv, i, nbi, i0 - I0, XT, NBO_MAX, sA, sY, sW)
+                if (i0 - I0 == 128) QT_YII_STEP(2);
+                else if (i0 - I0 == 256) QT_YII_STEP(4);
+                else QT_YII_STEP(6);
+#undef QT_YII_STEP
+                continue;
+            }
             SgemmArgs g;
             g.A = A + (size_t)I0 * K + i0; g.lda = K;
             g.B = Y + (size_t)I0 * K + I0; g.ldb = K;
@@ -877,6 +1025,11 @@
         }
         auto split_row = [&]() -> int {
             if (!g3->any || I1 >= K) return QT_OK;
+            if (pair_copies) {
+                const G3SplitSrc dR = {A + (size_t)I0 * K + I0, K, Wi, K - I0, Rpl + (size_t)I0 * K + I0, K, 0, 0, 0, eR, sA, sW * 2};
+                const G3SplitSrc dY = {Y + (size_t)I0 * K, K, Wi, I1, Ypl + (size_t)I0 * K, K, 1, I0, 0, eY, sY, sW * 2};
+                return qt_split_pair_launch(dR, dY, plane_stride, f16x2, stream, nprob);
+            }
             if (f16x2)
                 return qt_split2h_launch(Y + (size_t)I0 * K, K, Wi, I1, Ypl + (size_t)I0 * K, K, plane_stride, 1, I0, 0, eY,
                                          stream, nprob, sY, sW * 2);
@@ -884,11 +1037,16 @@
                                     nprob, sY, sW * 2);
         };
         if (I0 == 0) return split_row();
-        hipLaunchKernelGGL(transpose_lower_block_kernel, dim3((Wi + 31) / 32, (Wi + 31) / 32, nprob), dim3(256), 0, stream,
-                           (const float*)(Y + (size_t)I0 * K + I0), (int64_t)K, Wi, XT, NBO_MAX, sY, sW);
-        QT_LAUNCH_CHECK();
         SgemmArgs t;
-        t.A = XT; t.lda = NBO_MAX;
+        if (!fuse) {
+            QT_LAUNCH(transpose_lower_block_kernel, dim3((Wi + 31) / 32, (Wi + 31) / 32, nprob), dim3(256), 0, stream,
+                      (const float*)(Y + (size_t)I0 * K + I0), (int64_t)K, Wi, XT, NBO_MAX, sY, sW);
+            t.A = XT; t.lda = NBO_MAX;
+        } else if (Wi > NB) {
+            t.A = XT; t.lda = NBO_MAX;
+        } else {
+            t.A = Dinv + (size_t)(I0 / NB) * NB * NB; t.lda = NB;
+        }
         t.B = TI; t.ldb = K;
         t.Cin = nullptr; t.ldcin = 0;
         t.Cout = Y + (size_t)I0 * K; t.ldcout = K;
@@ -928,11 +1086,9 @@
             if (rc) return rc;
         }
     }
-    hipLaunchKernelGGL(flat_reverse_lower_to_upper_kernel, dim3((K + 255) / 256, K, nprob), dim3(256), 0, stream, U, K, sU);
-    QT_LAUNCH_CHECK();
-    hipLaunchKernelGGL(identity_if_failed_kernel, dim3(K < 1024 ? K : 1024, 1, nprob), dim3(256), 0, stream, U, K,
-                       (const int32_t*)info, sU);
-    QT_LAUNCH_CHECK();
+    QT_LAUNCH(flat_reverse_lower_to_upper_kernel, dim3((K + 255) / 256, K, nprob), dim3(256), 0, stream, U, K, sU);
+    QT_LAUNCH(identity_if_failed_kernel, dim3(K < 1024 ? K : 1024, 1, nprob), dim3(256), 0, stream, U, K,
+              (const int32_t*)info, sU);
     return QT_OK;
 }
 
@@ -966,6 +1122,16 @@
     QT_CHECK_ARG(n_problems == 1 || (strideA >= (int64_t)K * K && strideU >= (int64_t)K * K && strideA % 4 == 0 && strideU % 4 == 0),
                  "qt_cholesky_inverse_upper_batched_bounded: strides must be multiples of 4 elements and >= K*K");
     return chol_run(A, strideA, K, U, strideU, info, n_problems, workspace, workspace_bytes, (hipStream_t)stream_, min_eig_lb);
+}
+
+extern "C" long long qt_chol_launch_count(int K, int merge_mode, int fuse, int bounded) {
+    if (K <= 0 || merge_mode < CHOL_TWO_PHASE || merge_mode > CHOL_WALK_MERGED) return -1;
+    const CholDry dry = {merge_mode, fuse != 0, bounded != 0};
+    long long n = 0;
+    qt_dry_launches = &n;
+    const int rc = chol_run(nullptr, 0, K, nullptr, 0, nullptr, 1, nullptr, 0, nullptr, nullptr, &dry);
+    qt_dry_launches = nullptr;
+    return rc == QT_OK ? n : -1;
 }
 
 extern "C" int qt_chol_g3_plan_check(int K, int merged, int min_chunks, long long* counts_out) {
diff --git a/quantool_amd/csrc/common.h b/quantool_amd/csrc/common.h
--- a/quantool_amd/csrc/common.h
+++ b/quantool_amd/csrc/common.h
@@ -46,6 +46,17 @@
             qt_set_error("kernel launch failed: %s (%s:%d)", hipGetErrorString(_e), \
                          __FILE__, __LINE__);                                     \
             return QT_ERR_HIP;                                                    \
+        }                                                                         \
+    } while (0)
+
+inline thread_local long long* qt_dry_launches = nullptr;
+#define QT_LAUNCH(kernel, grid, block, lds, stream, ...)                          \
+    do {                                                                          \
+        if (qt_dry_launches) {                                                    \
+            ++*qt_dry_launches;                                                   \
+        } else {                                                                  \
+            hipLaunchKernelGGL(kernel, grid, block, lds, stream, __VA_ARGS__);    \
+            QT_LAUNCH_CHECK();                                                    \
         }                                                                         \
     } while (0)
 
diff --git a/quantool_amd/csrc/gemm3_tn.h b/quantool_amd/csrc/gemm3_tn.h
--- a/quantool_amd/csrc/gemm3_tn.h
+++ b/quantool_amd/csrc/gemm3_tn.h
@@ -68,6 +68,17 @@
                       int64_t plane_stride, int mask_upper, int row_g0, int col_g0, const int32_t* e, hipStream_t stream,
                       int batch = 1, int64_t bs_src = 0, int64_t bs_planes = 0);
 
+struct G3SplitSrc {
+    const float* src; int64_t ld_src;
+    int rows, cols;
+    unsigned short* planes; int64_t ld_pl;
+    int mask_upper, row_g0, col_g0;
+    const int32_t* e;
+    int64_t bs_src, bs_planes;
+};
+int qt_split_pair_launch(const G3SplitSrc& d0, const G3SplitSrc& d1, int64_t plane_stride, bool f16x2, hipStream_t stream,
+                         int batch = 1);
+
 int g3_scale_exponent(float bound);
 
 long g3_row_chunks(int Tm, int Tn, int c_end, int tri);
diff --git a/quantool_amd/csrc/gemm3_tn.hip b/quantool_amd/csrc/gemm3_tn.hip
--- a/quantool_amd/csrc/gemm3_tn.hip
+++ b/quantool_amd/csrc/gemm3_tn.hip
@@ -374,19 +374,12 @@
     return __builtin_bit_cast(unsigned short, (__bf16)v);
 }
 
-__global__ __launch_bounds__(256) void split3_kernel(const float* __restrict__ src, int64_t ld_src, int cols,
-                                                     unsigned short* __restrict__ planes, int64_t ld_pl,
-                                                     int64_t plane_stride, int mask_upper, int row_g0, int col_g0,
-                                                     int64_t bs_src, int64_t bs_planes) {
-    if (blockIdx.z) {
-        src += (size_t)blockIdx.z * bs_src;
-        planes += (size_t)blockIdx.z * bs_planes;
-    }
-    const int c4 = (blockIdx.x * 256 + threadIdx.x) * 4;
-    const int r = blockIdx.y;
-    if (c4 >= cols) return;
+typedef __attribute__((ext_vector_type(4))) unsigned short u16x4;
+
+__device__ __forceinline__ void split3_quad(const float* __restrict__ src, int64_t ld_src, unsigned short* __restrict__ planes,
+                                            int64_t ld_pl, int64_t plane_stride, int mask_upper, int row_g0, int col_g0,
+                                            int r, int c4) {
     f32x4 v = *(const f32x4*)(src + (size_t)r * ld_src + c4);
-    typedef __attribute__((ext_vector_type(4))) unsigned short u16x4;
     u16x4 hi, mid, lo;
 #pragma unroll
     for (int e = 0; e < 4; ++e) {
@@ -406,6 +399,40 @@
     *(u16x4*)(dst + 2 * plane_stride) = lo;
 }
 
+__global__ __launch_bounds__(256) void split3_kernel(const float* __restrict__ src, int64_t ld_src, int cols,
+                                                     unsigned short* __restrict__ planes, int64_t ld_pl,
+                                                     int64_t plane_stride, int mask_upper, int row_g0, int col_g0,
+                                                     int64_t bs_src, int64_t bs_planes) {
+    if (blockIdx.z) {
+        src += (size_t)blockIdx.z * bs_src;
+        planes += (size_t)blockIdx.z * bs_planes;
+    }
+    const int c4 = (blockIdx.x * 256 + threadIdx.x) * 4;
+    const int r = blockIdx.y;
+    if (c4 >= cols) return;
+    split3_quad(src, ld_src, planes, ld_pl, plane_stride, mask_upper, row_g0, col_g0, r, c4);
+}
+
+__device__ __forceinline__ void split2h_quad(const float* __restrict__ src, int64_t ld_src, unsigned short* __restrict__ planes,
+                                             int64_t ld_pl, int64_t plane_stride, int mask_upper, int row_g0, int col_g0,
+                                             int ex, int r, int c4) {
+    const float scale = __builtin_bit_cast(float, (unsigned)(127 + (ex < -G3_E_MAX ? -G3_E_MAX : ex > G3_E_MAX ? G3_E_MAX : ex)) << 23);
+    f32x4 v = *(const f32x4*)(src + (size_t)r * ld_src + c4);
+    u16x4 hi, lo;
+#pragma unroll
+    for (int q = 0; q < 4; ++q) {
+        float x = v[q] * scale;
+        if (mask_upper && col_g0 + c4 + q > row_g0 + r) x = 0.0f;
+        const _Float16 h = (_Float16)x;
+        const float r1 = x - (float)h;
+        hi[q] = __builtin_bit_cast(unsigned short, h);
+        lo[q] = __builtin_bit_cast(unsigned short, (_Float16)(r1 * 2048.0f));
+    }
+    unsigned short* dst = planes + (size_t)r * ld_pl + c4;
+    *(u16x4*)dst = hi;
+    *(u16x4*)(dst + plane_stride) = lo;
+}
+
 __global__ __launch_bounds__(256) void split2h_kernel(const float* __restrict__ src, int64_t ld_src, int cols,
                                                       unsigned short* __restrict__ planes, int64_t ld_pl,
                                                       int64_t plane_stride, int mask_upper, int row_g0, int col_g0,
@@ -418,22 +445,27 @@
     const int c4 = (blockIdx.x * 256 + threadIdx.x) * 4;
     const int r = blockIdx.y;
     if (c4 >= cols) return;
-    const float scale = __builtin_bit_cast(float, (unsigned)(127 + (ex < -G3_E_MAX ? -G3_E_MAX : ex > G3_E_MAX ? G3_E_MAX : ex)) << 23);
-    f32x4 v = *(const f32x4*)(src + (size_t)r * ld_src + c4);
-    typedef __attribute__((ext_vector_type(4))) unsigned short u16x4;
-    u16x4 hi, lo;
-#pragma unroll
-    for (int q = 0; q < 4; ++q) {
-        float x = v[q] * scale;
-        if (mask_upper && col_g0 + c4 + q > row_g0 + r) x = 0.0f;
-        const _Float16 h = (_Float16)x;
-        const float r1 = x - (float)h;
-        hi[q] = __builtin_bit_cast(unsigned short, h);
-        lo[q] = __builtin_bit_cast(unsigned short, (_Float16)(r1 * 2048.0f));
-    }
-    unsigned short* dst = planes + (size_t)r * ld_pl + c4;
-    *(u16x4*)dst = hi;
-    *(u16x4*)(dst + plane_stride) = lo;
+    split2h_quad(src, ld_src, planes, ld_pl, plane_stride, mask_upper, row_g0, col_g0, ex, r, c4);
+}
+
+__global__ __launch_bounds__(256) void split3_pair_kernel(const G3SplitSrc d0, const G3SplitSrc d1, int64_t plane_stride) {
+    const bool second = (int)blockIdx.y >= d0.rows;
+    const G3SplitSrc& d = second ? d1 : d0;
+    const int r = second ? blockIdx.y - d0.rows : blockIdx.y;
+    const int c4 = (blockIdx.x * 256 + threadIdx.x) * 4;
+    if (c4 >= d.cols) return;
+    split3_quad(d.src + (size_t)blockIdx.z * d.bs_src, d.ld_src, d.planes + (size_t)blockIdx.z * d.bs_planes, d.ld_pl,
+                plane_stride, d.mask_upper, d.row_g0, d.col_g0, r, c4);
+}
+
+__global__ __launch_bounds__(256) void split2h_pair_kernel(const G3SplitSrc d0, const G3SplitSrc d1, int64_t plane_stride) {
+    const bool second = (int)blockIdx.y >= d0.rows;
+    const G3SplitSrc& d = second ? d1 : d0;
+    const int r = second ? blockIdx.y - d0.rows : blockIdx.y;
+    const int c4 = (blockIdx.x * 256 + threadIdx.x) * 4;
+    if (c4 >= d.cols) return;
+    split2h_quad(d.src + (size_t)blockIdx.z * d.bs_src, d.ld_src, d.planes + (size_t)blockIdx.z * d.bs_planes, d.ld_pl,
+                 plane_stride, d.mask_upper, d.row_g0, d.col_g0, d.e[blockIdx.z], r, c4);
 }
 
 }
@@ -491,21 +523,21 @@
     const dim3 grid(a.n_items, nb);
     const char* loop_env = getenv("QT_G3_LOOP");
     const bool chunk_loop = loop_env && strcmp(loop_env, "chunk") == 0;
-    auto launch = [&](auto loop_c) {
+    auto launch = [&](auto loop_c) -> int {
         constexpr int LOOP = decltype(loop_c)::value;
-        if (a.mode == G3_SUB) hipLaunchKernelGGL((gemm3_kernel<G3_SUB, LOOP>), grid, dim3(NTHREADS), 0, stream, p);
-        else if (a.mode == G3_ADD) hipLaunchKernelGGL((gemm3_kernel<G3_ADD, LOOP>), grid, dim3(NTHREADS), 0, stream, p);
-        else hipLaunchKernelGGL((gemm3_kernel<G3_SET, LOOP>), grid, dim3(NTHREADS), 0, stream, p);
+        if (a.mode == G3_SUB) QT_LAUNCH((gemm3_kernel<G3_SUB, LOOP>), grid, dim3(NTHREADS), 0, stream, p);
+        else if (a.mode == G3_ADD) QT_LAUNCH((gemm3_kernel<G3_ADD, LOOP>), grid, dim3(NTHREADS), 0, stream, p);
+        else QT_LAUNCH((gemm3_kernel<G3_SET, LOOP>), grid, dim3(NTHREADS), 0, stream, p);
+        return QT_OK;
     };
-    if (a.planes == G3_F16X2) launch(std::integral_constant<int, LOOP_DUO>{});
-    else if (chunk_loop) launch(std::integral_constant<int, LOOP_CHUNK>{});
-    else launch(std::integral_constant<int, LOOP_TRI>{});
-    QT_LAUNCH_CHECK();
-    if (a.n_red > 0) {
-        hipLaunchKernelGGL(gemm3_reduce_kernel, dim3(a.n_red, 16, nb), dim3(256), 0, stream, (const float*)a.slabs, a.red,
-                           a.C, a.ldc, a.M, a.N, a.mode, a.bsSlabs, a.bsC, p.C1, p.ldc1, p.N1, p.mode1, p.bsC1);
-        QT_LAUNCH_CHECK();
-    }
+    int rc;
+    if (a.planes == G3_F16X2) rc = launch(std::integral_constant<int, LOOP_DUO>{});
+    else if (chunk_loop) rc = launch(std::integral_constant<int, LOOP_CHUNK>{});
+    else rc = launch(std::integral_constant<int, LOOP_TRI>{});
+    if (rc) return rc;
+    if (a.n_red > 0)
+        QT_LAUNCH(gemm3_reduce_kernel, dim3(a.n_red, 16, nb), dim3(256), 0, stream, (const float*)a.slabs, a.red,
+                  a.C, a.ldc, a.M, a.N, a.mode, a.bsSlabs, a.bsC, p.C1, p.ldc1, p.N1, p.mode1, p.bsC1);
     return QT_OK;
 }
 
@@ -517,9 +549,8 @@
                      ((uintptr_t)src & 15) == 0 && ((uintptr_t)planes & 7) == 0,
                  "qt_split3_launch: columns / pitches must be multiples of 4 and the pointers aligned");
     QT_CHECK_ARG(bs_src % 4 == 0 && bs_planes % 4 == 0, "qt_split3_launch: batch strides must be multiples of 4");
-    hipLaunchKernelGGL(split3_kernel, dim3((cols / 4 + 255) / 256, rows, batch > 1 ? batch : 1), dim3(256), 0, stream, src,
-                       ld_src, cols, planes, ld_pl, plane_stride, mask_upper, row_g0, col_g0, bs_src, bs_planes);
-    QT_LAUNCH_CHECK();
+    QT_LAUNCH(split3_kernel, dim3((cols / 4 + 255) / 256, rows, batch > 1 ? batch : 1), dim3(256), 0, stream, src,
+              ld_src, cols, planes, ld_pl, plane_stride, mask_upper, row_g0, col_g0, bs_src, bs_planes);
     return QT_OK;
 }
 
@@ -531,9 +562,24 @@
                      ((uintptr_t)src & 15) == 0 && ((uintptr_t)planes & 7) == 0,
                  "qt_split2h_launch: columns / pitches must be multiples of 4 and the pointers aligned");
     QT_CHECK_ARG(bs_src % 4 == 0 && bs_planes % 4 == 0, "qt_split2h_launch: batch strides must be multiples of 4");
-    hipLaunchKernelGGL(split2h_kernel, dim3((cols / 4 + 255) / 256, rows, batch > 1 ? batch : 1), dim3(256), 0, stream, src,
-                       ld_src, cols, planes, ld_pl, plane_stride, mask_upper, row_g0, col_g0, bs_src, bs_planes, e);
-    QT_LAUNCH_CHECK();
+    QT_LAUNCH(split2h_kernel, dim3((cols / 4 + 255) / 256, rows, batch > 1 ? batch : 1), dim3(256), 0, stream, src,
+              ld_src, cols, planes, ld_pl, plane_stride, mask_upper, row_g0, col_g0, bs_src, bs_planes, e);
+    return QT_OK;
+}
+
+int qt_split_pair_launch(const G3SplitSrc& d0, const G3SplitSrc& d1, int64_t plane_stride, bool f16x2, hipStream_t stream,
+                         int batch) {
+    for (const G3SplitSrc* d : {&d0, &d1}) {
+        QT_CHECK_ARG(d->rows > 0 && d->cols > 0 && d->cols % 4 == 0 && d->ld_src % 4 == 0 && d->ld_pl % 4 == 0 &&
+                         ((uintptr_t)d->src & 15) == 0 && ((uintptr_t)d->planes & 7) == 0 && d->bs_src % 4 == 0 &&
+                         d->bs_planes % 4 == 0 && (!f16x2 || d->e),
+                     "qt_split_pair_launch: columns / pitches / strides must be multiples of 4 and the pointers aligned");
+    }
+    QT_CHECK_ARG(plane_stride % 4 == 0 && d0.rows + d1.rows <= 65535, "qt_split_pair_launch: plane stride / rows unsupported");
+    const int cols = d0.cols > d1.cols ? d0.cols : d1.cols;
+    const dim3 grid((cols / 4 + 255) / 256, d0.rows + d1.rows, batch > 1 ? batch : 1);
+    if (f16x2) QT_LAUNCH(split2h_pair_kernel, grid, dim3(256), 0, stream, d0, d1, plane_stride);
+    else QT_LAUNCH(split3_pair_kernel, grid, dim3(256), 0, stream, d0, d1, plane_stride);
     return QT_OK;
 }
 
diff --git a/quantool_amd/csrc/sgemm_tn.hip b/quantool_amd/csrc/sgemm_tn.hip
--- a/quantool_amd/csrc/sgemm_tn.hip
+++ b/quantool_amd/csrc/sgemm_tn.hip
@@ -303,25 +303,24 @@
             if constexpr (BM == 128 && BN == 128) {
                 if (sub8) {
                     if (a.chain_len > 0)
-                        hipLaunchKernelGGL((sgemm_tn_kernel<BM, BN, SG_MODE_SUB, true, 8>), grid, dim3(512), 0, stream, a);
+                        QT_LAUNCH((sgemm_tn_kernel<BM, BN, SG_MODE_SUB, true, 8>), grid, dim3(512), 0, stream, a);
                     else
-                        hipLaunchKernelGGL((sgemm_tn_kernel<BM, BN, SG_MODE_SUB, false, 8>), grid, dim3(512), 0, stream, a);
+                        QT_LAUNCH((sgemm_tn_kernel<BM, BN, SG_MODE_SUB, false, 8>), grid, dim3(512), 0, stream, a);
                     break;
                 }
             }
             if (a.chain_len > 0)
-                hipLaunchKernelGGL((sgemm_tn_kernel<BM, BN, SG_MODE_SUB, true>), grid, dim3(256), 0, stream, a);
+                QT_LAUNCH((sgemm_tn_kernel<BM, BN, SG_MODE_SUB, true>), grid, dim3(256), 0, stream, a);
             else
-                hipLaunchKernelGGL((sgemm_tn_kernel<BM, BN, SG_MODE_SUB>), grid, dim3(256), 0, stream, a);
+                QT_LAUNCH((sgemm_tn_kernel<BM, BN, SG_MODE_SUB>), grid, dim3(256), 0, stream, a);
             break;
         case SG_MODE_SET:
-            hipLaunchKernelGGL((sgemm_tn_kernel<BM, BN, SG_MODE_SET>), grid, dim3(256), 0, stream, a);
+            QT_LAUNCH((sgemm_tn_kernel<BM, BN, SG_MODE_SET>), grid, dim3(256), 0, stream, a);
             break;
         default:
-            hipLaunchKernelGGL((sgemm_tn_kernel<BM, BN, SG_MODE_NEG>), grid, dim3(256), 0, stream, a);
+            QT_LAUNCH((sgemm_tn_kernel<BM, BN, SG_MODE_NEG>), grid, dim3(256), 0, stream, a);
             break;
     }
-    QT_LAUNCH_CHECK();
     return QT_OK;
 }
 
@@ -330,9 +329,8 @@
 int qt_splitk_reduce(const float* slabs, int splits, int M, int N, const float* Cin, int64_t ldcin, float* Cout,
                      int64_t ldcout, int mode, hipStream_t stream, int batch, int64_t bs_slabs, int64_t bs_cin,
                      int64_t bs_cout) {
-    hipLaunchKernelGGL(splitk_reduce_kernel, dim3((N / 4 + 255) / 256 + 1, M, batch > 1 ? batch : 1), dim3(256), 0, stream,
-                       slabs, splits, M, N, Cin, ldcin, Cout, ldcout, mode, bs_slabs, bs_cin, bs_cout);
-    QT_LAUNCH_CHECK();
+    QT_LAUNCH(splitk_reduce_kernel, dim3((N / 4 + 255) / 256 + 1, M, batch > 1 ? batch : 1), dim3(256), 0, stream,
+              slabs, splits, M, N, Cin, ldcin, Cout, ldcout, mode, bs_slabs, bs_cin, bs_cout);
     return QT_OK;
 }
 
@@ -396,8 +394,7 @@
         if (r.n_tiles >= ring_min_tiles) {
             const int all = r.n_tiles * r.batch;
             const int grid = all >= 2 * 256 ? 2 * 256 : all;
-            hipLaunchKernelGGL(sgemm_ring_kernel, dim3(grid), dim3(512), 0, stream, r);
-            QT_LAUNCH_CHECK();
+            QT_LAUNCH(sgemm_ring_kernel, dim3(grid), dim3(512), 0, stream, r);
             return QT_OK;
         }
     }
diff --git a/quantool_amd/hip/_lib.py b/quantool_amd/hip/_lib.py
--- a/quantool_amd/hip/_lib.py
+++ b/quantool_amd/hip/_lib.py
@@ -1,7 +1,7 @@
 from __future__ import annotations
 
 import ctypes
-from ctypes import c_char_p, c_double, c_float, c_int, c_int32, c_int64, c_size_t, c_void_p
+from ctypes import c_char_p, c_double, c_float, c_int, c_int32, c_int64, c_longlong, c_size_t, c_void_p
 from pathlib import Path
 
 _PKG = Path(__file__).resolve().parent.parent
@@ -83,6 +83,7 @@
     "qt_gemm3_plan_check": (c_int, [c_int, c_int, c_int, c_int, c_void_p, c_void_p, c_void_p]),
     "qt_xtx_tile_table_check": (c_int, [c_int, c_void_p, c_void_p, c_void_p]),
     "qt_chol_g3_plan_check": (c_int, [c_int, c_int, c_int, c_void_p]),
+    "qt_chol_launch_count": (c_longlong, [c_int, c_int, c_int, c_int]),
     "qt_gemm3_tn_f32_workspace_bytes": (c_size_t, [c_int, c_int, c_int]),
     "qt_gemm3_tn_f32": (c_int, [c_void_p, c_int64, c_void_p, c_int64, c_void_p, c_int64, c_int, c_int, c_int, c_int,
                                 c_void_p, c_size_t, c_void_p]),
```

Result: no change. 3.305 billion (median of 6 runs) (+0.6%).
